# cc-ai/MUNIT

Measured on AMD Instinct MI355X. Metric: images/sec (gen_update+dis_update) @256x256 bs=8, higher is better.
Workload: dtype f32; 1 GPU; config_256.yaml AdaINGen_double+MsImageDis dis_update+gen_update, 256x256, per-GPU batch 8, fp32; global_batch=8, parallelism=dp1, gen_state=1

## Files before the change

### munit_amd/csrc/common.h

```cpp
#pragma once
#include <hip/hip_runtime.h>
#include <cstdarg>
#include <cstdio>
#include <cstdlib>
#include "../../include/munit_hip.h"

typedef float f32x4 __attribute__((ext_vector_type(4)));
typedef float f32x16 __attribute__((ext_vector_type(16)));

typedef __bf16 bf16_t;
typedef __bf16 bf16v4 __attribute__((ext_vector_type(4)));
typedef __bf16 bf16v8 __attribute__((ext_vector_type(8)));

__device__ inline f32x4 ld4(const float* p) { return *reinterpret_cast<const f32x4*>(p); }
__device__ inline f32x4 ld4(const bf16_t* p) {
  const bf16v4 h = *reinterpret_cast<const bf16v4*>(p);
  return f32x4{(float)h[0], (float)h[1], (float)h[2], (float)h[3]};
}
__device__ inline void st4(float* p, f32x4 v) { *reinterpret_cast<f32x4*>(p) = v; }
__device__ inline void st4(bf16_t* p, f32x4 v) {
  *reinterpret_cast<bf16v4*>(p) = bf16v4{(bf16_t)v[0], (bf16_t)v[1], (bf16_t)v[2], (bf16_t)v[3]};
}
__device__ inline float ld1(const float* p) { return *p; }
__device__ inline float ld1(const bf16_t* p) { return (float)*p; }
__device__ inline void st1(float* p, float v) { *p = v; }
__device__ inline void st1(bf16_t* p, float v) { *p = (bf16_t)v; }

void munit_set_error(const char* fmt, ...);

#define MUNIT_CHECK_ARG(cond, ...)         \
  do {                                     \
    if (!(cond)) {                         \
      munit_set_error(__VA_ARGS__);        \
      return MUNIT_ERR_ARG;                \
    }                                      \
  } while (0)

#define MUNIT_CHECK_LAUNCH(what)                                                   \
  do {                                                                             \
    hipError_t e_ = hipGetLastError();                                             \
    if (e_ != hipSuccess) {                                                        \
      munit_set_error("%s: launch failed: %s", what, hipGetErrorString(e_));       \
      return MUNIT_ERR_LAUNCH;                                                     \
    }                                                                              \
  } while (0)

#define MUNIT_ENV_FLAG(name) ([]() -> bool { static const bool v_ = getenv(name) != nullptr; return v_; }())

static inline size_t align_up(size_t v, size_t a) { return (v + a - 1) / a * a; }
static inline int cdiv(long long a, long long b) { return (int)((a + b - 1) / b); }

__device__ inline float wave_sum(float v) {
#pragma unroll
  for (int off = 32; off > 0; off >>= 1) v += __shfl_xor(v, off, 64);
  return v;
}

__device__ inline float apply_act(float v, int act, float slope) {
  if (act == MUNIT_ACT_RELU) return v > 0.f ? v : 0.f;
  if (act == MUNIT_ACT_LRELU) return v > 0.f ? v : v * slope;
  if (act == MUNIT_ACT_TANH) return tanhf(v);
  return v;
}

__device__ inline int src_coord(int v, int Hu, int ups, int reflect) {
  const bool inside = v >= 0 && v < Hu;
  int r = v < 0 ? -v : v;
  r = r >= Hu ? 2 * Hu - 2 - r : r;
  r = reflect ? r : (inside ? v : -1);
  return r < 0 ? -1 : (r >> ups);
}

double munit_igemm_executed_flops(const munit_conv_desc* d, int pass);
const char* munit_igemm_kernel_name(const munit_conv_desc* d, int pass);

bool munit_small_fwd_supported(const munit_conv_desc* d);
bool munit_small_fwd_ok(const munit_conv_desc* d);
bool munit_small_wgrad_ok(const munit_conv_desc* d);
enum SmallFwdKernel { SMALL_FWD_PK, SMALL_FWD_MFMA, SMALL_FWD_PATCH };
SmallFwdKernel munit_small_fwd_kernel(int Cin);
bool munit_small_wgrad_pk();
size_t munit_small_fwd_workspace(const munit_conv_desc* d);
int munit_small_fwd(const munit_conv_desc* d, int Ho, int Wo, const void* x, const float* w, const float* bias,
                    float* y, void* ws, hipStream_t st);
size_t munit_small_wgrad_workspace(const munit_conv_desc* d, int Ho);
int munit_small_wgrad(const munit_conv_desc* d, int Ho, int Wo, const void* x, const float* dy, float* dw,
                      float* db, float beta, void* ws, hipStream_t st);
```

### munit_amd/csrc/conv_igemm.hip

```cpp
#include "common.h"
#include "wino.h"
#include <cstdlib>

namespace {

struct IgemmParams {
  const float* x;
  const float* w;
  const float* bias;
  void* y;
  int B, H, W, Cin;
  int Hu, Wu, ups;
  int Ho, Wo, Cout;
  int KH, KW, stride, pad, reflect;
  int Ktot;
  long long w_row;
  long long y_sb;
  long long y_sh;
  int y_sw;
  int M;
  int act;
  float slope;
  int ps;
  long long w_phase;
  long long y_phase_row;
  int y_phase_col;
  int n_tiles;
  int f_pad, f_ups, f_reflect, f_Hu, f_Wu;
  int frame;
  int ksplit, kt_per_split;
  float* slab;
  int ct;
  int patch;
  int out_bf16;
  int bf16s;
  int cin4;
};

__device__ inline f32x4 bf16x8_add4(f32x4 l, f32x4 a, f32x4 b, f32x4 c) {
  const bf16v8 L = __builtin_bit_cast(bf16v8, l), A = __builtin_bit_cast(bf16v8, a), B = __builtin_bit_cast(bf16v8, b),
               C = __builtin_bit_cast(bf16v8, c);
  bf16v8 r;
#pragma unroll
  for (int e = 0; e < 8; ++e) r[e] = (bf16_t)((float)L[e] + (((float)A[e] + (float)B[e]) + (float)C[e]));
  return __builtin_bit_cast(f32x4, r);
}

__device__ inline void decode_pixel(int m, int Ho, int Wo, int frame, int& b, int& oh, int& ow) {
  if (!frame) {
    const int HoWo = Ho * Wo;
    b = m / HoWo;
    const int rem = m - b * HoWo;
    oh = rem / Wo;
    ow = rem - oh * Wo;
  } else {
    const int F = frame, F2 = 2 * frame;
    const int nb = F2 * Wo + F2 * (Ho - F2);
    b = m / nb;
    int r = m - b * nb;
    if (r < F2 * Wo) {
      const int q = r / Wo;
      ow = r - q * Wo;
      oh = q < F ? q : Ho - F2 + q;
    } else {
      r -= F2 * Wo;
      const int rr = r / F2, q = r - rr * F2;
      oh = F + rr;
      ow = q < F ? q : Wo - F2 + q;
    }
  }
}

constexpr int BM = 128;
constexpr int BK = 32;
#ifndef IGEMM_WAVES
#define IGEMM_WAVES 8
#endif
constexpr int NWAVES = IGEMM_WAVES;
constexpr int NTHR = 64 * NWAVES;
constexpr int LDS_LD = BK + 4;

__device__ inline uint2 fold_cands(int i, int Hu, int ups, int P, int reflect) {
  unsigned long long pk = ~0ull;
  int n = 0;
  auto push = [&](int v) {
    if (n < 4) {
      const int sh = 16 * n;
      pk = (pk & ~(0xFFFFull << sh)) | ((unsigned long long)(unsigned)v << sh);
      ++n;
    }
  };
  const int nu = 1 << ups;
  for (int du = 0; du < nu; ++du) {
    const int hu = (i << ups) + du;
    push(hu + P);
    if (reflect) {
      if (hu >= 1 && hu <= P) push(P - hu);
      if (hu >= Hu - 1 - P && hu <= Hu - 2) push(2 * Hu - 2 - hu + P);
    }
  }
  return make_uint2((unsigned)(pk & 0xFFFFFFFFull), (unsigned)(pk >> 32));
}
__device__ inline int cand_at(uint2 v, int a) {
  const unsigned w = (a & 2) ? v.y : v.x;
  return (int)((w >> ((a & 1) * 16)) & 0xFFFFu);
}

typedef __bf16 bf16x4 __attribute__((ext_vector_type(4)));
typedef __bf16 bf16x8 __attribute__((ext_vector_type(8)));

__device__ const float munit_zero_page[32] = {0.f};

template <int BN, bool ALIGNED, int ROLE, int CT = 0>
__global__ __launch_bounds__(NTHR, NWAVES == 8 ? ((CT == 3 && BN == 64) ? 6 : 4) : 2) void conv_igemm_kernel(IgemmParams p) {
  constexpr bool BF16 = CT == 1 || CT == 2;
  constexpr bool DMA = CT == 3 || CT == 4 || CT == 5;
  constexpr bool BF16S = CT == 4;
  constexpr bool CIN4 = CT == 5;
  static_assert(!CIN4 || ROLE != 2, "4-channel taps: single-gather roles only");
  static_assert(!DMA || (ALIGNED && NWAVES == 8), "direct-to-LDS loads: aligned variants only");
  constexpr bool PATCH = DMA && ROLE == 2;
  constexpr int NPL = CT == 2 ? 3 : 1;
  static_assert(!BF16 || ALIGNED, "bf16 operands need Cin % 32 == 0");
  constexpr int WN = NWAVES == 8 ? 32 : 64;
  constexpr int WAVES_N = BN / WN;
  constexpr int WAVES_M = NWAVES / WAVES_N;
  constexpr int WM = BM / WAVES_M;
  constexpr int MT = WM / 16;
  constexpr int NT = WN / 16;
#ifndef IGEMM_LOADER_WAVES
#define IGEMM_LOADER_WAVES 8
#endif
  constexpr int LW = (CT == 3 && ROLE != 2 && NWAVES == 8) ? IGEMM_LOADER_WAVES : NWAVES;
  constexpr int RSTEP = 64 * LW / 8;
  constexpr int AROWS = BM / RSTEP;
  constexpr int BROWS = BN / RSTEP;
  constexpr int CLD = BN + 4;
  static_assert(BM * CLD <= 2 * (BM + BN) * LDS_LD, "C staging tile must fit in the operand buffers");
  constexpr int SMEM_FLOATS = DMA ? (2 * (BM + BN) * 32 > BM * CLD ? 2 * (BM + BN) * 32 : BM * CLD) : 2 * (BM + BN) * LDS_LD;
  __shared__ __attribute__((aligned(16))) float smem[SMEM_FLOATS];
  float* const As = smem;
  float* const Bs = smem + 2 * BM * LDS_LD;

  const int tid = threadIdx.x;
  const int lane = tid & 63;
  const int wave = tid >> 6;
  const int wm = wave / WAVES_N, wn = wave % WAVES_N;

  int tile = blockIdx.x;
  {
    const int nb = gridDim.x, q = nb >> 3, r = nb & 7, xcd = tile & 7, idx = tile >> 3;
    tile = (xcd < r ? xcd * (q + 1) : r * (q + 1) + (xcd - r) * q) + idx;
  }
  const int n_tile = tile % p.n_tiles;
  const int m_tile = tile / p.n_tiles;
  const int m0 = m_tile * BM;
  const int n0 = n_tile * BN;

  const float* __restrict__ xg = p.x;
  const float* __restrict__ wg = p.w;
  long long y_base = 0;
  if (p.ps > 1) {
    const int pa = blockIdx.y / p.ps, pb = blockIdx.y % p.ps;
    wg += (long long)blockIdx.y * p.w_phase;
    y_base = (long long)pa * p.y_phase_row + (long long)pb * p.y_phase_col;
  }

  const int c4 = tid & 7;
  const int r0 = tid >> 3;
  int a_base[AROWS];
  int a_ih0[AROWS], a_iw0[AROWS];
  bool a_ok[AROWS];
  uint2 a_ch[AROWS], a_cw[AROWS];
  int a_nc[AROWS];
  int f_h1[PATCH ? AROWS : 1], f_w1[PATCH ? AROWS : 1];
#pragma unroll
  for (int i = 0; i < AROWS; ++i) {
    int m = m0 + r0 + RSTEP * i;
    a_ok[i] = m < p.M;
    int mm = a_ok[i] ? m : 0;
    int b, oh, ow;
    decode_pixel(mm, p.Ho, p.Wo, p.frame, b, oh, ow);
    a_base[i] = b * p.H * p.W;
    a_ih0[i] = oh * p.stride - p.pad;
    a_iw0[i] = ow * p.stride - p.pad;
    if constexpr (PATCH) {
      constexpr int NONE = -(1 << 20);
      const int P = p.f_pad, K1 = p.KH - 1;
      int h1 = NONE, w1 = NONE;
      if (p.f_reflect) {
        if (oh >= 1 && oh <= P) h1 = P - oh - K1;
        else if (oh >= p.f_Hu - 1 - P && oh <= p.f_Hu - 2) h1 = 2 * p.f_Hu - 2 - oh + P - K1;
        if (ow >= 1 && ow <= P) w1 = P - ow - K1;
        else if (ow >= p.f_Wu - 1 - P && ow <= p.f_Wu - 2) w1 = 2 * p.f_Wu - 2 - ow + P - K1;
      }
      a_ih0[i] = oh + P - K1;
      a_iw0[i] = ow + P - K1;
      f_h1[i] = h1;
      f_w1[i] = w1;
    } else if constexpr (ROLE == 2) {
      a_ch[i] = fold_cands(oh, p.f_Hu, p.f_ups, p.f_pad, p.f_reflect);
      a_cw[i] = fold_cands(ow, p.f_Wu, p.f_ups, p.f_pad, p.f_reflect);
      int nh = 0, nw = 0;
      for (int a = 0; a < 4; ++a) {
        nh += cand_at(a_ch[i], a) != 0xFFFF;
        nw += cand_at(a_cw[i], a) != 0xFFFF;
      }
      a_nc[i] = nh | (nw << 4);
    }
  }

  f32x4 ra[AROWS], rb[BROWS];
  f32x4 rx[ROLE == 2 ? AROWS : 1];
  int kh = 0, kw = 0, c0 = 0;
  const int nk_total = (p.Ktot + BK - 1) / BK;
  const int kt_begin = p.ksplit > 1 ? blockIdx.z * p.kt_per_split : 0;
  const int kt_end = p.ksplit > 1 ? min(nk_total, kt_begin + p.kt_per_split) : nk_total;
  if constexpr (ALIGNED) {
    if (kt_begin > 0) {
      const int k0 = kt_begin * BK, tap = k0 / p.Cin;
      c0 = k0 - tap * p.Cin;
      kh = tap / p.KW;
      kw = tap - kh * p.KW;
    }
  }
  int aoff[AROWS];
  int aoff1[ROLE == 2 ? AROWS : 1];
  int aoffp[PATCH ? 3 : 1][AROWS];
  f32x4 xp[PATCH ? 3 : 1][AROWS];
  bool wave_patch = false;

  auto tap_setup = [&]() {
#pragma unroll
    for (int i = 0; i < AROWS; ++i) {
      if constexpr (PATCH) {
        const int vh0 = a_ih0[i] + kh, vh1 = f_h1[i] + kh, vw0 = a_iw0[i] + kw, vw1 = f_w1[i] + kw;
        const bool h0 = a_ok[i] && (unsigned)vh0 < (unsigned)p.H, h1 = a_ok[i] && (unsigned)vh1 < (unsigned)p.H;
        const bool w0 = (unsigned)vw0 < (unsigned)p.W, w1 = (unsigned)vw1 < (unsigned)p.W;
        aoff[i] = (h0 && w0) ? (a_base[i] + vh0 * p.W + vw0) * p.Cin : -1;
        aoffp[0][i] = (h0 && w1) ? (a_base[i] + vh0 * p.W + vw1) * p.Cin : -1;
        aoffp[1][i] = (h1 && w0) ? (a_base[i] + vh1 * p.W + vw0) * p.Cin : -1;
        aoffp[2][i] = (h1 && w1) ? (a_base[i] + vh1 * p.W + vw1) * p.Cin : -1;
        if (i == 0) wave_patch = false;
        wave_patch = wave_patch || __builtin_amdgcn_ballot_w64((aoffp[0][i] & aoffp[1][i] & aoffp[2][i]) >= 0) != 0;
      } else if constexpr (ROLE == 2) {
        const int nw = a_nc[i] >> 4;
        const int ncomb = (a_nc[i] & 15) * nw;
        int o0 = -1, o1 = -1;
        {
          const int vh = cand_at(a_ch[i], 0) + kh - (p.KH - 1);
          const int vw = cand_at(a_cw[i], 0) + kw - (p.KW - 1);
          const bool ok = a_ok[i] && vh >= 0 && vh < p.H && vw >= 0 && vw < p.W;
          o0 = ok ? (a_base[i] + vh * p.W + vw) * p.Cin : -1;
        }
        {
          const int vh = cand_at(a_ch[i], nw >= 2 ? 0 : 1) + kh - (p.KH - 1);
          const int vw = cand_at(a_cw[i], nw >= 2 ? 1 : 0) + kw - (p.KW - 1);
          const bool ok = a_ok[i] && ncomb >= 2 && vh >= 0 && vh < p.H && vw >= 0 && vw < p.W;
          o1 = ok ? (a_base[i] + vh * p.W + vw) * p.Cin : -1;
        }
        aoff[i] = o0;
        aoff1[i] = o1;
      } else {
        const int ih = src_coord(a_ih0[i] + kh, p.Hu, p.ups, p.reflect);
        const int iw = src_coord(a_iw0[i] + kw, p.Wu, p.ups, p.reflect);
        const bool ok = a_ok[i] && ih >= 0 && iw >= 0;
        aoff[i] = ok ? (a_base[i] + ih * p.W + iw) * p.Cin : -1;
      }
    }
  };

  auto load_tile = [&](int kt) {
    if constexpr (ALIGNED) {
      if (c0 == 0 || kt == kt_begin) tap_setup();
#pragma unroll
      for (int i = 0; i < AROWS; ++i) {
        f32x4 v = {0.f, 0.f, 0.f, 0.f};
        if (aoff[i] >= 0) v = *reinterpret_cast<const f32x4*>(xg + (long long)aoff[i] + c0 + c4 * 4);
        if constexpr (ROLE == 2) {
          f32x4 x1 = {0.f, 0.f, 0.f, 0.f};
          if (aoff1[i] >= 0) x1 = *reinterpret_cast<const f32x4*>(xg + (long long)aoff1[i] + c0 + c4 * 4);
          const int nw = a_nc[i] >> 4;
          const int ncomb = (a_nc[i] & 15) * nw;
          if (a_ok[i] && ncomb > 2) {
            for (int cidx = 2; cidx < ncomb; cidx += 2) {
              f32x4 t0 = {0.f, 0.f, 0.f, 0.f}, t1 = {0.f, 0.f, 0.f, 0.f};
              {
                const int a = cidx / nw, b2 = cidx - a * nw;
                const int vh = cand_at(a_ch[i], a) + kh - (p.KH - 1);
                const int vw = cand_at(a_cw[i], b2) + kw - (p.KW - 1);
                if (vh >= 0 && vh < p.H && vw >= 0 && vw < p.W)
                  t0 = *reinterpret_cast<const f32x4*>(xg + (long long)(a_base[i] + vh * p.W + vw) * p.Cin + c0 + c4 * 4);
              }
              if (cidx + 1 < ncomb) {
                const int a = (cidx + 1) / nw, b2 = cidx + 1 - a * nw;
                const int vh = cand_at(a_ch[i], a) + kh - (p.KH - 1);
                const int vw = cand_at(a_cw[i], b2) + kw - (p.KW - 1);
                if (vh >= 0 && vh < p.H && vw >= 0 && vw < p.W)
                  t1 = *reinterpret_cast<const f32x4*>(xg + (long long)(a_base[i] + vh * p.W + vw) * p.Cin + c0 + c4 * 4);
              }
              x1 += t0 + t1;
            }
          }
          rx[i] = x1;
        }
        ra[i] = v;
      }
#pragma unroll
      for (int i = 0; i < BROWS; ++i) {
        const int n = n0 + r0 + RSTEP * i;
        f32x4 v = {0.f, 0.f, 0.f, 0.f};
        if (n < p.Cout) v = *reinterpret_cast<const f32x4*>(wg + (long long)n * p.w_row + kt * BK + c4 * 4);
        rb[i] = v;
      }
      c0 += BK;
      if (c0 >= p.Cin) {
        c0 = 0;
        if (++kw == p.KW) { kw = 0; ++kh; }
      }
    } else {
      int ekh[4], ekw[4], eci[4];
      bool eok[4];
#pragma unroll
      for (int e = 0; e < 4; ++e) {
        int k = kt * BK + c4 * 4 + e;
        eok[e] = k < p.Ktot;
        int kk = eok[e] ? k : 0;
        int tap = kk / p.Cin;
        eci[e] = kk - tap * p.Cin;
        ekh[e] = tap / p.KW;
        ekw[e] = tap - ekh[e] * p.KW;
      }
#pragma unroll
      for (int i = 0; i < AROWS; ++i) {
        f32x4 v;
#pragma unroll
        for (int e = 0; e < 4; ++e) {
          int ih = src_coord(a_ih0[i] + ekh[e], p.Hu, p.ups, p.reflect);
          int iw = src_coord(a_iw0[i] + ekw[e], p.Wu, p.ups, p.reflect);
          bool ok = a_ok[i] && eok[e] && ih >= 0 && iw >= 0;
          float s = 0.f;
          if (ok) s = xg[(a_base[i] + (long long)ih * p.W + iw) * p.Cin + eci[e]];
          v[e] = s;
        }
        ra[i] = v;
      }
#pragma unroll
      for (int i = 0; i < BROWS; ++i) {
        int n = n0 + r0 + RSTEP * i;
        f32x4 v;
#pragma unroll
        for (int e = 0; e < 4; ++e) {
          int k = kt * BK + c4 * 4 + e;
          float s = 0.f;
          if (n < p.Cout && k < p.Ktot) s = wg[(long long)n * p.w_row + k];
          v[e] = s;
        }
        rb[i] = v;
      }
    }
  };

  const int dma_col = ((c4 ^ ((r0 >> 1) & 7)) * 4);
  auto dma_tile = [&](int kt, int buf) {
    if constexpr (DMA) {
      if (LW < NWAVES && __builtin_amdgcn_readfirstlane(wave) >= LW) return;
      if constexpr (!CIN4) {
        if (c0 == 0 || kt == kt_begin) tap_setup();
      }
      const int wrow = __builtin_amdgcn_readfirstlane(wave) * 8;
      const int tap4 = kt * 8 + (dma_col >> 2);
      const int kh4 = tap4 / p.KW, kw4 = tap4 - kh4 * p.KW;
#pragma unroll
      for (int i = 0; i < AROWS; ++i) {
        const float* g;
        if constexpr (CIN4) {
          const int ih = src_coord(a_ih0[i] + kh4, p.Hu, p.ups, p.reflect);
          const int iw = src_coord(a_iw0[i] + kw4, p.Wu, p.ups, p.reflect);
          const bool ok = a_ok[i] && tap4 < p.KH * p.KW && ih >= 0 && iw >= 0;
          g = ok ? xg + (long long)(a_base[i] + ih * p.W + iw) * 4 : munit_zero_page;
        } else {
          g = aoff[i] >= 0 ? xg + (long long)aoff[i] + c0 + dma_col : munit_zero_page + dma_col;
        }
        float* l = smem + buf * (BM * 32) + (wrow + RSTEP * i) * 32;
        __builtin_amdgcn_global_load_lds((const __attribute__((address_space(1))) void*)g,
                                         (__attribute__((address_space(3))) void*)l, 16, 0, 0);
        if constexpr (PATCH) {
          if (wave_patch) {
#pragma unroll
            for (int c = 0; c < 3; ++c) {
              f32x4 v = {0.f, 0.f, 0.f, 0.f};
              if (aoffp[c][i] >= 0) v = *reinterpret_cast<const f32x4*>(xg + (long long)aoffp[c][i] + c0 + dma_col);
              xp[c][i] = v;
            }
          }
        }
      }
#pragma unroll
      for (int i = 0; i < BROWS; ++i) {
        const int n = min(n0 + r0 + RSTEP * i, p.Cout - 1);
        const float* g = wg + (long long)n * p.w_row + kt * BK + dma_col;
        float* l = smem + 2 * BM * 32 + buf * (BN * 32) + (wrow + RSTEP * i) * 32;
        __builtin_amdgcn_global_load_lds((const __attribute__((address_space(1))) void*)g,
                                         (__attribute__((address_space(3))) void*)l, 16, 0, 0);
      }
      if constexpr (!CIN4) {
        c0 += BK;
        if (c0 >= p.Cin) {
          c0 = 0;
          if (++kw == p.KW) { kw = 0; ++kh; }
        }
      }
    }
  };

  __bf16* const Ah = reinterpret_cast<__bf16*>(smem);
  __bf16* const Bh = Ah + (CT == 2 ? 3 : 2) * BM * 32;
  const int st_swz = (0x78 >> (2 * ((r0 >> 2) & 3))) & 3;
  const int st_col = (((c4 >> 1) ^ st_swz) * 8) + (c4 & 1) * 4;
  auto store_tile = [&](int buf) {
    if constexpr (BF16) {
      auto put = [&](__bf16* base, int plane_elems, int row, f32x4 v) {
#pragma unroll
        for (int pl = 0; pl < NPL; ++pl) {
          bf16x4 h;
#pragma unroll
          for (int e = 0; e < 4; ++e) h[e] = (__bf16)v[e];
          *reinterpret_cast<bf16x4*>(&base[pl * plane_elems + row * 32 + st_col]) = h;
          if (pl + 1 < NPL) {
#pragma unroll
            for (int e = 0; e < 4; ++e) v[e] -= (float)h[e];
          }
        }
      };
#pragma unroll
      for (int i = 0; i < AROWS; ++i) {
        if constexpr (ROLE == 2) ra[i] += rx[i];
        put(Ah + buf * NPL * (BM * 32), BM * 32, r0 + RSTEP * i, ra[i]);
      }
#pragma unroll
      for (int i = 0; i < BROWS; ++i) put(Bh + buf * NPL * (BN * 32), BN * 32, r0 + RSTEP * i, rb[i]);
      return;
    }
    float* Ad = As + buf * (BM * LDS_LD);
    float* Bd = Bs + buf * (BN * LDS_LD);
#pragma unroll
    for (int i = 0; i < AROWS; ++i) {
      if constexpr (ROLE == 2) ra[i] += rx[i];
      *reinterpret_cast<f32x4*>(&Ad[(r0 + RSTEP * i) * LDS_LD + c4 * 4]) = ra[i];
    }
#pragma unroll
    for (int i = 0; i < BROWS; ++i)
      *reinterpret_cast<f32x4*>(&Bd[(r0 + RSTEP * i) * LDS_LD + c4 * 4]) = rb[i];
  };

  f32x4 acc[MT][NT];
#pragma unroll
  for (int mt = 0; mt < MT; ++mt)
#pragma unroll
    for (int nt = 0; nt < NT; ++nt)
#pragma unroll
      for (int r = 0; r < 4; ++r) acc[mt][nt][r] = 0.f;

  const int frag_row = lane & 15;
  const int frag_k = (lane >> 4) * 4;
  const int fr_col = (((lane >> 4) ^ ((0x78 >> (2 * ((frag_row >> 2) & 3))) & 3)) * 8);
  auto compute_half = [&](int buf, int kg) {
    if constexpr (BF16) {
      const __bf16* Ac = Ah + buf * NPL * (BM * 32);
      const __bf16* Bc = Bh + buf * NPL * (BN * 32);
      bf16x8 hb[NPL][NT];
#pragma unroll
      for (int pl = 0; pl < NPL; ++pl)
#pragma unroll
        for (int nt = 0; nt < NT; ++nt)
          hb[pl][nt] = *reinterpret_cast<const bf16x8*>(&Bc[pl * (BN * 32) + (wn * WN + nt * 16 + frag_row) * 32 + fr_col]);
#pragma unroll
      for (int mt = kg * (MT / 2); mt < (kg + 1) * (MT / 2); ++mt) {
        bf16x8 ha[NPL];
#pragma unroll
        for (int pl = 0; pl < NPL; ++pl)
          ha[pl] = *reinterpret_cast<const bf16x8*>(&Ac[pl * (BM * 32) + (wm * WM + mt * 16 + frag_row) * 32 + fr_col]);
#pragma unroll
        for (int sum = NPL - 1; sum >= 0; --sum)
#pragma unroll
          for (int i = 0; i <= sum; ++i)
#pragma unroll
            for (int nt = 0; nt < NT; ++nt)
              acc[mt][nt] = __builtin_amdgcn_mfma_f32_16x16x32_bf16(ha[i], hb[sum - i][nt], acc[mt][nt], 0, 0, 0);
      }
      return;
    }
    if constexpr (DMA) {
      const float* Ac = smem + buf * (BM * 32);
      const float* Bc = smem + 2 * BM * 32 + buf * (BN * 32);
      const int pos = ((kg * 4 + (lane >> 4)) ^ ((frag_row >> 1) & 7)) * 4;
      f32x4 a[MT], b[NT];
#pragma unroll
      for (int nt = 0; nt < NT; ++nt)
        b[nt] = *reinterpret_cast<const f32x4*>(&Bc[(wn * WN + nt * 16 + frag_row) * 32 + pos]);
#pragma unroll
      for (int mt = 0; mt < MT; ++mt)
        a[mt] = *reinterpret_cast<const f32x4*>(&Ac[(wm * WM + mt * 16 + frag_row) * 32 + pos]);
      if constexpr (BF16S) {
#pragma unroll
        for (int mt = 0; mt < MT; ++mt)
#pragma unroll
          for (int nt = 0; nt < NT; ++nt)
            acc[mt][nt] = __builtin_amdgcn_mfma_f32_16x16x32_bf16(__builtin_bit_cast(bf16x8, a[mt]),
                                                                  __builtin_bit_cast(bf16x8, b[nt]), acc[mt][nt], 0, 0, 0);
        return;
      }
#pragma unroll
      for (int t = 0; t < 4; ++t)
#pragma unroll
        for (int mt = 0; mt < MT; ++mt)
#pragma unroll
          for (int nt = 0; nt < NT; ++nt)
            acc[mt][nt] = __builtin_amdgcn_mfma_f32_16x16x4f32(a[mt][t], b[nt][t], acc[mt][nt], 0, 0, 0);
      return;
    }
    const float* Ac = As + buf * (BM * LDS_LD);
    const float* Bc = Bs + buf * (BN * LDS_LD);
    f32x4 a[MT], b[NT];
#pragma unroll
    for (int nt = 0; nt < NT; ++nt)
      b[nt] = *reinterpret_cast<const f32x4*>(&Bc[(wn * WN + nt * 16 + frag_row) * LDS_LD + kg * 16 + frag_k]);
    constexpr int MB = (ROLE == 2 && MT >= 4) ? MT / 2 : MT;
#pragma unroll
    for (int m0t = 0; m0t < MT; m0t += MB) {
#pragma unroll
      for (int mt = m0t; mt < m0t + MB; ++mt)
        a[mt] = *reinterpret_cast<const f32x4*>(&Ac[(wm * WM + mt * 16 + frag_row) * LDS_LD + kg * 16 + frag_k]);
#pragma unroll
      for (int t = 0; t < 4; ++t)
#pragma unroll
        for (int mt = m0t; mt < m0t + MB; ++mt)
#pragma unroll
          for (int nt = 0; nt < NT; ++nt)
            acc[mt][nt] = __builtin_amdgcn_mfma_f32_16x16x4f32(a[mt][t], b[nt][t], acc[mt][nt], 0, 0, 0);
      if constexpr (MB != MT) __builtin_amdgcn_sched_barrier(0);
    }
  };

  const int nk = kt_end - kt_begin;
  auto patch_tile = [&](int buf) {
    if constexpr (PATCH) {
      if (!wave_patch) return;
#pragma unroll
      for (int i = 0; i < AROWS; ++i) {
        if ((aoffp[0][i] & aoffp[1][i] & aoffp[2][i]) >= 0) {
          f32x4* l = reinterpret_cast<f32x4*>(smem + buf * (BM * 32) + (r0 + RSTEP * i) * 32 + c4 * 4);
          if constexpr (BF16S) *l = bf16x8_add4(*l, xp[0][i], xp[1][i], xp[2][i]);
          else *l = *l + ((xp[0][i] + xp[1][i]) + xp[2][i]);
        }
      }
    }
  };
  if constexpr (DMA) {
    if (nk > 0) dma_tile(kt_begin, 0);
    asm volatile("s_waitcnt vmcnt(0)" ::: "memory");
    if (nk > 0) patch_tile(0);
    __syncthreads();
    for (int kt = 0; kt < nk; ++kt) {
      const int cur = kt & 1;
      if (kt + 1 < nk) dma_tile(kt_begin + kt + 1, cur ^ 1);
      compute_half(cur, 0);
      compute_half(cur, 1);
      asm volatile("s_waitcnt vmcnt(0)" ::: "memory");
      if (kt + 1 < nk) patch_tile(cur ^ 1);
      __syncthreads();
    }
  } else if constexpr (CT == 2) {
    if (nk > 0) load_tile(kt_begin);
    for (int kt = 0; kt < nk; ++kt) {
      __syncthreads();
      store_tile(0);
      if (kt + 1 < nk) load_tile(kt_begin + kt + 1);
      __syncthreads();
      compute_half(0, 0);
      compute_half(0, 1);
    }
    __syncthreads();
  } else {
    if (nk > 0) {
      load_tile(kt_begin);
      store_tile(0);
    }
    __syncthreads();
    if (nk > 1) load_tile(kt_begin + 1);
    for (int kt = 0; kt < nk; ++kt) {
      const int cur = kt & 1;
      compute_half(cur, 0);
      if (kt + 1 < nk) {
#ifndef ABL_NOLDSW
        store_tile(cur ^ 1);
#endif
#ifndef ABL_NOGLOBAL
        if (kt + 2 < nk) load_tile(kt_begin + kt + 2);
#endif
      }
      if constexpr (ROLE == 2) __builtin_amdgcn_sched_barrier(0);
      compute_half(cur, 1);
#ifndef ABL_NOBAR
      __syncthreads();
#endif
    }
  }

  float* const Cs = smem;
#pragma unroll
  for (int nt = 0; nt < NT; ++nt)
#pragma unroll
    for (int mt = 0; mt < MT; ++mt)
#pragma unroll
      for (int r = 0; r < 4; ++r)
        Cs[(wm * WM + mt * 16 + 4 * (lane >> 4) + r) * CLD + wn * WN + nt * 16 + (lane & 15)] = acc[mt][nt][r];
  __syncthreads();
  constexpr int CQ = BN / 4;
  constexpr int CRPT = NTHR / CQ;
  const int cq = tid % CQ, cr0 = tid / CQ;
  const int n = n0 + cq * 4;
  const bool split = p.ksplit > 1;
  float* const sl = split ? p.slab + ((long long)blockIdx.y * p.ksplit + blockIdx.z) * (long long)p.M * p.Cout : nullptr;
  const bool vec = (p.Cout & 3) == 0 && (split || ((p.y_sw & 3) == 0 && (p.y_sh & 3) == 0 && (p.y_sb & 3) == 0));
  f32x4 bv = {0.f, 0.f, 0.f, 0.f};
  if (!split && p.bias != nullptr) {
#pragma unroll
    for (int e = 0; e < 4; ++e)
      if (n + e < p.Cout) bv[e] = p.bias[n + e];
  }
#pragma unroll 2
  for (int row = cr0; row < BM; row += CRPT) {
    const int m = m0 + row;
    if (m >= p.M || n >= p.Cout) continue;
    f32x4 v = *reinterpret_cast<const f32x4*>(&Cs[row * CLD + cq * 4]);
    if (split) {
      float* dst = sl + (long long)m * p.Cout + n;
      if (vec) {
        *reinterpret_cast<f32x4*>(dst) = v;
      } else {
#pragma unroll
        for (int e = 0; e < 4; ++e)
          if (n + e < p.Cout) dst[e] = v[e];
      }
      continue;
    }
    int b, oh, ow;
    decode_pixel(m, p.Ho, p.Wo, p.frame, b, oh, ow);
    const long long off = y_base + (long long)b * p.y_sb + (long long)oh * p.y_sh + (long long)ow * p.y_sw + n;
#pragma unroll
    for (int e = 0; e < 4; ++e) v[e] = apply_act(v[e] + bv[e], p.act, p.slope);
    if (p.out_bf16) {
      bf16_t* dst = reinterpret_cast<bf16_t*>(p.y) + off;
      if (vec) {
        st4(dst, v);
      } else {
#pragma unroll
        for (int e = 0; e < 4; ++e)
          if (n + e < p.Cout) dst[e] = (bf16_t)v[e];
      }
    } else {
      float* dst = reinterpret_cast<float*>(p.y) + off;
      if (vec) {
        *reinterpret_cast<f32x4*>(dst) = v;
      } else {
#pragma unroll
        for (int e = 0; e < 4; ++e)
          if (n + e < p.Cout) dst[e] = v[e];
      }
    }
  }
}

__global__ void splitk_epilogue_kernel(IgemmParams p, int phases) {
  const long long per = (long long)p.M * p.Cout;
  const long long total = per * phases;
  for (long long i = (long long)blockIdx.x * blockDim.x + threadIdx.x; i < total;
       i += (long long)gridDim.x * blockDim.x) {
    const int ph = (int)(i / per);
    const long long r = i - (long long)ph * per;
    const int m = (int)(r / p.Cout), n = (int)(r - (long long)m * p.Cout);
    float s = 0.f;
    for (int k = 0; k < p.ksplit; ++k) s += p.slab[((long long)ph * p.ksplit + k) * per + r];
    int b, oh, ow;
    decode_pixel(m, p.Ho, p.Wo, p.frame, b, oh, ow);
    long long off = (long long)b * p.y_sb + (long long)oh * p.y_sh + (long long)ow * p.y_sw + n;
    if (p.ps > 1) off += (long long)(ph / p.ps) * p.y_phase_row + (long long)(ph % p.ps) * p.y_phase_col;
    const float bv = p.bias != nullptr ? p.bias[n] : 0.f;
    const float res = apply_act(s + bv, p.act, p.slope);
    if (p.out_bf16) reinterpret_cast<bf16_t*>(p.y)[off] = (bf16_t)res;
    else reinterpret_cast<float*>(p.y)[off] = res;
  }
}

typedef munit_prep_item PrepItem;

__device__ inline void prep_dgrad_elem(const PrepItem& it, long long i) {
  const int ps = it.ps, TH = it.KH / ps, TW = it.KW / ps;
  long long r_ = i;
  int co = (int)(r_ % it.Cout); r_ /= it.Cout;
  int r = (int)(r_ % TW); r_ /= TW;
  int t = (int)(r_ % TH); r_ /= TH;
  int ci = (int)(r_ % it.Cin); r_ /= it.Cin;
  int ph = (int)r_;
  int pa = ph / ps, pb = ph % ps;
  int kh = pa + ps * (TH - 1 - t);
  int kw = pb + ps * (TW - 1 - r);
  const float v = it.w[(((long long)co * it.KH + kh) * it.KW + kw) * it.Cin + ci];
  if (it.bf16) reinterpret_cast<bf16_t*>(it.wp)[i] = (bf16_t)v;
  else it.wp[i] = v;
}

__device__ inline void prep_cast_elem(const PrepItem& it, long long i) { reinterpret_cast<bf16_t*>(it.wp)[i] = (bf16_t)it.w[i]; }

__device__ inline void prep_subpixel_elem(const PrepItem& it, long long i) {
  const long long merged = (long long)4 * 9 * it.Cout * it.Cin;
  if (i >= merged) {
    reinterpret_cast<bf16_t*>(it.wp)[i] = (bf16_t)it.w[i - merged];
    return;
  }
  long long r = i;
  const int ci = (int)(r % it.Cin); r /= it.Cin;
  const int dw = (int)(r % 3); r /= 3;
  const int dh = (int)(r % 3); r /= 3;
  const int co = (int)(r % it.Cout); r /= it.Cout;
  const int ph = (int)r;
  const int a = ph >> 1, b = ph & 1;
  const int h0 = a == 0 ? (dh == 0 ? 0 : dh == 1 ? 2 : 4) : (dh == 0 ? 0 : dh == 1 ? 1 : 3);
  const int hn = a == 0 ? (dh == 2 ? 1 : 2) : (dh == 0 ? 1 : 2);
  const int w0 = b == 0 ? (dw == 0 ? 0 : dw == 1 ? 2 : 4) : (dw == 0 ? 0 : dw == 1 ? 1 : 3);
  const int wn = b == 0 ? (dw == 2 ? 1 : 2) : (dw == 0 ? 1 : 2);
  float s = 0.f;
  for (int kh = h0; kh < h0 + hn; ++kh)
    for (int kw = w0; kw < w0 + wn; ++kw) s += it.w[(((long long)co * 5 + kh) * 5 + kw) * it.Cin + ci];
  if (it.bf16) reinterpret_cast<bf16_t*>(it.wp)[i] = (bf16_t)s;
  else it.wp[i] = s;
}

__host__ __device__ inline long long prep_elems(const PrepItem& it) {
  const long long cc = (long long)it.Cout * it.Cin;
  if (it.kind == MUNIT_PREP_SUBPIXEL) return it.bf16 ? (4 * 9 + 25) * cc : 4 * 9 * cc;
  if (it.kind == MUNIT_PREP_WINOGRAD || it.kind == MUNIT_PREP_WINOGRAD_DGRAD) return wino_image_elems(it.Cin, it.Cout);
  if (it.kind == MUNIT_PREP_SUBPIXEL_WINOGRAD_DGRAD) return cc * it.KH * it.KW + 4 * wino_image_elems(it.Cin, it.Cout);
  if (it.kind == MUNIT_PREP_SUBPIXEL_WINOGRAD || it.kind == MUNIT_PREP_WINOGRAD_S2 || it.kind == MUNIT_PREP_WINOGRAD_S2_DGRAD)
    return 4 * wino_image_elems(it.Cin, it.Cout);
  return cc * it.KH * it.KW;
}

__host__ __device__ inline long long prep_trips(const PrepItem& it) {
  const bool wino = it.kind == MUNIT_PREP_WINOGRAD || it.kind == MUNIT_PREP_WINOGRAD_DGRAD || it.kind == MUNIT_PREP_SUBPIXEL_WINOGRAD ||
                    it.kind == MUNIT_PREP_WINOGRAD_S2 || it.kind == MUNIT_PREP_WINOGRAD_S2_DGRAD;
  if (it.kind == MUNIT_PREP_SUBPIXEL_WINOGRAD_DGRAD) return (long long)it.Cout * it.Cin * (it.KH * it.KW + 4);
  return wino ? prep_elems(it) / 16 : prep_elems(it);
}
template <bool DEV>
__global__ void prep_weights_kernel(const PrepItem* __restrict__ items, PrepItem one) {
  const PrepItem it = DEV ? items[blockIdx.y] : one;
  const long long total = prep_trips(it);
  for (long long i = (long long)blockIdx.x * blockDim.x + threadIdx.x; i < total; i += (long long)gridDim.x * blockDim.x) {
    if (it.kind == MUNIT_PREP_SUBPIXEL) prep_subpixel_elem(it, i);
    else if (it.kind == MUNIT_PREP_WINOGRAD || it.kind == MUNIT_PREP_WINOGRAD_DGRAD)
      wino_weight_item(it.w, it.wp, it.Cout, it.Cin, it.kind == MUNIT_PREP_WINOGRAD_DGRAD, i);
    else if (it.kind == MUNIT_PREP_SUBPIXEL_WINOGRAD) wino_subpixel_weight_item(it.w, it.wp, it.Cout, it.Cin, i);
    else if (it.kind == MUNIT_PREP_WINOGRAD_S2) wino_s2_weight_item(it.w, it.wp, it.Cout, it.Cin, i);
    else if (it.kind == MUNIT_PREP_WINOGRAD_S2_DGRAD) wino_s2_dgrad_weight_item(it.w, it.wp, it.Cout, it.Cin, i);
    else if (it.kind == MUNIT_PREP_SUBPIXEL_WINOGRAD_DGRAD) {
      const long long nd = (long long)it.Cout * it.Cin * it.KH * it.KW;
      if (i < nd) prep_dgrad_elem(it, i);
      else wino_subpixel_dgrad_weight_item(it.w, it.wp + nd, it.Cout, it.Cin, i - nd);
    }
    else if (it.kind == MUNIT_PREP_CAST) prep_cast_elem(it, i);
    else prep_dgrad_elem(it, i);
  }
}

int launch_prep_one(const PrepItem& it, hipStream_t st) {
  const long long total = prep_trips(it);
  const int blocks = (int)std::min<long long>((total + 255) / 256, 4096);
  hipLaunchKernelGGL(prep_weights_kernel<false>, dim3(blocks), dim3(256), 0, st, nullptr, it);
  MUNIT_CHECK_LAUNCH("prep_weights");
  return MUNIT_OK;
}

template <typename T>
__global__ void fold_kernel(const T* __restrict__ g, const T* __restrict__ add,
                            T* __restrict__ dx, int B, int H, int W, int C, int ups, int pad,
                            int reflect, int Hq, int Wq) {
  const int C4 = C >> 2;
  const long long total = (long long)B * H * W * C4;
  const int Hu = H << ups, Wu = W << ups;
  for (long long i = (long long)blockIdx.x * blockDim.x + threadIdx.x; i < total;
       i += (long long)gridDim.x * blockDim.x) {
    long long r_ = i;
    int c4 = (int)(r_ % C4); r_ /= C4;
    int iw = (int)(r_ % W); r_ /= W;
    int ih = (int)(r_ % H); r_ /= H;
    int b = (int)r_;
    f32x4 s = {0.f, 0.f, 0.f, 0.f};
    const int nu = 1 << ups;
    for (int du = 0; du < nu; ++du) {
      int hu = (ih << ups) + du;
      int qr[3], nr = 0;
      qr[nr++] = hu + pad;
      if (reflect) {
        if (hu >= 1 && hu <= pad) qr[nr++] = pad - hu;
        if (hu >= Hu - 1 - pad && hu <= Hu - 2) qr[nr++] = 2 * Hu - 2 - hu + pad;
      }
      for (int dv = 0; dv < nu; ++dv) {
        int wu = (iw << ups) + dv;
        int qc[3], nc = 0;
        qc[nc++] = wu + pad;
        if (reflect) {
          if (wu >= 1 && wu <= pad) qc[nc++] = pad - wu;
          if (wu >= Wu - 1 - pad && wu <= Wu - 2) qc[nc++] = 2 * Wu - 2 - wu + pad;
        }
        for (int a = 0; a < nr; ++a) {
          if (qr[a] >= Hq) continue;
          for (int c = 0; c < nc; ++c) {
            if (qc[c] >= Wq) continue;
            s += ld4(g + (((long long)b * Hq + qr[a]) * Wq + qc[c]) * C + c4 * 4);
          }
        }
      }
    }
    if (add != nullptr) s += ld4(add + i * 4);
    st4(dx + i * 4, s);
  }
}

__global__ void fold_scalar_kernel(const float* __restrict__ g, const float* __restrict__ add,
                                   float* __restrict__ dx, int B, int H, int W, int C, int ups, int pad,
                                   int reflect, int Hq, int Wq) {
  const long long total = (long long)B * H * W * C;
  const int Hu = H << ups, Wu = W << ups;
  for (long long i = (long long)blockIdx.x * blockDim.x + threadIdx.x; i < total;
       i += (long long)gridDim.x * blockDim.x) {
    long long r_ = i;
    int c = (int)(r_ % C); r_ /= C;
    int iw = (int)(r_ % W); r_ /= W;
    int ih = (int)(r_ % H); r_ /= H;
    int b = (int)r_;
    float s = 0.f;
    const int nu = 1 << ups;
    for (int du = 0; du < nu; ++du) {
      int hu = (ih << ups) + du;
      int qr[3], nr = 0;
      qr[nr++] = hu + pad;
      if (reflect) {
        if (hu >= 1 && hu <= pad) qr[nr++] = pad - hu;
        if (hu >= Hu - 1 - pad && hu <= Hu - 2) qr[nr++] = 2 * Hu - 2 - hu + pad;
      }
      for (int dv = 0; dv < nu; ++dv) {
        int wu = (iw << ups) + dv;
        int qc[3], nc = 0;
        qc[nc++] = wu + pad;
        if (reflect) {
          if (wu >= 1 && wu <= pad) qc[nc++] = pad - wu;
          if (wu >= Wu - 1 - pad && wu <= Wu - 2) qc[nc++] = 2 * Wu - 2 - wu + pad;
        }
        for (int a = 0; a < nr; ++a) {
          if (qr[a] >= Hq) continue;
          for (int cc = 0; cc < nc; ++cc) {
            if (qc[cc] >= Wq) continue;
            s += g[(((long long)b * Hq + qr[a]) * Wq + qc[cc]) * C + c];
          }
        }
      }
    }
    if (add != nullptr) s += add[i];
    dx[i] = s;
  }
}

__global__ void add_inplace_kernel(float* __restrict__ y, const float* __restrict__ a, long long n) {
  for (long long i = (long long)blockIdx.x * blockDim.x + threadIdx.x; i < n; i += (long long)gridDim.x * blockDim.x)
    y[i] += a[i];
}

int pick_ksplit(int M, int Cout, int Ktot, int phases) {
  const int bn = Cout <= 64 ? 64 : 128;
  const int tiles = cdiv(M, BM) * cdiv(Cout, bn) * phases;
  const int nk = cdiv(Ktot, BK);
  if (tiles >= 192 || nk < 16 || MUNIT_ENV_FLAG("MUNIT_DEBUG_NO_SPLITK")) return 1;
  int ks = std::min(cdiv(512, tiles), nk / 4);
  return std::max(1, std::min(ks, 32));
}
size_t splitk_bytes(int M, int Cout, int Ktot, int phases) {
  const int ks = pick_ksplit(M, Cout, Ktot, phases);
  return ks > 1 ? align_up((size_t)ks * phases * M * Cout * sizeof(float), 256) : 0;
}

enum IgemmForm {
  IG_REFUSED_BF16_CIN, IG_REFUSED_CIN4_FOLD, IG_REFUSED_BF16_FOLD, IG_REFUSED_FOLD_UNALIGNED,
  IG_CIN4,
  IG_BF16S,
  IG_PATCH,
  IG_DMA,
  IG_CT2,
  IG_CT1,
  IG_F32,
  IG_UNALIGNED
};
IgemmForm igemm_form(const IgemmParams& p, int role) {
  if (p.bf16s && (p.Cin % (2 * BK) != 0 || NWAVES != 8)) return IG_REFUSED_BF16_CIN;
  const int cin = p.bf16s ? p.Cin / 2 : p.Cin, w_row = p.bf16s ? p.w_row / 2 : p.w_row;
  const bool aligned = (cin % BK == 0) && (w_row % 4 == 0);
  if (p.cin4) return role == 2 ? IG_REFUSED_CIN4_FOLD : IG_CIN4;
  if (p.bf16s) return role == 2 && (!p.patch || p.frame) ? IG_REFUSED_BF16_FOLD : IG_BF16S;
  if (role == 2) {
    if (!aligned) return IG_REFUSED_FOLD_UNALIGNED;
    if (p.ct == 0 && p.patch && !p.frame && NWAVES == 8 && !MUNIT_ENV_FLAG("MUNIT_DEBUG_NO_PATCH")) return IG_PATCH;
    return p.ct == 2 ? IG_CT2 : p.ct == 1 ? IG_CT1 : IG_F32;
  }
  if (aligned && p.ct == 0 && NWAVES == 8 && !MUNIT_ENV_FLAG("MUNIT_DEBUG_NO_DMA")) return IG_DMA;
  if (!aligned) return IG_UNALIGNED;
  return p.ct == 2 ? IG_CT2 : p.ct == 1 ? IG_CT1 : IG_F32;
}
int igemm_bn(const IgemmParams& p) { return p.Cout <= 64 ? 64 : 128; }

#define IGEMM_LAUNCH(...)                                                                                  \
  do {                                                                                                     \
    if (bn == 64) hipLaunchKernelGGL((conv_igemm_kernel<64, __VA_ARGS__>), grid, block, 0, st, q);         \
    else hipLaunchKernelGGL((conv_igemm_kernel<128, __VA_ARGS__>), grid, block, 0, st, q);                 \
  } while (0)

template <int ROLE>
int launch_igemm(const IgemmParams& p, int phases, hipStream_t st, void* slab = nullptr, size_t slab_bytes = 0) {
  const int bn = igemm_bn(p);
  IgemmParams q = p;
  const IgemmForm form = igemm_form(p, ROLE);
  switch (form) {
    case IG_REFUSED_BF16_CIN:
      munit_set_error("conv_igemm: bf16 storage needs a multiple of 64 input channels (got %d)", p.Cin);
      return MUNIT_ERR_ARG;
    case IG_REFUSED_CIN4_FOLD:
      munit_set_error("conv_igemm: 4-channel taps are not a folded-backward-data form");
      return MUNIT_ERR_ARG;
    case IG_REFUSED_BF16_FOLD:
      munit_set_error("conv_igemm: bf16-storage folded backward-data exists for the LDS-patch form only");
      return MUNIT_ERR_ARG;
    case IG_REFUSED_FOLD_UNALIGNED:
      munit_set_error("conv_igemm: folded backward-data needs Cout %% 32 == 0");
      return MUNIT_ERR_ARG;
    default: break;
  }
  if (p.bf16s) {
    q.Cin = p.Cin / 2; q.Ktot = p.Ktot / 2; q.w_row = p.w_row / 2; q.w_phase = p.w_phase / 2;
    slab = nullptr;
  }
  q.n_tiles = cdiv(p.Cout, bn);
  const int m_tiles = cdiv(p.M, BM);
  q.ksplit = 1;
  if (slab != nullptr) {
    const int ks = pick_ksplit(p.M, p.Cout, p.Ktot, phases);
    if (ks > 1 && slab_bytes >= splitk_bytes(p.M, p.Cout, p.Ktot, phases)) {
      const int nk = cdiv(p.Ktot, BK);
      q.kt_per_split = cdiv(nk, ks);
      q.ksplit = cdiv(nk, q.kt_per_split);
      q.slab = reinterpret_cast<float*>(slab);
    }
  }
  dim3 grid((unsigned)(m_tiles * q.n_tiles), (unsigned)phases, (unsigned)q.ksplit);
  dim3 block(NTHR);
  switch (form) {
    case IG_CIN4:
      if constexpr (ROLE != 2) IGEMM_LAUNCH(true, ROLE, 5);
      break;
    case IG_BF16S: IGEMM_LAUNCH(true, ROLE, 4); break;
    case IG_PATCH: IGEMM_LAUNCH(true, 2, 3); break;
    case IG_DMA: IGEMM_LAUNCH(true, ROLE, 3); break;
    case IG_CT2: IGEMM_LAUNCH(true, ROLE, 2); break;
    case IG_CT1: IGEMM_LAUNCH(true, ROLE, 1); break;
    case IG_F32: IGEMM_LAUNCH(true, ROLE); break;
    default:
      if constexpr (ROLE != 2) IGEMM_LAUNCH(false, ROLE);
      break;
  }
  MUNIT_CHECK_LAUNCH("conv_igemm");
  if (q.ksplit > 1) {
    const long long total = (long long)p.M * p.Cout * phases;
    const int blocks = (int)std::min<long long>((total + 255) / 256, 4096);
    hipLaunchKernelGGL(splitk_epilogue_kernel, dim3(blocks), dim3(256), 0, st, q, phases);
    MUNIT_CHECK_LAUNCH("splitk_epilogue");
  }
  return MUNIT_OK;
}

int check_desc(const munit_conv_desc* d) {
  MUNIT_CHECK_ARG(d != nullptr, "conv: null descriptor");
  MUNIT_CHECK_ARG(d->B > 0 && d->H > 0 && d->W > 0 && d->Cin > 0 && d->Cout > 0, "conv: bad dims");
  MUNIT_CHECK_ARG(d->KH > 0 && d->KW > 0 && d->stride > 0 && d->pad >= 0, "conv: bad kernel geometry");
  MUNIT_CHECK_ARG(d->upsample == 0 || d->upsample == 1, "conv: upsample must be 0 or 1");
  MUNIT_CHECK_ARG(d->compute >= MUNIT_COMPUTE_F32 && d->compute <= MUNIT_COMPUTE_F32X3, "conv: bad compute mode %d", d->compute);
  MUNIT_CHECK_ARG(d->pad_mode == MUNIT_PAD_ZERO || d->pad_mode == MUNIT_PAD_REFLECT, "conv: bad pad mode");
  MUNIT_CHECK_ARG((d->in_dtype == MUNIT_DTYPE_F32 || d->in_dtype == MUNIT_DTYPE_BF16) &&
                  (d->out_dtype == MUNIT_DTYPE_F32 || d->out_dtype == MUNIT_DTYPE_BF16), "conv: bad tensor dtype");
  MUNIT_CHECK_ARG(d->in_dtype == MUNIT_DTYPE_F32 || d->Cin % 64 == 0, "conv: a bf16 input needs Cin %% 64 == 0 (got %d)", d->Cin);
  MUNIT_CHECK_ARG(d->out_dtype == MUNIT_DTYPE_F32 || d->Cout % 64 == 0, "conv: a bf16 output needs Cout %% 64 == 0 (got %d)", d->Cout);
  const int Hu = d->H << d->upsample, Wu = d->W << d->upsample;
  if (d->pad_mode == MUNIT_PAD_REFLECT)
    MUNIT_CHECK_ARG(d->pad < Hu && d->pad < Wu, "conv: reflect pad %d needs input > pad (got %dx%d)", d->pad, Hu, Wu);
  MUNIT_CHECK_ARG(Hu + 2 * d->pad >= d->KH && Wu + 2 * d->pad >= d->KW, "conv: kernel larger than padded input");
  MUNIT_CHECK_ARG((long long)d->B * Hu * Wu < (1ll << 31) / 4, "conv: too many pixels for 32-bit tile indices");
  MUNIT_CHECK_ARG((long long)d->B * (Hu + 2 * d->pad) * (Wu + 2 * d->pad) * std::max(d->Cin, d->Cout) < (1ll << 31),
                  "conv: tensor too large for the 32-bit element offsets of the tile loader");
  return MUNIT_OK;
}

}

extern "C" int munit_conv2d_out_hw(const munit_conv_desc* d, int* Ho, int* Wo) {
  int rc = check_desc(d);
  if (rc) return rc;
  *Ho = ((d->H << d->upsample) + 2 * d->pad - d->KH) / d->stride + 1;
  *Wo = ((d->W << d->upsample) + 2 * d->pad - d->KW) / d->stride + 1;
  return MUNIT_OK;
}

namespace {
bool subpixel_ok(const munit_conv_desc* d) {
  return d->upsample == 1 && d->KH == 5 && d->KW == 5 && d->pad == 2 && d->stride == 1 &&
         d->pad_mode == MUNIT_PAD_REFLECT && d->Cin % 32 == 0 && d->H >= 3 && d->W >= 3 &&
         !MUNIT_ENV_FLAG("MUNIT_DEBUG_NO_SUBPIXEL");
}
}

namespace {
__global__ void pad3to4_image_kernel(const float* __restrict__ x, f32x4* __restrict__ x4, long long npix) {
  for (long long i = (long long)blockIdx.x * blockDim.x + threadIdx.x; i < npix; i += (long long)gridDim.x * blockDim.x)
    x4[i] = f32x4{x[3 * i], x[3 * i + 1], x[3 * i + 2], 0.f};
}
__global__ void pad3to4_weight_kernel(const float* __restrict__ w, float* __restrict__ w4, int N, int taps, int kpad) {
  const long long total = (long long)N * kpad;
  for (long long i = (long long)blockIdx.x * blockDim.x + threadIdx.x; i < total; i += (long long)gridDim.x * blockDim.x) {
    const int n = (int)(i / kpad), k = (int)(i - (long long)n * kpad);
    const int tap = k >> 2, c = k & 3;
    w4[i] = (tap < taps && c < 3) ? w[((long long)n * taps + tap) * 3 + c] : 0.f;
  }
}
struct Cin4Plan {
  int kpad;
  size_t x4_bytes, w4_bytes;
};
Cin4Plan plan_cin4(long long npix, int N, int taps) {
  Cin4Plan c;
  c.kpad = (taps * 4 + BK - 1) / BK * BK;
  c.x4_bytes = align_up((size_t)npix * 4 * sizeof(float), 256);
  c.w4_bytes = align_up((size_t)N * c.kpad * sizeof(float), 256);
  return c;
}
int build_cin4(const Cin4Plan& c, const float* x3, long long npix, const float* w3, int N, int taps, void* ws, hipStream_t st) {
  f32x4* x4 = reinterpret_cast<f32x4*>(ws);
  float* w4 = reinterpret_cast<float*>(reinterpret_cast<char*>(ws) + c.x4_bytes);
  hipLaunchKernelGGL(pad3to4_image_kernel, dim3((unsigned)std::min<long long>((npix + 255) / 256, 8192)), dim3(256), 0, st, x3, x4, npix);
  MUNIT_CHECK_LAUNCH("pad3to4_image");
  hipLaunchKernelGGL(pad3to4_weight_kernel, dim3((unsigned)cdiv((long long)N * c.kpad, 256)), dim3(256), 0, st, w3, w4, N, taps, c.kpad);
  MUNIT_CHECK_LAUNCH("pad3to4_weight");
  return MUNIT_OK;
}
bool cin4_fwd_ok(const munit_conv_desc* d) {
  return d->Cin == 3 && d->in_dtype == MUNIT_DTYPE_F32 && d->upsample == 0 && d->KH * d->KW <= 64 && d->Cout % 4 == 0 &&
         NWAVES == 8 && !MUNIT_ENV_FLAG("MUNIT_DEBUG_NO_CIN4");
}

void set_cin4(IgemmParams* p, const Cin4Plan& c) { p->Ktot = c.kpad; p->w_row = c.kpad; p->cin4 = 1; }

IgemmParams fwd_params(const munit_conv_desc* d, int Ho, int Wo) {
  IgemmParams p{};
  p.B = d->B; p.H = d->H; p.W = d->W; p.Cin = d->Cin;
  p.ups = d->upsample; p.Hu = d->H << p.ups; p.Wu = d->W << p.ups;
  p.Ho = Ho; p.Wo = Wo; p.Cout = d->Cout;
  p.KH = d->KH; p.KW = d->KW; p.stride = d->stride; p.pad = d->pad;
  p.reflect = d->pad_mode == MUNIT_PAD_REFLECT;
  p.Ktot = d->KH * d->KW * d->Cin;
  p.w_row = p.Ktot;
  p.y_sw = d->Cout;
  p.y_sh = (long long)Wo * d->Cout;
  p.y_sb = (long long)Ho * Wo * d->Cout;
  p.M = d->B * Ho * Wo;
  p.act = d->act; p.slope = d->slope;
  p.ct = d->compute;
  p.ps = 1;
  p.bf16s = d->in_dtype == MUNIT_DTYPE_BF16;
  p.out_bf16 = d->out_dtype == MUNIT_DTYPE_BF16;
  return p;
}
IgemmParams subpixel_phase_params(const IgemmParams& p, const munit_conv_desc* d, int Wo) {
  IgemmParams q = p;
  q.ups = 0; q.Hu = d->H; q.Wu = d->W;
  q.Ho = d->H; q.Wo = d->W;
  q.KH = 3; q.KW = 3; q.pad = 1; q.reflect = 0;
  q.Ktot = 9 * d->Cin; q.w_row = q.Ktot;
  q.y_sw = 2 * d->Cout;
  q.y_sh = (long long)2 * Wo * d->Cout;
  q.M = d->B * d->H * d->W;
  q.ps = 2;
  q.w_phase = (long long)d->Cout * q.Ktot;
  q.y_phase_row = (long long)Wo * d->Cout;
  q.y_phase_col = d->Cout;
  return q;
}
void set_subpixel_frame(IgemmParams* p, const munit_conv_desc* d, int Ho, int Wo, int ring) {
  p->frame = ring;
  p->M = d->B * (2 * ring * Wo + 2 * ring * (Ho - 2 * ring));
}

bool wino_geometry_ok(const munit_conv_desc* d) {
  return d->compute == MUNIT_COMPUTE_F32 && d->in_dtype == MUNIT_DTYPE_F32 && d->out_dtype == MUNIT_DTYPE_F32 &&
         d->KH == 3 && d->KW == 3 && d->stride == 1 && d->pad == 1 && d->upsample == 0 && d->act != MUNIT_ACT_TANH;
}
bool wino_fwd_ok(const munit_conv_desc* d) { return wino_geometry_ok(d) && munit_wino_ok(d->B, d->H, d->W, d->Cin, d->Cout); }
long long wino_s2_min_blocks(bool dgrad) {
  static const char* const e = getenv("MUNIT_WINO_S2_MIN_BLOCKS");
  static const long long v = e ? atoll(e) : 0;
  return e ? v : dgrad ? 100 : 192;
}
bool wino_s2_fwd_ok(const munit_conv_desc* d) {
  return d->compute == MUNIT_COMPUTE_F32 && d->in_dtype == MUNIT_DTYPE_F32 && d->out_dtype == MUNIT_DTYPE_F32 && d->KH == 4 &&
         d->KW == 4 && d->stride == 2 && d->pad == 1 && d->upsample == 0 && d->act != MUNIT_ACT_TANH && d->H >= 4 && d->W >= 4 &&
         munit_wino_ok(d->B, d->H, d->W, d->Cin, d->Cout) && !MUNIT_ENV_FLAG("MUNIT_DEBUG_NO_WINOGRAD_S2") &&
         (long long)cdiv((long long)d->B * cdiv(d->H / 2, 3) * cdiv(d->W / 2, 3), 64) * (d->Cout / 64) >= wino_s2_min_blocks(false);
}
bool wino_s2_dgrad_ok(const munit_conv_desc* d) {
  if (!(d->compute == MUNIT_COMPUTE_F32 && d->in_dtype == MUNIT_DTYPE_F32 && d->out_dtype == MUNIT_DTYPE_F32 && d->KH == 4 &&
        d->KW == 4 && d->stride == 2 && d->pad == 1 && d->upsample == 0 && d->H >= 4 && d->W >= 4 && d->H % 2 == 0 && d->W % 2 == 0 &&
        d->Cout % 8 == 0 && d->Cin % 64 == 0 && !MUNIT_ENV_FLAG("MUNIT_DEBUG_NO_WINOGRAD_S2") && !MUNIT_ENV_FLAG("MUNIT_DEBUG_NO_WINOGRAD")))
    return false;
  const int Hd = d->H / 2, Wd = d->W / 2;
  if (d->pad_mode == MUNIT_PAD_REFLECT && (Hd % 3 == 0 || Wd % 3 == 0)) return false;
  if ((long long)d->B * d->H * d->W * std::max(d->Cin, d->Cout) >= (1ll << 29)) return false;
  return (long long)cdiv((long long)d->B * cdiv(Hd + 1, 3) * cdiv(Wd + 1, 3), 64) * (d->Cin / 64) * 4 >= wino_s2_min_blocks(true);
}
bool subpixel_wino_ok(const munit_conv_desc* d) {
  return d->compute == MUNIT_COMPUTE_F32 && d->in_dtype == MUNIT_DTYPE_F32 && d->out_dtype == MUNIT_DTYPE_F32 &&
         d->act != MUNIT_ACT_TANH && munit_wino_ok(d->B, d->H, d->W, d->Cin, d->Cout);
}

enum FwdRoute { FWD_SMALL, FWD_SUBPIXEL_WINO, FWD_SUBPIXEL, FWD_WINO, FWD_WINO_S2, FWD_CIN4, FWD_IGEMM };
struct FwdPlan {
  int rc;
  FwdRoute route;
  int Ho, Wo;
  munit_prep_item prep;
  Cin4Plan cin4;
  int ring;
  size_t img_bytes, ws_bytes;
};
FwdPlan plan_fwd(const munit_conv_desc* d) {
  FwdPlan pl{};
  if ((pl.rc = munit_conv2d_out_hw(d, &pl.Ho, &pl.Wo)) != MUNIT_OK) return pl;
  const int Ho = pl.Ho, Wo = pl.Wo, Ktot = d->KH * d->KW * d->Cin;
  const bool bf16 = d->in_dtype == MUNIT_DTYPE_BF16;
  int kind = bf16 ? MUNIT_PREP_CAST : MUNIT_PREP_NONE;
  if (munit_small_fwd_ok(d)) {
    pl.route = FWD_SMALL; kind = MUNIT_PREP_NONE;
  } else if (subpixel_ok(d)) {
    const bool wino = subpixel_wino_ok(d);
    pl.route = wino ? FWD_SUBPIXEL_WINO : FWD_SUBPIXEL; kind = wino ? MUNIT_PREP_SUBPIXEL_WINOGRAD : MUNIT_PREP_SUBPIXEL;
    pl.ring = wino ? 1 : 2;
  } else if (wino_fwd_ok(d)) {
    pl.route = FWD_WINO; kind = MUNIT_PREP_WINOGRAD;
  } else if (wino_s2_fwd_ok(d)) {
    pl.route = FWD_WINO_S2; kind = MUNIT_PREP_WINOGRAD_S2;
  } else {
    pl.route = cin4_fwd_ok(d) ? FWD_CIN4 : FWD_IGEMM;
  }
  pl.prep = munit_prep_item{nullptr, nullptr, d->Cout, d->KH, d->KW, d->Cin, kind, 1, pl.route != FWD_SMALL && bf16};
  pl.ws_bytes = pl.img_bytes = kind == MUNIT_PREP_NONE ? 0 : align_up((size_t)prep_elems(pl.prep) * (bf16 ? 2 : 4), 256);
  if (pl.route == FWD_SMALL) pl.ws_bytes = munit_small_fwd_workspace(d);
  if (pl.route == FWD_CIN4) pl.cin4 = plan_cin4((long long)d->B * d->H * d->W, d->Cout, d->KH * d->KW), pl.ws_bytes = pl.cin4.x4_bytes + pl.cin4.w4_bytes;
  if (bf16 || munit_small_fwd_supported(d)) return pl;
  if (pl.ring)
    pl.ws_bytes += std::max(splitk_bytes(d->B * (4 * Wo + 4 * (Ho - 4)), d->Cout, Ktot, 1), splitk_bytes(d->B * (2 * Wo + 2 * (Ho - 2)), d->Cout, Ktot, 1));
  if (pl.route == FWD_IGEMM) pl.ws_bytes += splitk_bytes(d->B * Ho * Wo, d->Cout, Ktot, 1);
  return pl;
}

enum WinoForm { WINO_FWD, WINO_FWD_S2, WINO_FWD_SUBPIXEL, WINO_DGRAD, WINO_DGRAD_S2, WINO_DGRAD_UP };
WinoParams wino_params(const munit_conv_desc* d, int Ho, int Wo, WinoForm f, const float* x, const float* u, const float* bias, float* y) {
  const bool fwd = f <= WINO_FWD_SUBPIXEL, refl = d->pad_mode == MUNIT_PAD_REFLECT;
  WinoParams q{};
  q.x = x; q.u = u; q.bias = bias; q.y = y;
  q.B = d->B; q.H = d->H; q.W = d->W;
  q.xc = fwd ? d->Cin : d->Cout; q.N = fwd ? d->Cout : d->Cin; q.K = q.xc;
  const int oh = fwd ? Ho : d->H, ow = fwd ? Wo : d->W;
  q.y_sw = q.N; q.y_sh = (long long)ow * q.N; q.y_sb = (long long)oh * ow * q.N;
  q.mode = refl ? 0 : 1;
  q.th = d->H / 2; q.tw = d->W / 2;
  q.act = fwd ? d->act : MUNIT_ACT_NONE; q.slope = fwd ? d->slope : 0.f;
  switch (f) {
    case WINO_FWD: break;
    case WINO_FWD_S2:
      q.K = 4 * q.xc; q.s2 = 1; q.Ho = Ho; q.Wo = Wo;
      q.th = cdiv(Ho, 3); q.tw = cdiv(Wo, 3);
      break;
    case WINO_FWD_SUBPIXEL:
      q.y_sw *= 2; q.y_sh *= 2; q.y_prow = (long long)Wo * d->Cout; q.y_pcol = d->Cout;
      q.u_phase = wino_image_elems(d->Cin, d->Cout); q.phases = 4;
      q.mode = 1; q.edge = 1;
      break;
    case WINO_DGRAD: q.mode = refl ? 2 : 1; break;
    case WINO_DGRAD_S2:
      q.H = d->H / 2; q.W = d->W / 2; q.s2 = 2; q.Ho = d->H; q.Wo = d->W;
      q.th = cdiv(q.H + 1, 3); q.tw = cdiv(q.W + 1, 3);
      q.u_phase = wino_image_elems(d->Cout, d->Cin); q.phases = 4;
      break;
    case WINO_DGRAD_UP:
      q.H = Ho; q.W = Wo; q.K = 4 * q.xc; q.s2 = 3; q.mode = 1;
      q.th = (d->H - 4) / 2; q.tw = (d->W - 4) / 2;
      break;
  }
  q.cpp = q.xc / 8; q.NB = q.N / 64;
  q.x_bytes = (unsigned)((size_t)d->B * q.H * q.W * q.xc * 4);
  q.bth = cdiv(q.th, 8); q.btw = cdiv(q.tw, 8);
  return q;
}
}

extern "C" size_t munit_conv2d_fwd_workspace_bytes(const munit_conv_desc* d) {
  const FwdPlan pl = plan_fwd(d);
  return pl.rc ? 0 : pl.ws_bytes;
}

extern "C" int munit_conv2d_fwd(const munit_conv_desc* d, const void* x, const float* w,
                                const float* bias, void* y, void* ws, size_t ws_bytes,
                                munit_stream_t stream) {
  return munit_conv2d_fwd_prepared(d, x, w, nullptr, bias, y, ws, ws_bytes, stream);
}

extern "C" int munit_conv2d_fwd_prepared(const munit_conv_desc* d, const void* x, const float* w, const void* wp,
                                         const float* bias, void* y, void* ws, size_t ws_bytes,
                                         munit_stream_t stream) {
  const FwdPlan pl = plan_fwd(d);
  int rc = pl.rc;
  if (rc) return rc;
  const int Ho = pl.Ho, Wo = pl.Wo;
  MUNIT_CHECK_ARG(x && w && y, "conv2d_fwd: null pointer");
  MUNIT_CHECK_ARG(pl.route != FWD_SMALL || d->out_dtype == MUNIT_DTYPE_F32, "conv2d_fwd: the 3-channel image head writes fp32");
  hipStream_t st = (hipStream_t)stream;
  if (pl.ws_bytes != 0 && (ws == nullptr || ws_bytes < pl.ws_bytes)) {
    munit_set_error("conv2d_fwd: workspace %zu < %zu", ws_bytes, pl.ws_bytes);
    return MUNIT_ERR_WORKSPACE;
  }
  if (pl.route == FWD_SMALL) return munit_small_fwd(d, Ho, Wo, x, w, bias, reinterpret_cast<float*>(y), ws, st);
  const float* wimg = w;
  if (pl.prep.kind != MUNIT_PREP_NONE) {
    wimg = reinterpret_cast<const float*>(wp);
    if (wimg == nullptr) {
      munit_prep_item it = pl.prep;
      it.w = w; it.wp = reinterpret_cast<float*>(ws);
      rc = launch_prep_one(it, st);
      if (rc) return rc;
      wimg = it.wp;
    }
  }
  if (pl.route == FWD_WINO || pl.route == FWD_WINO_S2 || pl.route == FWD_SUBPIXEL_WINO) {
    const WinoForm f = pl.route == FWD_WINO ? WINO_FWD : pl.route == FWD_WINO_S2 ? WINO_FWD_S2 : WINO_FWD_SUBPIXEL;
    rc = munit_wino_launch(wino_params(d, Ho, Wo, f, reinterpret_cast<const float*>(x), wimg, bias, reinterpret_cast<float*>(y)), st);
    if (rc || pl.route != FWD_SUBPIXEL_WINO) return rc;
  }
  IgemmParams p = fwd_params(d, Ho, Wo);
  p.x = reinterpret_cast<const float*>(x); p.w = wimg; p.bias = bias; p.y = y;
  if (pl.route == FWD_CIN4) {
    const long long npix = (long long)d->B * d->H * d->W;
    rc = build_cin4(pl.cin4, reinterpret_cast<const float*>(x), npix, w, d->Cout, d->KH * d->KW, ws, st);
    if (rc) return rc;
    p.x = reinterpret_cast<const float*>(ws);
    p.w = reinterpret_cast<const float*>(reinterpret_cast<const char*>(ws) + pl.cin4.x4_bytes);
    set_cin4(&p, pl.cin4);
    return launch_igemm<0>(p, 1, st);
  }
  if (pl.ring) {
    if (pl.route == FWD_SUBPIXEL) rc = launch_igemm<0>(subpixel_phase_params(p, d, Wo), 4, st);
    if (rc) return rc;
    set_subpixel_frame(&p, d, Ho, Wo, pl.ring);
    p.w = pl.prep.bf16 ? reinterpret_cast<const float*>(reinterpret_cast<const bf16_t*>(wimg) + (size_t)4 * 9 * d->Cout * d->Cin) : w;
  }
  return launch_igemm<0>(p, 1, st, ws ? reinterpret_cast<char*>(ws) + pl.img_bytes : nullptr, ws ? ws_bytes - pl.img_bytes : 0);
}

namespace {
__global__ void box2x2_kernel(const f32x4* __restrict__ dy, f32x4* __restrict__ s, int B, int H, int W, int C4) {
  const long long total = (long long)B * H * W * C4;
  for (long long i = (long long)blockIdx.x * blockDim.x + threadIdx.x; i < total; i += (long long)gridDim.x * blockDim.x) {
    const int c = (int)(i % C4);
    long long r = i / C4;
    const int v = (int)(r % W); r /= W;
    const int u = (int)(r % H);
    f32x4 a = dy[i];
    if (v + 1 < W) a += dy[i + C4];
    if (u + 1 < H) {
      a += dy[i + (long long)W * C4];
      if (v + 1 < W) a += dy[i + (long long)W * C4 + C4];
    }
    s[i] = a;
    (void)c;
  }
}

enum DgradRoute {
  DG_WINO_S2,
  DG_WINO,
  DG_SMALL,
  DG_FOLD_UPWINO,
  DG_FOLD_BOXSUM,
  DG_FOLD,
  DG_CIN4,
  DG_DIRECT,
  DG_CORR
};
struct DgradPlan {
  int rc;
  DgradRoute route;
  int Ho, Wo, ps, TH, TW, Hq, Wq;
  bool bf16s;
  bool patch;
  munit_prep_item prep;
  munit_conv_desc t;
  Cin4Plan cin4;
  size_t off_g, off_tail, slab_bytes, ws_bytes;
};
int max_fold_cands(int H, int ups, int P, int reflect) {
  const int Hu = H << ups;
  int worst = 0;
  for (int i = 0; i < H; ++i) {
    int n = 0;
    for (int du = 0; du < (1 << ups); ++du) {
      const int hu = (i << ups) + du;
      ++n;
      if (reflect) {
        if (hu >= 1 && hu <= P) ++n;
        if (hu >= Hu - 1 - P && hu <= Hu - 2) ++n;
      }
    }
    worst = std::max(worst, n);
    if (i == 2 * P + 2 && H > 4 * P + 8) i = H - 2 * P - 4;
  }
  return worst;
}
DgradPlan plan_dgrad(const munit_conv_desc* d) {
  DgradPlan pl{};
  if ((pl.rc = munit_conv2d_out_hw(d, &pl.Ho, &pl.Wo)) != MUNIT_OK) return pl;
  if (d->KH % d->stride != 0 || d->KW % d->stride != 0) {
    munit_set_error("conv2d_dgrad: kernel %dx%d not a multiple of stride %d", d->KH, d->KW, d->stride);
    pl.rc = MUNIT_ERR_ARG;
    return pl;
  }
  pl.ps = d->stride;
  pl.TH = d->KH / d->stride;
  pl.TW = d->KW / d->stride;
  pl.Hq = d->stride * (pl.Ho + pl.TH - 1);
  pl.Wq = d->stride * (pl.Wo + pl.TW - 1);
  const bool direct = d->pad == 0 && d->upsample == 0 && pl.Hq == d->H && pl.Wq == d->W;
  const int reflect = d->pad_mode == MUNIT_PAD_REFLECT;
  munit_conv_desc& t = pl.t;
  t.B = d->B; t.H = pl.Ho; t.W = pl.Wo; t.Cin = d->Cout; t.Cout = d->Cin; t.KH = pl.TH; t.KW = pl.TW;
  t.stride = 1; t.pad = pl.TH - 1; t.pad_mode = MUNIT_PAD_ZERO; t.upsample = 0; t.act = MUNIT_ACT_NONE;
  t.in_dtype = d->out_dtype; t.out_dtype = MUNIT_DTYPE_F32;
  int kind = MUNIT_PREP_DGRAD;
  if (wino_s2_dgrad_ok(d)) {
    pl.route = DG_WINO_S2; kind = MUNIT_PREP_WINOGRAD_S2_DGRAD;
  } else if (wino_geometry_ok(d) && munit_wino_ok(d->B, d->H, d->W, d->Cout, d->Cin)) {
    pl.route = DG_WINO; kind = MUNIT_PREP_WINOGRAD_DGRAD;
  } else if (!direct && pl.ps == 1 && munit_small_fwd_supported(&t) && !MUNIT_ENV_FLAG("MUNIT_DEBUG_NO_SMALL_DGRAD")) {
    pl.route = DG_SMALL;
  } else {
    pl.bf16s = d->out_dtype == MUNIT_DTYPE_BF16;
    const bool foldable = !direct && d->stride == 1 && d->Cout % 32 == 0 && d->KH == d->KW &&
                          (d->H << d->upsample) + 2 * d->pad < 0xFFFF && (d->W << d->upsample) + 2 * d->pad < 0xFFFF &&
                          max_fold_cands(d->H, d->upsample, d->pad, reflect) <= 4 &&
                          max_fold_cands(d->W, d->upsample, d->pad, reflect) <= 4 && !MUNIT_ENV_FLAG("MUNIT_DEBUG_NO_FOLD");
    pl.patch = foldable && d->upsample == 0 && max_fold_cands(d->H, 0, d->pad, reflect) <= 2 &&
               max_fold_cands(d->W, 0, d->pad, reflect) <= 2;
    if (foldable && (!pl.bf16s || pl.patch)) {
      const bool boxsum = !pl.bf16s && d->in_dtype == MUNIT_DTYPE_F32 && d->upsample == 1 && d->KH == 5 && d->pad == 2 && reflect &&
                          d->Cin % 4 == 0 && d->H >= 8 && d->W >= 8 && !MUNIT_ENV_FLAG("MUNIT_DEBUG_NO_BOXSUM");
      const bool upwino = boxsum && d->compute == MUNIT_COMPUTE_F32 && d->H % 2 == 0 && d->W % 2 == 0 && d->Cout % 8 == 0 &&
                          d->Cin % 64 == 0 && (long long)d->B * 4 * d->H * d->W * d->Cout < (1ll << 29) &&
                          !MUNIT_ENV_FLAG("MUNIT_DEBUG_NO_WINOGRAD");
      pl.route = upwino ? DG_FOLD_UPWINO : boxsum ? DG_FOLD_BOXSUM : DG_FOLD;
      if (upwino) kind = MUNIT_PREP_SUBPIXEL_WINOGRAD_DGRAD;
    } else if (!direct && pl.ps == 1 && d->Cout == 3 && d->out_dtype == MUNIT_DTYPE_F32 && pl.TH * pl.TW <= 64 && d->Cin % 4 == 0 &&
               NWAVES == 8 && !MUNIT_ENV_FLAG("MUNIT_DEBUG_NO_CIN4")) {
      pl.route = DG_CIN4;
    } else {
      pl.route = direct ? DG_DIRECT : DG_CORR;
    }
  }
  pl.prep = munit_prep_item{nullptr, nullptr, d->Cout, d->KH, d->KW, d->Cin, kind, pl.ps, pl.bf16s};
  pl.off_g = align_up((size_t)prep_elems(pl.prep) * (pl.bf16s ? 2 : 4), 256);
  size_t g_bytes = align_up((size_t)d->B * pl.Hq * pl.Wq * d->Cin * (d->in_dtype == MUNIT_DTYPE_BF16 ? 2 : 4), 256), tail = 0;
  switch (pl.route) {
    case DG_WINO_S2: case DG_WINO: case DG_FOLD: g_bytes = 256; break;
    case DG_SMALL: tail = munit_small_fwd_workspace(&t); break;
    case DG_FOLD_UPWINO: case DG_FOLD_BOXSUM:
      g_bytes = align_up((size_t)d->B * pl.Ho * pl.Wo * d->Cout * sizeof(float), 256);
      tail = pl.slab_bytes = splitk_bytes(d->B * (4 * d->W + 4 * (d->H - 4)), d->Cin, d->KH * d->KW * d->Cout, 1);
      break;
    case DG_CIN4:
      pl.cin4 = plan_cin4((long long)d->B * pl.Ho * pl.Wo, d->Cin, pl.TH * pl.TW);
      tail = pl.cin4.x4_bytes + pl.cin4.w4_bytes;
      break;
    case DG_DIRECT: case DG_CORR:
      if (!pl.bf16s)
        tail = pl.slab_bytes = splitk_bytes(d->B * (pl.Ho + pl.TH - 1) * (pl.Wo + pl.TW - 1), d->Cin, pl.TH * pl.TW * d->Cout, pl.ps * pl.ps);
      break;
  }
  pl.off_tail = pl.off_g + g_bytes;
  pl.ws_bytes = pl.off_tail + tail;
  return pl;
}

IgemmParams dgrad_fold_params(const munit_conv_desc* d, const DgradPlan& pl) {
  IgemmParams p{};
  p.B = d->B; p.H = pl.Ho; p.W = pl.Wo; p.Cin = d->Cout;
  p.ups = 0; p.Hu = pl.Ho; p.Wu = pl.Wo;
  p.Ho = d->H; p.Wo = d->W; p.Cout = d->Cin;
  p.KH = d->KH; p.KW = d->KW; p.stride = 1; p.pad = d->KH - 1; p.reflect = 0;
  p.Ktot = d->KH * d->KW * d->Cout;
  p.w_row = p.Ktot;
  p.y_sw = d->Cin;
  p.y_sh = (long long)d->W * d->Cin;
  p.y_sb = (long long)d->H * d->W * d->Cin;
  p.M = d->B * d->H * d->W;
  p.act = MUNIT_ACT_NONE; p.slope = 0.f;
  p.ct = d->compute;
  p.ps = 1;
  p.f_pad = d->pad; p.f_ups = d->upsample; p.f_reflect = d->pad_mode == MUNIT_PAD_REFLECT;
  p.f_Hu = d->H << d->upsample; p.f_Wu = d->W << d->upsample;
  p.patch = pl.patch;
  p.bf16s = pl.bf16s; p.out_bf16 = d->in_dtype == MUNIT_DTYPE_BF16;
  return p;
}
bool dgrad_fold_dtypes_ok(const munit_conv_desc* d, const DgradPlan& pl) {
  return d->in_dtype != MUNIT_DTYPE_BF16 || pl.bf16s || pl.patch;
}
IgemmParams boxsum_interior_params(const IgemmParams& p, const munit_conv_desc* d) {
  IgemmParams q = p;
  q.Ho = d->H - 4; q.Wo = d->W - 4;
  q.stride = 2; q.pad = -2;
  q.M = d->B * q.Ho * q.Wo;
  return q;
}
void set_boxsum_frame(IgemmParams* p, const munit_conv_desc* d) {
  p->frame = 2;
  p->M = d->B * (4 * d->W + 4 * (d->H - 4));
}
IgemmParams dgrad_corr_params(const munit_conv_desc* d, const DgradPlan& pl) {
  IgemmParams p{};
  p.B = d->B; p.H = pl.Ho; p.W = pl.Wo; p.Cin = d->Cout;
  p.ups = 0; p.Hu = pl.Ho; p.Wu = pl.Wo;
  p.Ho = pl.Ho + pl.TH - 1; p.Wo = pl.Wo + pl.TW - 1; p.Cout = d->Cin;
  p.KH = pl.TH; p.KW = pl.TW; p.stride = 1; p.pad = pl.TH - 1;
  p.reflect = 0;
  p.Ktot = pl.TH * pl.TW * d->Cout;
  p.w_row = p.Ktot;
  p.y_sw = pl.ps * d->Cin;
  p.y_sh = (long long)pl.ps * pl.Wq * d->Cin;
  p.y_sb = (long long)pl.Hq * pl.Wq * d->Cin;
  p.M = d->B * p.Ho * p.Wo;
  p.act = MUNIT_ACT_NONE; p.slope = 0.f;
  p.ct = d->compute;
  p.ps = pl.ps;
  p.w_phase = (long long)d->Cin * p.Ktot;
  p.y_phase_row = (long long)pl.Wq * d->Cin;
  p.y_phase_col = d->Cin;
  p.bf16s = pl.bf16s; p.out_bf16 = d->in_dtype == MUNIT_DTYPE_BF16;
  return p;
}
bool fold_vectorised(const munit_conv_desc* d) { return d->Cin % 4 == 0; }
}

extern "C" size_t munit_conv2d_dgrad_workspace_bytes(const munit_conv_desc* d) {
  const DgradPlan pl = plan_dgrad(d);
  return pl.rc ? 0 : pl.ws_bytes;
}

extern "C" int munit_conv2d_dgrad(const munit_conv_desc* d, const void* dy, const float* w,
                                  const void* add, void* dx, void* ws, size_t ws_bytes,
                                  munit_stream_t stream) {
  return munit_conv2d_dgrad_prepared(d, dy, w, nullptr, add, dx, ws, ws_bytes, stream);
}

namespace {
template <typename T>
int launch_fold(const munit_conv_desc* d, const DgradPlan& pl, const void* g, const void* add, void* dx, hipStream_t st) {
  const int reflect = d->pad_mode == MUNIT_PAD_REFLECT;
  long long total = (long long)d->B * d->H * d->W * (d->Cin / 4);
  int blocks = (int)std::min<long long>((total + 255) / 256, 8192);
  hipLaunchKernelGGL(fold_kernel<T>, dim3(blocks), dim3(256), 0, st, reinterpret_cast<const T*>(g),
                     reinterpret_cast<const T*>(add), reinterpret_cast<T*>(dx), d->B, d->H, d->W, d->Cin, d->upsample,
                     d->pad, reflect, pl.Hq, pl.Wq);
  MUNIT_CHECK_LAUNCH("fold");
  return MUNIT_OK;
}
int launch_fold_scalar(const munit_conv_desc* d, const DgradPlan& pl, const float* g, const float* add, float* dx, hipStream_t st) {
  const int reflect = d->pad_mode == MUNIT_PAD_REFLECT;
  long long total = (long long)d->B * d->H * d->W * d->Cin;
  int blocks = (int)std::min<long long>((total + 255) / 256, 8192);
  hipLaunchKernelGGL(fold_scalar_kernel, dim3(blocks), dim3(256), 0, st, g, add, dx, d->B, d->H, d->W,
                     d->Cin, d->upsample, d->pad, reflect, pl.Hq, pl.Wq);
  MUNIT_CHECK_LAUNCH("fold");
  return MUNIT_OK;
}
int launch_add_inplace(const munit_conv_desc* d, float* dx, const float* add, hipStream_t st) {
  long long n = (long long)d->B * d->H * d->W * d->Cin;
  int blocks = (int)std::min<long long>((n + 255) / 256, 8192);
  hipLaunchKernelGGL(add_inplace_kernel, dim3(blocks), dim3(256), 0, st, dx, add, n);
  MUNIT_CHECK_LAUNCH("add_inplace");
  return MUNIT_OK;
}
}

extern "C" int munit_conv2d_dgrad_prepared(const munit_conv_desc* d, const void* dy_, const float* w, const void* wp,
                                           const void* add_, void* dx_, void* ws, size_t ws_bytes,
                                           munit_stream_t stream) {
  const DgradPlan pl = plan_dgrad(d);
  int rc = pl.rc;
  if (rc) return rc;
  MUNIT_CHECK_ARG(dy_ && (w || wp) && dx_ && ws, "conv2d_dgrad: null pointer");
  if (ws_bytes < pl.ws_bytes) {
    munit_set_error("conv2d_dgrad: workspace %zu < %zu", ws_bytes, pl.ws_bytes);
    return MUNIT_ERR_WORKSPACE;
  }
  const float* dy = reinterpret_cast<const float*>(dy_);
  const float* add = reinterpret_cast<const float*>(add_);
  float* dx = reinterpret_cast<float*>(dx_);
  const bool dx_bf16 = d->in_dtype == MUNIT_DTYPE_BF16;
  MUNIT_CHECK_ARG(!dx_bf16 || d->Cin % 4 == 0, "conv2d_dgrad: bf16 dx needs Cin %% 4 == 0");
  hipStream_t st = (hipStream_t)stream;
  const float* wt = reinterpret_cast<const float*>(wp);
  float* g = reinterpret_cast<float*>(reinterpret_cast<char*>(ws) + pl.off_g);
  char* tail = reinterpret_cast<char*>(ws) + pl.off_tail;
  if (wt == nullptr) {
    munit_prep_item it = pl.prep;
    it.w = w; it.wp = reinterpret_cast<float*>(ws);
    rc = launch_prep_one(it, st);
    if (rc) return rc;
    wt = it.wp;
  }
  switch (pl.route) {
    case DG_WINO_S2:
      rc = munit_wino_launch(wino_params(d, pl.Ho, pl.Wo, WINO_DGRAD_S2, dy, wt, nullptr, dx), st);
      if (rc || add == nullptr) return rc;
      return launch_add_inplace(d, dx, add, st);
    case DG_WINO: {
      WinoParams q = wino_params(d, pl.Ho, pl.Wo, WINO_DGRAD, dy, wt, nullptr, dx);
      q.add = add;
      return munit_wino_launch(q, st);
    }
    case DG_SMALL:
      MUNIT_CHECK_ARG(!dx_bf16, "conv2d_dgrad: the 3-channel data gradient is fp32");
      rc = munit_small_fwd(&pl.t, pl.Hq, pl.Wq, dy_, wt, nullptr, g, tail, st);
      if (rc) return rc;
      return launch_fold_scalar(d, pl, g, add, dx, st);
    case DG_FOLD_UPWINO: case DG_FOLD_BOXSUM: case DG_FOLD: {
      IgemmParams p = dgrad_fold_params(d, pl);
      p.x = dy; p.w = wt; p.bias = nullptr; p.y = dx;
      MUNIT_CHECK_ARG(dgrad_fold_dtypes_ok(d, pl), "conv2d_dgrad: unsupported dtype combination");
      if (pl.route == DG_FOLD) {
        rc = launch_igemm<2>(p, 1, st);
      } else {
        if (pl.route == DG_FOLD_UPWINO) {
          rc = munit_wino_launch(wino_params(d, pl.Ho, pl.Wo, WINO_DGRAD_UP, dy, wt + (size_t)d->Cout * 25 * d->Cin, nullptr,
                                             dx + ((long long)2 * d->W + 2) * d->Cin), st);
        } else {
          const long long total = (long long)d->B * pl.Ho * pl.Wo * (d->Cout / 4);
          hipLaunchKernelGGL(box2x2_kernel, dim3((unsigned)std::min<long long>((total + 255) / 256, 16384)), dim3(256), 0, st,
                             reinterpret_cast<const f32x4*>(dy), reinterpret_cast<f32x4*>(g), d->B, pl.Ho, pl.Wo, d->Cout / 4);
          MUNIT_CHECK_LAUNCH("box2x2");
          IgemmParams q = boxsum_interior_params(p, d);
          q.x = g;
          q.y = dx + ((long long)2 * d->W + 2) * d->Cin;
          rc = launch_igemm<0>(q, 1, st);
        }
        if (rc) return rc;
        set_boxsum_frame(&p, d);
        rc = launch_igemm<2>(p, 1, st, tail, pl.slab_bytes);
      }
      if (rc || add == nullptr) return rc;
      MUNIT_CHECK_ARG(!dx_bf16, "conv2d_dgrad: `add` with a bf16 dx is not supported on the folded path");
      return launch_add_inplace(d, dx, add, st);
    }
    case DG_CIN4: case DG_DIRECT: case DG_CORR: break;
  }
  MUNIT_CHECK_ARG(pl.TH == pl.TW, "conv2d_dgrad: non-square kernels are not supported");
  const bool direct = pl.route == DG_DIRECT && add == nullptr;
  IgemmParams p = dgrad_corr_params(d, pl);
  p.x = dy; p.w = wt; p.bias = nullptr; p.y = direct ? (void*)dx : (void*)g;
  if (pl.route == DG_CIN4) {
    rc = build_cin4(pl.cin4, dy, (long long)d->B * pl.Ho * pl.Wo, wt, d->Cin, pl.TH * pl.TW, tail, st);
    if (rc) return rc;
    p.x = reinterpret_cast<const float*>(tail);
    p.w = reinterpret_cast<const float*>(tail + pl.cin4.x4_bytes);
    set_cin4(&p, pl.cin4);
    rc = launch_igemm<1>(p, 1, st);
  } else {
    rc = launch_igemm<1>(p, pl.ps * pl.ps, st, tail, pl.slab_bytes);
  }
  if (rc || direct) return rc;
  if (!fold_vectorised(d)) return launch_fold_scalar(d, pl, g, add, dx, st);
  return dx_bf16 ? launch_fold<bf16_t>(d, pl, g, add_, dx_, st) : launch_fold<float>(d, pl, g, add_, dx_, st);
}

extern "C" int munit_conv2d_prep_item(const munit_conv_desc* d, int pass, const float* w, float* wp, munit_prep_item* out) {
  int Ho, Wo;
  int rc = munit_conv2d_out_hw(d, &Ho, &Wo);
  if (rc) return rc;
  MUNIT_CHECK_ARG(out != nullptr, "conv2d_prep_item: null item");
  MUNIT_CHECK_ARG(pass == MUNIT_PASS_FWD || pass == MUNIT_PASS_DGRAD, "conv2d_prep_item: pass must be MUNIT_PASS_FWD or _DGRAD");
  munit_prep_item it;
  if (pass == MUNIT_PASS_FWD) {
    it = plan_fwd(d).prep;
  } else {
    const DgradPlan pl = plan_dgrad(d);
    if (pl.rc) return pl.rc;
    it = pl.prep;
  }
  it.w = w; it.wp = wp;
  *out = it;
  return MUNIT_OK;
}

extern "C" size_t munit_conv2d_prepared_weight_bytes(const munit_conv_desc* d, int pass) {
  munit_prep_item it;
  if (munit_conv2d_prep_item(d, pass, nullptr, nullptr, &it) || it.kind == MUNIT_PREP_NONE) return 0;
  return (size_t)prep_elems(it) * (it.bf16 ? 2 : 4);
}

extern "C" int munit_conv2d_prepare_weights(const munit_prep_item* item, munit_stream_t stream) {
  MUNIT_CHECK_ARG(item && item->w && item->wp, "conv2d_prepare_weights: null pointer");
  const bool wino = item->kind == MUNIT_PREP_WINOGRAD || item->kind == MUNIT_PREP_WINOGRAD_DGRAD;
  const bool spw = item->kind == MUNIT_PREP_SUBPIXEL_WINOGRAD || item->kind == MUNIT_PREP_SUBPIXEL_WINOGRAD_DGRAD;
  const bool ws2 = item->kind == MUNIT_PREP_WINOGRAD_S2 || item->kind == MUNIT_PREP_WINOGRAD_S2_DGRAD;
  MUNIT_CHECK_ARG(!ws2 || (item->KH == 4 && item->KW == 4 && !item->bf16 &&
                           (item->kind == MUNIT_PREP_WINOGRAD_S2 ? item->Cin % 8 == 0 && item->Cout % 64 == 0
                                                                 : item->Cout % 8 == 0 && item->Cin % 64 == 0)),
                  "conv2d_prepare_weights: stride-2 Winograd image needs a 4x4 fp32 filter, K %% 8 == 0, N %% 64 == 0");
  MUNIT_CHECK_ARG(!spw || (item->KH == 5 && item->KW == 5 && !item->bf16 &&
                           (item->kind != MUNIT_PREP_SUBPIXEL_WINOGRAD_DGRAD ? item->Cin % 8 == 0 && item->Cout % 64 == 0
                                                                       : item->Cout % 8 == 0 && item->Cin % 64 == 0)),
                  "conv2d_prepare_weights: sub-pixel Winograd image needs a 5x5 fp32 filter, Cin %% 8 == 0, Cout %% 64 == 0");
  MUNIT_CHECK_ARG(item->kind == MUNIT_PREP_DGRAD || item->kind == MUNIT_PREP_SUBPIXEL || wino || spw || ws2 || (item->kind == MUNIT_PREP_CAST && item->bf16),
                  "conv2d_prepare_weights: bad kind %d", item->kind);
  MUNIT_CHECK_ARG(!wino || (item->KH == 3 && item->KW == 3 && !item->bf16 &&
                            (item->kind != MUNIT_PREP_WINOGRAD_DGRAD ? item->Cin % 8 == 0 && item->Cout % 64 == 0
                                                               : item->Cout % 8 == 0 && item->Cin % 64 == 0)),
                  "conv2d_prepare_weights: Winograd image needs a 3x3 fp32 filter, K %% 8 == 0, N %% 64 == 0");
  MUNIT_CHECK_ARG(item->ps >= 1 && item->KH % item->ps == 0 && item->KW % item->ps == 0, "conv2d_prepare_weights: bad phase count");
  MUNIT_CHECK_ARG(item->kind != MUNIT_PREP_SUBPIXEL || (item->KH == 5 && item->KW == 5), "conv2d_prepare_weights: sub-pixel needs 5x5");
  return launch_prep_one(*item, (hipStream_t)stream);
}

extern "C" int munit_conv2d_prepare_weights_batch(const munit_prep_item* items_dev, int n, munit_stream_t stream) {
  MUNIT_CHECK_ARG(items_dev != nullptr && n > 0 && n <= 65535, "conv2d_prepare_weights_batch: bad table (n=%d)", n);
  hipLaunchKernelGGL(prep_weights_kernel<true>, dim3(64, (unsigned)n), dim3(256), 0, (hipStream_t)stream, items_dev, PrepItem{});
  MUNIT_CHECK_LAUNCH("prep_weights_batch");
  return MUNIT_OK;
}

namespace {
const char* igemm_refusal(IgemmForm f) {
  switch (f) {
    case IG_REFUSED_BF16_CIN: return "refused: bf16 storage needs a multiple of 64 input channels";
    case IG_REFUSED_CIN4_FOLD: return "refused: 4-channel taps are not a folded backward-data form";
    case IG_REFUSED_BF16_FOLD: return "refused: bf16-storage folded backward-data exists for the LDS-patch form only";
    case IG_REFUSED_FOLD_UNALIGNED: return "refused: folded backward-data needs Cout % 32 == 0";
    default: return nullptr;
  }
}
}

const char* munit_igemm_kernel_name(const munit_conv_desc* d, int pass) {
  const bool refl = d->pad_mode == MUNIT_PAD_REFLECT;
  const bool x_bf16 = d->in_dtype == MUNIT_DTYPE_BF16, y_bf16 = d->out_dtype == MUNIT_DTYPE_BF16;
  static const char* const head[2][3][2] = {
      {{"conv_head_pk_kernel", "conv_head_pk_kernel<bf16_t>"}, {"conv_head_mfma_kernel", "conv_head_mfma_kernel<bf16_t>"},
       {"conv_patch_fwd_kernel", "conv_patch_fwd_kernel<bf16_t>"}},
      {{"conv_head_pk_kernel (padded-domain correlation)", "conv_head_pk_kernel<bf16_t> (padded-domain correlation)"},
       {"conv_head_mfma_kernel (padded-domain correlation)", "conv_head_mfma_kernel<bf16_t> (padded-domain correlation)"},
       {"conv_patch_fwd_kernel (padded-domain correlation)", "conv_patch_fwd_kernel<bf16_t> (padded-domain correlation)"}}};
  if (pass == MUNIT_PASS_FWD) {
    const FwdPlan fp = plan_fwd(d);
    if (fp.rc) return "invalid";
    const int Ho = fp.Ho, Wo = fp.Wo;
    IgemmParams p = fwd_params(d, Ho, Wo);
    const int bn = igemm_bn(p);
    switch (fp.route) {
      case FWD_SMALL: return y_bf16 ? "refused: the 3-channel image head writes fp32" : head[0][munit_small_fwd_kernel(d->Cin)][x_bf16];
      case FWD_SUBPIXEL_WINO: return "conv_wino_kernel<1, 0> x4 sub-pixel phases + conv_igemm_kernel frame";
      case FWD_SUBPIXEL: {
        const IgemmForm ph = igemm_form(subpixel_phase_params(p, d, Wo), 0);
        set_subpixel_frame(&p, d, Ho, Wo, fp.ring);
        const IgemmForm fr = igemm_form(p, 0);
        if (igemm_refusal(ph)) return igemm_refusal(ph);
        if (igemm_refusal(fr)) return igemm_refusal(fr);
        if (ph != fr) return "invalid";
        if (ph == IG_BF16S) return bn == 64 ? "conv_igemm_kernel<64, true, 0, 4> x4 sub-pixel phases + frame"
                                            : "conv_igemm_kernel<128, true, 0, 4> x4 sub-pixel phases + frame";
        if (ph == IG_CT1) return "conv_igemm_kernel<.., 0, 1> x4 sub-pixel phases + frame";
        if (ph == IG_CT2) return "conv_igemm_kernel<.., 0, 2> x4 sub-pixel phases + frame";
        return "conv_igemm_kernel x4 sub-pixel phases + frame";
      }
      case FWD_WINO: return refl ? "conv_wino_kernel<0, 0>" : "conv_wino_kernel<1, 0>";
      case FWD_WINO_S2: return refl ? "conv_wino_kernel<0, 1>" : "conv_wino_kernel<1, 1>";
      case FWD_CIN4: set_cin4(&p, fp.cin4); break;
      case FWD_IGEMM: break;
    }
    const IgemmForm f = igemm_form(p, 0);
    if (igemm_refusal(f)) return igemm_refusal(f);
    if (fp.route == FWD_CIN4) return y_bf16 ? "conv_igemm_kernel<.., 5> (3 input channels as 4-channel taps, bf16 y)"
                                            : "conv_igemm_kernel<.., 5> (3 input channels as 4-channel taps)";
    if (f == IG_BF16S) return bn == 64 ? "conv_igemm_kernel<64, true, 0, 4>" : "conv_igemm_kernel<128, true, 0, 4>";
    if (f == IG_CT1) return "conv_igemm_kernel<.., 0, 1>";
    if (f == IG_CT2) return "conv_igemm_kernel<.., 0, 2>";
    return "conv_igemm_kernel<fwd>";
  }
  const DgradPlan pl = plan_dgrad(d);
  if (pl.rc) return "invalid";
  if (x_bf16 && d->Cin % 4 != 0) return "refused: bf16 dx needs Cin % 4 == 0";
  switch (pl.route) {
    case DG_WINO_S2: return refl ? "conv_wino_kernel<0, 2>" : "conv_wino_kernel<1, 2>";
    case DG_WINO: return refl ? "conv_wino_kernel<2, 0>" : "conv_wino_kernel<1, 0>";
    case DG_SMALL: return x_bf16 ? "refused: the 3-channel data gradient is fp32" : head[1][munit_small_fwd_kernel(d->Cout)][y_bf16];
    case DG_FOLD_UPWINO: case DG_FOLD_BOXSUM: case DG_FOLD: {
      if (!dgrad_fold_dtypes_ok(d, pl)) return "refused: unsupported dtype combination";
      IgemmParams p = dgrad_fold_params(d, pl);
      const int bn = igemm_bn(p);
      if (pl.route == DG_FOLD_UPWINO) return "conv_wino_kernel<1, 3> + conv_igemm_kernel frame";
      if (pl.route == DG_FOLD_BOXSUM) {
        const IgemmForm in = igemm_form(boxsum_interior_params(p, d), 0);
        set_boxsum_frame(&p, d);
        const IgemmForm fr = igemm_form(p, 2);
        if (igemm_refusal(in)) return igemm_refusal(in);
        if (igemm_refusal(fr)) return igemm_refusal(fr);
        if (in == IG_CT1 && fr == IG_CT1) return "box2x2_kernel + conv_igemm_kernel<.., 1> (box-sum backward-data)";
        if (in == IG_CT2 && fr == IG_CT2) return "box2x2_kernel + conv_igemm_kernel<.., 2> (box-sum backward-data)";
        return "box2x2_kernel + conv_igemm_kernel (box-sum backward-data)";
      }
      const IgemmForm f = igemm_form(p, 2);
      if (igemm_refusal(f)) return igemm_refusal(f);
      if (f == IG_BF16S) return bn == 64 ? "conv_igemm_kernel<64, true, 2, 4> (LDS-patch fold)" : "conv_igemm_kernel<128, true, 2, 4> (LDS-patch fold)";
      if (f == IG_PATCH) return "conv_igemm_kernel<.., 2, 3> (LDS-patch fold)";
      if (f == IG_CT1) return "conv_igemm_kernel<.., 2, 1> (folded gather)";
      if (f == IG_CT2) return "conv_igemm_kernel<.., 2, 2> (folded gather)";
      return "conv_igemm_kernel<.., 2, 0> (folded gather)";
    }
    case DG_CIN4: case DG_DIRECT: case DG_CORR: break;
  }
  if (pl.TH != pl.TW) return "refused: non-square kernels are not supported";
  IgemmParams p = dgrad_corr_params(d, pl);
  const int bn = igemm_bn(p);
  if (pl.route == DG_CIN4) set_cin4(&p, pl.cin4);
  const IgemmForm f = igemm_form(p, 1);
  if (igemm_refusal(f)) return igemm_refusal(f);
  if (pl.route == DG_CIN4) return x_bf16 ? "conv_igemm_kernel<.., 1, 5> (3 output channels as 4-channel taps) + fold_kernel<bf16_t>"
                                         : "conv_igemm_kernel<.., 1, 5> (3 output channels as 4-channel taps)";
  if (pl.route == DG_DIRECT) {
    if (f == IG_BF16S) return bn == 64 ? "conv_igemm_kernel<64, true, 1, 4> direct" : "conv_igemm_kernel<128, true, 1, 4> direct";
    if (f == IG_CT1) return "conv_igemm_kernel<.., 1, 1> direct";
    if (f == IG_CT2) return "conv_igemm_kernel<.., 1, 2> direct";
    return "conv_igemm_kernel<dgrad direct>";
  }
  const bool fold16 = x_bf16 && fold_vectorised(d);
  if (f == IG_BF16S) {
    if (fold16) return bn == 64 ? "conv_igemm_kernel<64, true, 1, 4> phases + fold_kernel<bf16_t>" : "conv_igemm_kernel<128, true, 1, 4> phases + fold_kernel<bf16_t>";
    return bn == 64 ? "conv_igemm_kernel<64, true, 1, 4> phases + fold_kernel" : "conv_igemm_kernel<128, true, 1, 4> phases + fold_kernel";
  }
  if (f == IG_CT1) return fold16 ? "conv_igemm_kernel<.., 1, 1> phases + fold_kernel<bf16_t>" : "conv_igemm_kernel<.., 1, 1> phases + fold_kernel";
  if (f == IG_CT2) return fold16 ? "conv_igemm_kernel<.., 1, 2> phases + fold_kernel<bf16_t>" : "conv_igemm_kernel<.., 1, 2> phases + fold_kernel";
  return fold16 ? "conv_igemm_kernel<.., 1, .> phases + fold_kernel<bf16_t>" : "conv_igemm_kernel<.., 1, .> phases + fold_kernel";
}

double munit_igemm_executed_flops(const munit_conv_desc* d, int pass) {
  int Ho, Wo;
  if (munit_conv2d_out_hw(d, &Ho, &Wo)) return 0.0;
  const double cc = 2.0 * d->Cin * d->Cout;
  if (pass == MUNIT_PASS_FWD) {
    const FwdPlan fp = plan_fwd(d);
    switch (fp.route) {
      case FWD_SUBPIXEL_WINO: return cc * d->B * ((double)(d->H / 2) * (d->W / 2) * 4 * 16 + (2.0 * Wo + 2.0 * (Ho - 2)) * 25);
      case FWD_SUBPIXEL: return cc * d->B * ((double)d->H * d->W * 4 * 9 + (4.0 * Wo + 4.0 * (Ho - 4)) * 25);
      case FWD_WINO: return cc * d->B * (d->H / 2) * (d->W / 2) * 16;
      case FWD_WINO_S2: return 4 * cc * d->B * cdiv(Ho, 3) * cdiv(Wo, 3) * 16;
      case FWD_CIN4: return 2.0 * d->Cout * d->B * Ho * Wo * fp.cin4.kpad;
      default: return cc * d->B * Ho * Wo * d->KH * d->KW;
    }
  }
  const DgradPlan pl = plan_dgrad(d);
  if (pl.rc) return 0.0;
  switch (pl.route) {
    case DG_WINO_S2: return 4 * cc * d->B * cdiv(d->H / 2 + 1, 3) * cdiv(d->W / 2 + 1, 3) * 16;
    case DG_WINO: return cc * d->B * (d->H / 2) * (d->W / 2) * 16;
    case DG_FOLD_UPWINO: return cc * d->B * ((double)((d->H - 4) / 2) * ((d->W - 4) / 2) * 4 * 16 + (4.0 * d->W + 4.0 * (d->H - 4)) * 25);
    case DG_FOLD_BOXSUM: return cc * d->B * ((double)(d->H - 4) * (d->W - 4) + 4.0 * d->W + 4.0 * (d->H - 4)) * d->KH * d->KW;
    case DG_FOLD: return cc * d->B * d->H * d->W * d->KH * d->KW;
    case DG_DIRECT: return cc * d->B * Ho * Wo * d->KH * d->KW;
    case DG_CIN4: return 2.0 * d->Cin * d->B * (double)(pl.Ho + pl.TH - 1) * (pl.Wo + pl.TW - 1) * pl.cin4.kpad;
    case DG_SMALL: case DG_CORR: return cc * d->B * (double)(pl.Ho + pl.TH - 1) * (pl.Wo + pl.TW - 1) * pl.TH * pl.TW * pl.ps * pl.ps;
  }
  return 0.0;
}

namespace {
munit_conv_desc linear_desc(int B, int K, int N, int act, float slope, int compute) {
  munit_conv_desc d{};
  d.B = B; d.H = 1; d.W = 1; d.Cin = K; d.Cout = N; d.KH = 1; d.KW = 1; d.stride = 1; d.pad = 0;
  d.pad_mode = MUNIT_PAD_ZERO; d.upsample = 0; d.act = act; d.slope = slope; d.compute = compute;
  return d;
}
}

extern "C" size_t munit_linear_workspace_bytes(int B, int K, int N) {
  const munit_conv_desc d = linear_desc(B, K, N, MUNIT_ACT_NONE, 0.f, MUNIT_COMPUTE_F32);
  return std::max(std::max(munit_conv2d_fwd_workspace_bytes(&d), munit_conv2d_dgrad_workspace_bytes(&d)),
                  munit_conv2d_wgrad_workspace_bytes(&d));
}

extern "C" int munit_linear_fwd(const float* x, const float* w, const float* bias, float* y, int B, int K, int N, int act,
                                float slope, void* ws, size_t ws_bytes, munit_stream_t stream) {
  const munit_conv_desc d = linear_desc(B, K, N, act, slope, MUNIT_COMPUTE_F32);
  return munit_conv2d_fwd(&d, x, w, bias, y, ws, ws_bytes, stream);
}

extern "C" int munit_linear_bwd(const float* x, const float* w, const float* dy, float* dx, float* dw, float* db, int B,
                                int K, int N, float beta, void* ws, size_t ws_bytes, munit_stream_t stream) {
  const munit_conv_desc d = linear_desc(B, K, N, MUNIT_ACT_NONE, 0.f, MUNIT_COMPUTE_F32);
  const size_t need = std::max(dx != nullptr ? munit_conv2d_dgrad_workspace_bytes(&d) : 0,
                               dw != nullptr ? munit_conv2d_wgrad_workspace_bytes(&d) : 0);
  if (ws_bytes < need) {
    munit_set_error("linear_bwd: workspace %zu < %zu", ws_bytes, need);
    return MUNIT_ERR_WORKSPACE;
  }
  if (dx != nullptr) {
    const int rc = munit_conv2d_dgrad(&d, dy, w, nullptr, dx, ws, ws_bytes, stream);
    if (rc) return rc;
  }
  if (dw != nullptr) return munit_conv2d_wgrad(&d, x, dy, dw, db, beta, ws, ws_bytes, stream);
  return MUNIT_OK;
}
```

### munit_amd/csrc/conv_wgrad.hip

```cpp
#include "common.h"
#include "wino.h"
#include <cstdlib>
#include <type_traits>

namespace {

struct WgradParams {
  const void* x;
  const void* dy;
  float* slab;
  float* bias_slab;
  int B, H, W, Cin, Hu, Wu, ups;
  int Ho, Wo, Cout;
  int KH, KW, stride, pad, reflect;
  int Ktot, M;
  int pix_per_split;
  long long dy_sb, dy_sh;
  int dy_sw;
  long long dy_off;
  int frame;
  unsigned x_bytes, dy_bytes;
  int ct;
  int x_bf16, dy_bf16;
};

__device__ const float munit_wgrad_zero16[4] = {0.f, 0.f, 0.f, 0.f};
constexpr int DMA_MAX_HW = 1024;

__device__ inline void decode_pixel(int m, int Ho, int Wo, int frame, int& b, int& oh, int& ow) {
  if (!frame) {
    const int HoWo = Ho * Wo;
    b = m / HoWo;
    const int rem = m - b * HoWo;
    oh = rem / Wo;
    ow = rem - oh * Wo;
  } else {
    const int F = frame, F2 = 2 * frame;
    const int nb = F2 * Wo + F2 * (Ho - F2);
    b = m / nb;
    int r = m - b * nb;
    if (r < F2 * Wo) {
      const int q = r / Wo;
      ow = r - q * Wo;
      oh = q < F ? q : Ho - F2 + q;
    } else {
      r -= F2 * Wo;
      const int rr = r / F2, q = r - rr * F2;
      oh = F + rr;
      ow = q < F ? q : Wo - F2 + q;
    }
  }
}

constexpr int WP = 32;

constexpr int WTHR = 512;

typedef float f32x2 __attribute__((ext_vector_type(2)));
typedef unsigned u32x4 __attribute__((ext_vector_type(4)));
constexpr unsigned OOB = 0x80000000u;

template <int NTILE>
struct Frag;
template <>
struct Frag<4> {
  f32x4 v;
  __device__ inline void load(const float* row, int col, int ) { v = *reinterpret_cast<const f32x4*>(row + col); }
  __device__ inline float at(int t) const { return v[t]; }
};
template <>
struct Frag<2> {
  f32x2 v;
  __device__ inline void load(const float* row, int col, int swz) { v = *reinterpret_cast<const f32x2*>(row + (col ^ swz)); }
  __device__ inline float at(int t) const { return v[t]; }
};

typedef __bf16 bf16x4 __attribute__((ext_vector_type(4)));
typedef __bf16 bf16x8 __attribute__((ext_vector_type(8)));
typedef short s16x4 __attribute__((ext_vector_type(4)));
typedef short s16x8 __attribute__((ext_vector_type(8)));

__device__ inline int img_off(int row, int ch) { return 256 * row + 16 * (ch ^ (((row & 3) << 2) | ((row >> 2) & 3))); }

template <int BC, bool ALIGNED, bool FAST, int CT = 0, bool XB = false, bool DYB = false>
__global__ __launch_bounds__(WTHR, 4) void conv_wgrad_kernel(WgradParams p) {
  constexpr bool DMA = CT == 3;
  static_assert(!(XB || DYB) || (FAST && !DMA), "bf16 tensors: FAST register loader only");
  constexpr bool BF16 = CT == 1 || CT == 2;
  static_assert(!DMA || (FAST && ALIGNED), "direct-to-LDS loads: FAST variants only");
  constexpr int NPL = CT == 2 ? 3 : 1;
  static_assert(!BF16 || FAST, "the bf16 variants use the FAST loader");
  constexpr int WKT = BC == 128 ? 128 : 256;
  constexpr int WC = BC / 2;
  constexpr int WK = WKT / 4;
  constexpr int MT = WC / 16;
  constexpr int NT = WK / 16;
  constexpr int XQ = WKT / 4;
  constexpr int XRPT = WTHR / XQ;
  constexpr int XROWS = WP / XRPT;
  constexpr int DQ = BC / 4;
  constexpr int DRPT = WTHR / DQ;
  constexpr int DROWS = WP / DRPT;
  constexpr int SWZ_D = MT == 2 ? 32 : 0;
  constexpr int SWZ_X = NT == 2 ? 32 : 0;
  static_assert(XRPT % 2 == 0 && DRPT % 2 == 0, "row parity of a loader thread must not change between passes");
  __shared__ __attribute__((aligned(16))) float smem[2 * WP * BC + 2 * WP * WKT + (DMA ? DMA_MAX_HW : 0)];
  float* const Ds = smem;
  float* const Xs = smem + 2 * WP * BC;
  int* const offtab = reinterpret_cast<int*>(smem + 2 * WP * BC + 2 * WP * WKT);

  const int tid = threadIdx.x;
  const int lane = tid & 63;
  const int wave = tid >> 6;
  const int wm = wave >> 2, wn = wave & 3;
  const int kc0 = blockIdx.x * WKT;
  const int co0 = blockIdx.y * BC;
  const int split = blockIdx.z;
  const int m_begin = split * p.pix_per_split;
  const int m_end = min(p.M, m_begin + p.pix_per_split);

  const int xq = tid % XQ;
  const int xr0 = tid / XQ;
  int ekh[4], ekw[4], eci[4];
  bool eok[4];
  if constexpr (ALIGNED) {
    int k = kc0 + (DMA ? (xq ^ (((xr0 & 1) ? SWZ_X : 0) >> 2)) : xq) * 4;
    eok[0] = k < p.Ktot;
    int kk = eok[0] ? k : 0;
    int tap = kk / p.Cin;
    eci[0] = kk - tap * p.Cin;
    ekh[0] = tap / p.KW;
    ekw[0] = tap - ekh[0] * p.KW;
  } else {
#pragma unroll
    for (int e = 0; e < 4; ++e) {
      int k = kc0 + xq * 4 + e;
      eok[e] = k < p.Ktot;
      int kk = eok[e] ? k : 0;
      int tap = kk / p.Cin;
      eci[e] = kk - tap * p.Cin;
      ekh[e] = tap / p.KW;
      ekw[e] = tap - ekh[e] * p.KW;
    }
  }
  const int dq = tid % DQ;
  const int dr0 = tid / DQ;
  const int dq_g = DMA ? (dq ^ (((dr0 & 1) ? SWZ_D : 0) >> 2)) : dq;
  const int xs_col = (xq * 4) ^ ((xr0 & 1) ? SWZ_X : 0);
  const int ds_col = (dq * 4) ^ ((dr0 & 1) ? SWZ_D : 0);

  f32x4 rx[XROWS], rd[DROWS];

  int px_oh[FAST ? XROWS : 1], px_ow[FAST ? XROWS : 1], px_b[FAST ? XROWS : 1];
  int dp_oh[FAST ? DROWS : 1], dp_ow[FAST ? DROWS : 1], dp_b[FAST ? DROWS : 1];
  if constexpr (FAST) {
#pragma unroll
    for (int i = 0; i < XROWS; ++i) {
      int m = m_begin + xr0 + XRPT * i;
      decode_pixel(m < p.M ? m : 0, p.Ho, p.Wo, 0, px_b[i], px_oh[i], px_ow[i]);
    }
#pragma unroll
    for (int i = 0; i < DROWS; ++i) {
      int m = m_begin + dr0 + DRPT * i;
      decode_pixel(m < p.M ? m : 0, p.Ho, p.Wo, 0, dp_b[i], dp_oh[i], dp_ow[i]);
    }
  }
  const int hw = p.Ho * p.Wo;
  const int step_b = WP / hw;
  const int step_h = (WP - step_b * hw) / p.Wo;
  const int step_w = WP - step_b * hw - step_h * p.Wo;
  int dp_off[DROWS];
  const int d_step = step_b * (int)p.dy_sb + step_h * (int)p.dy_sh + step_w * p.dy_sw;
  const int d_carry_w = (int)p.dy_sh - p.Wo * p.dy_sw;
  const int d_carry_h = (int)p.dy_sb - p.Ho * (int)p.dy_sh;
  if constexpr (FAST) {
#pragma unroll
    for (int i = 0; i < DROWS; ++i)
      dp_off[i] = dp_b[i] * (int)p.dy_sb + dp_oh[i] * (int)p.dy_sh + dp_ow[i] * p.dy_sw + (int)p.dy_off + co0 + dq_g * 4;
  }
  const bool d_col_ok = co0 + dq_g * 4 < p.Cout;

  auto load_tiles = [&](int mbase) {
    if constexpr (FAST) {
      const __amdgpu_buffer_rsrc_t xres = __builtin_amdgcn_make_buffer_rsrc(const_cast<void*>(p.x), 0, p.x_bytes, 0x00020000);
      const __amdgpu_buffer_rsrc_t dres = __builtin_amdgcn_make_buffer_rsrc(const_cast<void*>(p.dy), 0, p.dy_bytes, 0x00020000);
      auto fetch4 = [&](const __amdgpu_buffer_rsrc_t& res, bool ok, unsigned off, auto is_bf16) -> f32x4 {
        if constexpr (decltype(is_bf16)::value) {
          typedef unsigned u32x2 __attribute__((ext_vector_type(2)));
          const u32x2 raw = __builtin_amdgcn_raw_buffer_load_b64(res, ok ? off * 2u : OOB, 0, 0);
          const bf16v4 h = __builtin_bit_cast(bf16v4, raw);
          return f32x4{(float)h[0], (float)h[1], (float)h[2], (float)h[3]};
        } else {
          return __builtin_bit_cast(f32x4, __builtin_amdgcn_raw_buffer_load_b128(res, ok ? off * 4u : OOB, 0, 0));
        }
      };
#pragma unroll
      for (int i = 0; i < XROWS; ++i) {
        const int m = mbase + xr0 + XRPT * i;
        const int ih = src_coord(__mul24(px_oh[i], p.stride) - p.pad + ekh[0], p.Hu, p.ups, p.reflect);
        const int iw = src_coord(__mul24(px_ow[i], p.stride) - p.pad + ekw[0], p.Wu, p.ups, p.reflect);
        const bool ok = m < m_end && eok[0] && ih >= 0 && iw >= 0;
        const int pix = __mul24(__mul24(px_b[i], p.H) + ih, p.W) + iw;
        const unsigned off = (unsigned)(__mul24(pix, p.Cin) + eci[0]);
        rx[i] = fetch4(xres, ok, off, std::integral_constant<bool, XB>{});
        int ow = px_ow[i] + step_w;
        const bool cw = ow >= p.Wo;
        ow -= cw ? p.Wo : 0;
        int oh = px_oh[i] + step_h + (cw ? 1 : 0);
        const bool ch = oh >= p.Ho;
        oh -= ch ? p.Ho : 0;
        px_ow[i] = ow;
        px_oh[i] = oh;
        px_b[i] += step_b + (ch ? 1 : 0);
      }
#pragma unroll
      for (int i = 0; i < DROWS; ++i) {
        const int m = mbase + dr0 + DRPT * i;
        const bool ok = m < m_end && d_col_ok;
        rd[i] = fetch4(dres, ok, (unsigned)dp_off[i], std::integral_constant<bool, DYB>{});
        int ow = dp_ow[i] + step_w;
        const bool cw = ow >= p.Wo;
        ow -= cw ? p.Wo : 0;
        int oh = dp_oh[i] + step_h + (cw ? 1 : 0);
        const bool ch = oh >= p.Ho;
        oh -= ch ? p.Ho : 0;
        dp_ow[i] = ow;
        dp_oh[i] = oh;
        dp_off[i] += d_step + (cw ? d_carry_w : 0) + (ch ? d_carry_h : 0);
      }
      return;
    }
#pragma unroll
    for (int i = 0; i < XROWS; ++i) {
      const int m = mbase + xr0 + XRPT * i;
      const bool mok = m < m_end;
      int b, oh, ow;
      decode_pixel(mok ? m : 0, p.Ho, p.Wo, p.frame, b, oh, ow);
      const long long base = (long long)b * p.H * p.W;
      int ih0 = oh * p.stride - p.pad, iw0 = ow * p.stride - p.pad;
      f32x4 v = {0.f, 0.f, 0.f, 0.f};
      if constexpr (ALIGNED) {
        int ih = src_coord(ih0 + ekh[0], p.Hu, p.ups, p.reflect);
        int iw = src_coord(iw0 + ekw[0], p.Wu, p.ups, p.reflect);
        if (mok && eok[0] && ih >= 0 && iw >= 0)
          v = *reinterpret_cast<const f32x4*>(reinterpret_cast<const float*>(p.x) + (base + (long long)ih * p.W + iw) * p.Cin + eci[0]);
      } else {
#pragma unroll
        for (int e = 0; e < 4; ++e) {
          int ih = src_coord(ih0 + ekh[e], p.Hu, p.ups, p.reflect);
          int iw = src_coord(iw0 + ekw[e], p.Wu, p.ups, p.reflect);
          float s = 0.f;
          if (mok && eok[e] && ih >= 0 && iw >= 0) s = reinterpret_cast<const float*>(p.x)[(base + (long long)ih * p.W + iw) * p.Cin + eci[e]];
          v[e] = s;
        }
      }
      rx[i] = v;
    }
#pragma unroll
    for (int i = 0; i < DROWS; ++i) {
      const int m = mbase + dr0 + DRPT * i;
      const bool mok = m < m_end;
      int b, oh, ow;
      decode_pixel(mok ? m : 0, p.Ho, p.Wo, p.frame, b, oh, ow);
      const float* ptr = reinterpret_cast<const float*>(p.dy) + (long long)b * p.dy_sb + (long long)oh * p.dy_sh +
                         (long long)ow * p.dy_sw + p.dy_off + co0 + dq * 4;
      const int co = co0 + dq * 4;
      f32x4 v = {0.f, 0.f, 0.f, 0.f};
      if (mok) {
        if ((p.Cout & 3) == 0) {
          if (co < p.Cout) v = *reinterpret_cast<const f32x4*>(ptr);
        } else {
#pragma unroll
          for (int e = 0; e < 4; ++e)
            if (co + e < p.Cout) v[e] = ptr[e];
        }
      }
      rd[i] = v;
    }
  };
  constexpr int OFF_NONE = -(1 << 30);
  if constexpr (DMA) {
    for (int t = tid; t < p.Ho + p.Wo; t += WTHR) {
      if (t < p.Ho) {
        const int ih = src_coord(t * p.stride - p.pad + ekh[0], p.Hu, p.ups, p.reflect);
        offtab[t] = ih >= 0 ? ih * p.W * p.Cin : OFF_NONE;
      } else {
        const int iw = src_coord((t - p.Ho) * p.stride - p.pad + ekw[0], p.Wu, p.ups, p.reflect);
        offtab[t] = iw >= 0 ? iw * p.Cin : OFF_NONE;
      }
    }
    __syncthreads();
  }
  const int hwc = p.H * p.W * p.Cin;
  auto dma_tiles = [&](int mbase, int buf) {
    if constexpr (DMA) {
      const int w = __builtin_amdgcn_readfirstlane(wave);
#pragma unroll
      for (int i = 0; i < XROWS; ++i) {
        const int m = mbase + xr0 + XRPT * i;
        const int off = px_b[i] * hwc + offtab[px_oh[i]] + offtab[p.Ho + px_ow[i]] + eci[0];
        const bool ok = m < m_end && eok[0] && off >= 0;
        const float* g = ok ? reinterpret_cast<const float*>(p.x) + off : munit_wgrad_zero16;
        float* l = Xs + buf * (WP * WKT) + (XRPT * i) * WKT + w * 256;
        __builtin_amdgcn_global_load_lds((const __attribute__((address_space(1))) void*)g,
                                         (__attribute__((address_space(3))) void*)l, 16, 0, 0);
        int ow = px_ow[i] + step_w;
        const bool cw = ow >= p.Wo;
        ow -= cw ? p.Wo : 0;
        int oh = px_oh[i] + step_h + (cw ? 1 : 0);
        const bool ch = oh >= p.Ho;
        oh -= ch ? p.Ho : 0;
        px_ow[i] = ow;
        px_oh[i] = oh;
        px_b[i] += step_b + (ch ? 1 : 0);
      }
#pragma unroll
      for (int i = 0; i < DROWS; ++i) {
        const int m = mbase + dr0 + DRPT * i;
        const bool ok = m < m_end && d_col_ok;
        const float* g = ok ? reinterpret_cast<const float*>(p.dy) + dp_off[i] : munit_wgrad_zero16;
        float* l = Ds + buf * (WP * BC) + (DRPT * i) * BC + w * 256;
        __builtin_amdgcn_global_load_lds((const __attribute__((address_space(1))) void*)g,
                                         (__attribute__((address_space(3))) void*)l, 16, 0, 0);
        int ow = dp_ow[i] + step_w;
        const bool cw = ow >= p.Wo;
        ow -= cw ? p.Wo : 0;
        int oh = dp_oh[i] + step_h + (cw ? 1 : 0);
        const bool ch = oh >= p.Ho;
        oh -= ch ? p.Ho : 0;
        dp_ow[i] = ow;
        dp_oh[i] = oh;
        dp_off[i] += d_step + (cw ? d_carry_w : 0) + (ch ? d_carry_h : 0);
      }
    }
  };
  constexpr int NXI = WKT / 128;
  static_assert((CT == 2 ? 3 : 2) * (1 + NXI) * 8192 <= (int)sizeof(float) * (2 * WP * BC + 2 * WP * WKT), "bf16 images must fit the LDS allocation");
  char* const img_base = reinterpret_cast<char*>(smem);
  auto store_tiles = [&](int buf) {
    if constexpr (BF16) {
      char* ib = img_base + buf * (NPL * (1 + NXI) * 8192);
      auto put = [&](char* dst, f32x4 v) {
#pragma unroll
        for (int pl = 0; pl < NPL; ++pl) {
          bf16x4 h;
#pragma unroll
          for (int e = 0; e < 4; ++e) h[e] = (__bf16)v[e];
          *reinterpret_cast<bf16x4*>(dst + pl * ((1 + NXI) * 8192)) = h;
          if (pl + 1 < NPL) {
#pragma unroll
            for (int e = 0; e < 4; ++e) v[e] -= (float)h[e];
          }
        }
      };
#pragma unroll
      for (int i = 0; i < XROWS; ++i) {
        const int quad = xq & 31;
        put(ib + (1 + (xq >> 5)) * 8192 + img_off(xr0 + XRPT * i, quad >> 1) + 8 * (quad & 1), rx[i]);
      }
#pragma unroll
      for (int i = 0; i < DROWS; ++i) put(ib + img_off(dr0 + DRPT * i, dq >> 1) + 8 * (dq & 1), rd[i]);
      return;
    }
    float* Xd = Xs + buf * (WP * WKT);
    float* Dd = Ds + buf * (WP * BC);
#pragma unroll
    for (int i = 0; i < XROWS; ++i) *reinterpret_cast<f32x4*>(&Xd[(xr0 + XRPT * i) * WKT + xs_col]) = rx[i];
#pragma unroll
    for (int i = 0; i < DROWS; ++i) *reinterpret_cast<f32x4*>(&Dd[(dr0 + DRPT * i) * BC + ds_col]) = rd[i];
  };

  f32x4 acc[MT][NT];
#pragma unroll
  for (int a = 0; a < MT; ++a)
#pragma unroll
    for (int t = 0; t < NT; ++t)
#pragma unroll
      for (int r = 0; r < 4; ++r) acc[a][t][r] = 0.f;
  float bsum = 0.f;
  const bool do_bias = p.bias_slab != nullptr && blockIdx.x == 0;

  const int fj = lane & 15;
  const int fg = lane >> 4;
  const int a_col = wm * WC + MT * fj;
  const int b_col = wn * WK + NT * fj;
  const int a_swz = (fg & 1) ? SWZ_D : 0;
  const int b_swz = (fg & 1) ? SWZ_X : 0;
  constexpr int GB = (FAST || BC == 128) ? 4 : 2;
  auto tr_frag = [&](const char* im, int c0) -> bf16x8 {
    const int q = fj >> 2, pp = lane & 3;
    const int ch = (c0 >> 3) + (pp >> 1);
    const s16x4 lo = __builtin_amdgcn_ds_read_tr16_b64_v4i16(
        (s16x4 __attribute__((address_space(3)))*)(im + img_off(8 * fg + q, ch) + 8 * (pp & 1)));
    const s16x4 hi = __builtin_amdgcn_ds_read_tr16_b64_v4i16(
        (s16x4 __attribute__((address_space(3)))*)(im + img_off(8 * fg + 4 + q, ch) + 8 * (pp & 1)));
    const s16x8 v = __builtin_shufflevector(lo, hi, 0, 1, 2, 3, 4, 5, 6, 7);
    return __builtin_bit_cast(bf16x8, v);
  };
  auto compute_half = [&](int buf, int p0) {
    if constexpr (BF16) {
      const char* ib = img_base + buf * (NPL * (1 + NXI) * 8192);
      constexpr int PLB = (1 + NXI) * 8192;
      const int h = p0 ? 1 : 0;
      if constexpr (NT <= MT) {
        bf16x8 hb[NPL][NT];
#pragma unroll
        for (int pl = 0; pl < NPL; ++pl)
#pragma unroll
          for (int u = 0; u < NT; ++u) {
            const int col = wn * WK + 16 * u;
            hb[pl][u] = tr_frag(ib + pl * PLB + (1 + (col >> 7)) * 8192, col & 127);
          }
#pragma unroll
        for (int t = h * (MT / 2); t < (h + 1) * (MT / 2); ++t) {
          bf16x8 ha[NPL];
#pragma unroll
          for (int pl = 0; pl < NPL; ++pl) ha[pl] = tr_frag(ib + pl * PLB, wm * WC + 16 * t);
#pragma unroll
          for (int sum = NPL - 1; sum >= 0; --sum)
#pragma unroll
            for (int i = 0; i <= sum; ++i)
#pragma unroll
              for (int u = 0; u < NT; ++u)
                acc[t][u] = __builtin_amdgcn_mfma_f32_16x16x32_bf16(ha[i], hb[sum - i][u], acc[t][u], 0, 0, 0);
        }
      } else {
        bf16x8 ha[NPL][MT];
#pragma unroll
        for (int pl = 0; pl < NPL; ++pl)
#pragma unroll
          for (int t = 0; t < MT; ++t) ha[pl][t] = tr_frag(ib + pl * PLB, wm * WC + 16 * t);
#pragma unroll
        for (int u = h * (NT / 2); u < (h + 1) * (NT / 2); ++u) {
          const int col = wn * WK + 16 * u;
          bf16x8 hb[NPL];
#pragma unroll
          for (int pl = 0; pl < NPL; ++pl) hb[pl] = tr_frag(ib + pl * PLB + (1 + (col >> 7)) * 8192, col & 127);
#pragma unroll
          for (int sum = NPL - 1; sum >= 0; --sum)
#pragma unroll
            for (int i = 0; i <= sum; ++i)
#pragma unroll
              for (int t = 0; t < MT; ++t)
                acc[t][u] = __builtin_amdgcn_mfma_f32_16x16x32_bf16(ha[i][t], hb[sum - i], acc[t][u], 0, 0, 0);
        }
      }
      return;
    }
    const float* Dc = Ds + buf * (WP * BC);
    const float* Xc = Xs + buf * (WP * WKT);
#pragma unroll
    for (int s0 = 0; s0 < 4; s0 += GB) {
      Frag<MT> a[GB];
      Frag<NT> b[GB];
#pragma unroll
      for (int s = 0; s < GB; ++s) {
        a[s].load(Dc + (p0 + 4 * (s0 + s) + fg) * BC, a_col, a_swz);
        b[s].load(Xc + (p0 + 4 * (s0 + s) + fg) * WKT, b_col, b_swz);
      }
#pragma unroll
      for (int s = 0; s < GB; ++s)
#pragma unroll
        for (int t = 0; t < MT; ++t)
#pragma unroll
          for (int u = 0; u < NT; ++u)
            acc[t][u] = __builtin_amdgcn_mfma_f32_16x16x4f32(a[s].at(t), b[s].at(u), acc[t][u], 0, 0, 0);
      if constexpr (GB != 4) __builtin_amdgcn_sched_barrier(0);
    }
  };

  if constexpr (DMA) {
    if (m_begin < m_end) dma_tiles(m_begin, 0);
    asm volatile("s_waitcnt vmcnt(0)" ::: "memory");
    __syncthreads();
    int cur = 0;
    for (int mb = m_begin; mb < m_end; mb += WP) {
      if (mb + WP < m_end) dma_tiles(mb + WP, cur ^ 1);
      compute_half(cur, 0);
      compute_half(cur, WP / 2);
      if (do_bias && tid < BC) {
        const float* Dc = Ds + cur * (WP * BC);
#pragma unroll 8
        for (int r = 0; r < WP; ++r) bsum += Dc[r * BC + (tid ^ ((r & 1) ? SWZ_D : 0))];
      }
      asm volatile("s_waitcnt vmcnt(0)" ::: "memory");
      __syncthreads();
      cur ^= 1;
    }
  } else if constexpr (CT == 2) {
    if (m_begin < m_end) load_tiles(m_begin);
    for (int mb = m_begin; mb < m_end; mb += WP) {
      __syncthreads();
      store_tiles(0);
      if (mb + WP < m_end) load_tiles(mb + WP);
      __syncthreads();
      compute_half(0, 0);
      compute_half(0, WP / 2);
      if (do_bias && tid < BC) {
        const char* ib = img_base;
#pragma unroll 8
        for (int r = 0; r < WP; ++r) {
          float v = 0.f;
#pragma unroll
          for (int pl = NPL - 1; pl >= 0; --pl)
            v += (float)*reinterpret_cast<const __bf16*>(ib + pl * ((1 + NXI) * 8192) + img_off(r, tid >> 3) + 2 * (tid & 7));
          bsum += v;
        }
      }
    }
  } else {
    if (m_begin < m_end) {
      load_tiles(m_begin);
      store_tiles(0);
    }
    __syncthreads();
    if (m_begin + WP < m_end) load_tiles(m_begin + WP);
    int cur = 0;
    for (int mb = m_begin; mb < m_end; mb += WP) {
      compute_half(cur, 0);
      if (mb + WP < m_end) {
        store_tiles(cur ^ 1);
        if (mb + 2 * WP < m_end) load_tiles(mb + 2 * WP);
      }
      compute_half(cur, WP / 2);
      if (do_bias && tid < BC) {
        if constexpr (BF16) {
          const char* ib = img_base + cur * (NPL * (1 + NXI) * 8192);
  #pragma unroll 8
          for (int r = 0; r < WP; ++r) {
            float v = 0.f;
  #pragma unroll
            for (int pl = NPL - 1; pl >= 0; --pl)
              v += (float)*reinterpret_cast<const __bf16*>(ib + pl * ((1 + NXI) * 8192) + img_off(r, tid >> 3) + 2 * (tid & 7));
            bsum += v;
          }
        } else {
          const float* Dc = Ds + cur * (WP * BC);
  #pragma unroll 8
          for (int r = 0; r < WP; ++r) bsum += Dc[r * BC + (tid ^ ((r & 1) ? SWZ_D : 0))];
        }
      }
      __syncthreads();
      cur ^= 1;
    }
  }

  float* out = p.slab + (long long)split * p.Cout * p.Ktot;
  if constexpr (BF16) {
#pragma unroll
    for (int t = 0; t < MT; ++t)
#pragma unroll
      for (int r = 0; r < 4; ++r) {
        const int co = co0 + wm * WC + 16 * t + 4 * fg + r;
#pragma unroll
        for (int u = 0; u < NT; ++u) {
          const int k = kc0 + wn * WK + 16 * u + fj;
          if (co < p.Cout && k < p.Ktot) out[(long long)co * p.Ktot + k] = acc[t][u][r];
        }
      }
    if (do_bias && tid < BC && co0 + tid < p.Cout) p.bias_slab[(long long)split * p.Cout + co0 + tid] = bsum;
    return;
  }
  const int k_base = kc0 + wn * WK + NT * fj;
#pragma unroll
  for (int t = 0; t < MT; ++t) {
#pragma unroll
    for (int r = 0; r < 4; ++r) {
      const int co = co0 + wm * WC + MT * (4 * fg + r) + t;
      if (co >= p.Cout) continue;
      float* dst = out + (long long)co * p.Ktot + k_base;
      if (ALIGNED && k_base + NT <= p.Ktot) {
        if constexpr (NT == 2) {
          f32x2 v = {acc[t][0][r], acc[t][1][r]};
          *reinterpret_cast<f32x2*>(dst) = v;
        } else {
          f32x4 v = {acc[t][0][r], acc[t][1][r], acc[t][2][r], acc[t][3][r]};
          *reinterpret_cast<f32x4*>(dst) = v;
        }
      } else {
#pragma unroll
        for (int u = 0; u < NT; ++u)
          if (k_base + u < p.Ktot) dst[u] = acc[t][u][r];
      }
    }
  }
  if (do_bias && tid < BC && co0 + tid < p.Cout) p.bias_slab[(long long)split * p.Cout + co0 + tid] = bsum;
}

constexpr int BS_WP = 64;
__device__ const float munit_wgrad_zero16b[4] = {0.f, 0.f, 0.f, 0.f};
#ifdef WGB_STAMP
__device__ long long g_wgb_stamps[8 * 8 * 4];
#define WGB(i) do { const long long t_ = __builtin_amdgcn_s_memtime(); wgb_acc[i] += t_ - wgb_last; wgb_last = t_; } while (0)
#else
#define WGB(i) do { } while (0)
#endif

template <int TC>
__global__ __launch_bounds__(WTHR, TC == 1 ? 4 : 2) void conv_wgrad_bf16s_kernel(WgradParams p) {
  constexpr int BC = 128 * TC, WKT = 128 * TC, WC = 64 * TC, WK = 32 * TC, MT = 4 * TC, NT = 2 * TC;
  constexpr int IMG = 8192;
  constexpr int STAGE = 4 * TC * IMG;
  __shared__ __attribute__((aligned(16))) char smem[2 * STAGE + 4 * DMA_MAX_HW];
  int* const offtab = reinterpret_cast<int*>(smem + 2 * STAGE);

  const int tid = threadIdx.x, lane = tid & 63, wave = tid >> 6;
  const int wm = wave >> 2, wn = wave & 3;
  int blk = blockIdx.x + gridDim.x * (blockIdx.y + gridDim.y * blockIdx.z);
  {
    const int nb = gridDim.x * gridDim.y * gridDim.z, q = nb >> 3, rr = nb & 7, xcd = blk & 7, idx = blk >> 3;
    blk = (xcd < rr ? xcd * (q + 1) : rr * (q + 1) + (xcd - rr) * q) + idx;
  }
  const int bx = blk % gridDim.x, by = (blk / gridDim.x) % gridDim.y, split = blk / (gridDim.x * gridDim.y);
  const int kc0 = bx * WKT, co0 = by * BC;
  const int m_begin = split * p.pix_per_split;
  const int m_end = min(p.M, m_begin + p.pix_per_split);
  const bf16_t* __restrict__ xg = reinterpret_cast<const bf16_t*>(p.x);
  const bf16_t* __restrict__ dyg = reinterpret_cast<const bf16_t*>(p.dy);

  const int tap = kc0 / p.Cin, ci0 = kc0 - tap * p.Cin;
  const int kh = tap / p.KW, kw = tap - kh * p.KW;
  constexpr int OFF_NONE = -(1 << 30);
  for (int t = tid; t < p.Ho + p.Wo; t += WTHR) {
    if (t < p.Ho) {
      const int ih = src_coord(t * p.stride - p.pad + kh, p.Hu, p.ups, p.reflect);
      offtab[t] = ih >= 0 ? ih * p.W * p.Cin : OFF_NONE;
    } else {
      const int iw = src_coord((t - p.Ho) * p.stride - p.pad + kw, p.Wu, p.ups, p.reflect);
      offtab[t] = iw >= 0 ? iw * p.Cin : OFF_NONE;
    }
  }

  const int r = tid >> 4, pos = tid & 15;
  const int chunk = pos ^ (((r & 3) << 2) | ((r >> 2) & 3));
  const int x_col = ci0 + 8 * chunk;
  const int d_col = co0 + 8 * chunk;
  int px_b[2], px_oh[2], px_ow[2], dp_off[2];
#pragma unroll
  for (int i = 0; i < 2; ++i) {
    const int m = m_begin + 32 * i + r;
    decode_pixel(m < p.M ? m : 0, p.Ho, p.Wo, p.frame, px_b[i], px_oh[i], px_ow[i]);
    dp_off[i] = px_b[i] * (int)p.dy_sb + px_oh[i] * (int)p.dy_sh + px_ow[i] * p.dy_sw + (int)p.dy_off + d_col;
  }
  const int hw = p.Ho * p.Wo;
  const int step_b = BS_WP / hw;
  const int step_h = (BS_WP - step_b * hw) / p.Wo;
  const int step_w = BS_WP - step_b * hw - step_h * p.Wo;
  const int d_step = step_b * (int)p.dy_sb + step_h * (int)p.dy_sh + step_w * p.dy_sw;
  const int d_carry_w = (int)p.dy_sh - p.Wo * p.dy_sw;
  const int d_carry_h = (int)p.dy_sb - p.Ho * (int)p.dy_sh;
  const int hwc = p.H * p.W * p.Cin;
  __syncthreads();

  auto dma = [&](int mbase, int stage) {
    const int w = __builtin_amdgcn_readfirstlane(wave);
    char* sb = smem + stage * STAGE;
#pragma unroll
    for (int i = 0; i < 2; ++i) {
      const int m = mbase + 32 * i + r;
      const bool mok = m < m_end;
      const int xo = px_b[i] * hwc + offtab[px_oh[i]] + offtab[p.Ho + px_ow[i]] + x_col;
#pragma unroll
      for (int c = 0; c < TC; ++c) {
        const void* gx = (mok && xo >= 0) ? (const void*)(xg + xo + 128 * c) : (const void*)munit_wgrad_zero16b;
        const void* gd = (mok && d_col + 128 * c < p.Cout) ? (const void*)(dyg + dp_off[i] + 128 * c) : (const void*)munit_wgrad_zero16b;
        __builtin_amdgcn_global_load_lds((const __attribute__((address_space(1))) void*)gd,
                                         (__attribute__((address_space(3))) void*)(sb + (i * TC + c) * IMG + 1024 * w), 16, 0, 0);
        __builtin_amdgcn_global_load_lds((const __attribute__((address_space(1))) void*)gx,
                                         (__attribute__((address_space(3))) void*)(sb + ((2 + i) * TC + c) * IMG + 1024 * w), 16, 0, 0);
      }
      if (p.frame) {
        const int mn = m + BS_WP;
        decode_pixel(mn < p.M ? mn : 0, p.Ho, p.Wo, p.frame, px_b[i], px_oh[i], px_ow[i]);
        dp_off[i] = px_b[i] * (int)p.dy_sb + px_oh[i] * (int)p.dy_sh + px_ow[i] * p.dy_sw + (int)p.dy_off + d_col;
        continue;
      }
      int ow = px_ow[i] + step_w;
      const bool cw = ow >= p.Wo;
      ow -= cw ? p.Wo : 0;
      int oh = px_oh[i] + step_h + (cw ? 1 : 0);
      const bool ch = oh >= p.Ho;
      oh -= ch ? p.Ho : 0;
      px_ow[i] = ow;
      px_oh[i] = oh;
      px_b[i] += step_b + (ch ? 1 : 0);
      dp_off[i] += d_step + (cw ? d_carry_w : 0) + (ch ? d_carry_h : 0);
    }
  };

  f32x4 acc[MT][NT];
#pragma unroll
  for (int a = 0; a < MT; ++a)
#pragma unroll
    for (int t = 0; t < NT; ++t)
#pragma unroll
      for (int e = 0; e < 4; ++e) acc[a][t][e] = 0.f;
  float bsum = 0.f;
  const bool do_bias = p.bias_slab != nullptr && bx == 0;
  const int fj = lane & 15, fg = lane >> 4;
  auto tr_frag = [&](const char* im0, int c0) -> bf16x8 {
    const int q = fj >> 2, pp = lane & 3;
    const char* im = im0 + (c0 >> 7) * IMG;
    const int ch = ((c0 & 127) >> 3) + (pp >> 1);
    const s16x4 lo = __builtin_amdgcn_ds_read_tr16_b64_v4i16(
        (s16x4 __attribute__((address_space(3)))*)(im + img_off(8 * fg + q, ch) + 8 * (pp & 1)));
    const s16x4 hi = __builtin_amdgcn_ds_read_tr16_b64_v4i16(
        (s16x4 __attribute__((address_space(3)))*)(im + img_off(8 * fg + 4 + q, ch) + 8 * (pp & 1)));
    const s16x8 v = __builtin_shufflevector(lo, hi, 0, 1, 2, 3, 4, 5, 6, 7);
    return __builtin_bit_cast(bf16x8, v);
  };

  if (m_begin < m_end) dma(m_begin, 0);
  asm volatile("s_waitcnt vmcnt(0)" ::: "memory");
  __syncthreads();
#ifdef WGB_STAMP
  long long wgb_acc[4] = {0, 0, 0, 0};
  long long wgb_last = __builtin_amdgcn_s_memtime();
#endif
  int cur = 0;
  for (int mb = m_begin; mb < m_end; mb += BS_WP) {
    if (mb + BS_WP < m_end) dma(mb + BS_WP, cur ^ 1);
    WGB(0);
    const char* sb = smem + cur * STAGE;
#pragma unroll
    for (int h = 0; h < 2; ++h) {
      bf16x8 hb[NT];
#pragma unroll
      for (int u = 0; u < NT; ++u) hb[u] = tr_frag(sb + (2 + h) * TC * IMG, wn * WK + 16 * u);
#pragma unroll
      for (int t = 0; t < MT; ++t) {
        const bf16x8 ha = tr_frag(sb + h * TC * IMG, wm * WC + 16 * t);
#pragma unroll
        for (int u = 0; u < NT; ++u)
          acc[t][u] = __builtin_amdgcn_mfma_f32_16x16x32_bf16(ha, hb[u], acc[t][u], 0, 0, 0);
      }
    }
    if (do_bias && tid < BC) {
#pragma unroll 8
      for (int rr = 0; rr < BS_WP; ++rr)
        bsum += (float)*reinterpret_cast<const bf16_t*>(sb + ((rr >> 5) * TC + (tid >> 7)) * IMG + img_off(rr & 31, (tid & 127) >> 3) +
                                                       2 * (tid & 7));
    }
    WGB(1);
    asm volatile("s_waitcnt vmcnt(0)" ::: "memory");
    WGB(2);
    __syncthreads();
    WGB(3);
    cur ^= 1;
  }
#ifdef WGB_STAMP
  if (blk < 8 && lane == 0)
    for (int i = 0; i < 4; ++i) g_wgb_stamps[(blk * 8 + wave) * 4 + i] = wgb_acc[i];
#endif

  float* out = p.slab + (long long)split * p.Cout * p.Ktot;
#pragma unroll
  for (int t = 0; t < MT; ++t)
#pragma unroll
    for (int e = 0; e < 4; ++e) {
      const int co = co0 + wm * WC + 16 * t + 4 * fg + e;
#pragma unroll
      for (int u = 0; u < NT; ++u) {
        const int k = kc0 + wn * WK + 16 * u + fj;
        if (co < p.Cout && k < p.Ktot) out[(long long)co * p.Ktot + k] = acc[t][u][e];
      }
    }
  if (do_bias && tid < BC && co0 + tid < p.Cout) p.bias_slab[(long long)split * p.Cout + co0 + tid] = bsum;
}

__global__ void slab_reduce_kernel(const float* __restrict__ slab, float* __restrict__ dw, long long n,
                                   const float* __restrict__ bias_slab, float* __restrict__ db, int nb,
                                   int nsplit, float beta, float beta_b) {
  const long long total = n + (db != nullptr ? nb : 0);
  for (long long i = (long long)blockIdx.x * blockDim.x + threadIdx.x; i < total;
       i += (long long)gridDim.x * blockDim.x) {
    float s = 0.f;
    if (i < n) {
      for (int k = 0; k < nsplit; ++k) s += slab[(long long)k * n + i];
      dw[i] = (beta != 0.f ? beta * dw[i] : 0.f) + s;
    } else {
      const long long j = i - n;
      for (int k = 0; k < nsplit; ++k) s += bias_slab[(long long)k * nb + j];
      db[j] = (beta_b != 0.f ? beta_b * db[j] : 0.f) + s;
    }
  }
}

__global__ __launch_bounds__(1024) void slab_reduce_wide_kernel(const float* __restrict__ slab, float* __restrict__ dw,
                                                                long long n, const float* __restrict__ bias_slab,
                                                                float* __restrict__ db, int nb, int nsplit, float beta,
                                                                float beta_b) {
  __shared__ float red[16][64];
  const int il = threadIdx.x & 63, kg = threadIdx.x >> 6;
  const long long total = n + (db != nullptr ? nb : 0);
  const long long i = (long long)blockIdx.x * 64 + il;
  float s = 0.f;
  if (i < total) {
    if (i < n) {
      for (int k = kg; k < nsplit; k += 16) s += slab[(long long)k * n + i];
    } else {
      const long long j = i - n;
      for (int k = kg; k < nsplit; k += 16) s += bias_slab[(long long)k * nb + j];
    }
  }
  red[kg][il] = s;
  __syncthreads();
  if (kg == 0 && i < total) {
    float t = 0.f;
#pragma unroll
    for (int g = 0; g < 16; ++g) t += red[g][il];
    if (i < n) dw[i] = (beta != 0.f ? beta * dw[i] : 0.f) + t;
    else db[i - n] = (beta_b != 0.f ? beta_b * db[i - n] : 0.f) + t;
  }
}

int wgrad_blocks_per_cu(int bc, bool aligned) {
  static int cache[2][2] = {{0, 0}, {0, 0}};
  int& c = cache[bc == 128][aligned];
  if (c == 0) {
    int n = 0;
    hipError_t e;
    if (bc == 128) {
      if (aligned) e = hipOccupancyMaxActiveBlocksPerMultiprocessor(&n, conv_wgrad_kernel<128, true, true>, WTHR, 0);
      else e = hipOccupancyMaxActiveBlocksPerMultiprocessor(&n, conv_wgrad_kernel<128, false, false>, WTHR, 0);
    } else {
      if (aligned) e = hipOccupancyMaxActiveBlocksPerMultiprocessor(&n, conv_wgrad_kernel<64, true, true>, WTHR, 0);
      else e = hipOccupancyMaxActiveBlocksPerMultiprocessor(&n, conv_wgrad_kernel<64, false, false>, WTHR, 0);
    }
    if (e != hipSuccess) (void)hipGetLastError();
    c = (e == hipSuccess && n > 0) ? std::min(n, 8) : 2;
  }
  return c;
}

__global__ void upw_scatter_kernel(const float* __restrict__ dwc, float* __restrict__ dw, int Cout, int Cin) {
  const long long total = (long long)Cout * 25 * Cin;
  const long long per_phase = (long long)Cout * 9 * Cin;
  for (long long i = (long long)blockIdx.x * blockDim.x + threadIdx.x; i < total;
       i += (long long)gridDim.x * blockDim.x) {
    long long r = i;
    const int ci = (int)(r % Cin); r /= Cin;
    const int kw = (int)(r % 5); r /= 5;
    const int kh = (int)(r % 5); r /= 5;
    const int co = (int)r;
    float s = 0.f;
#pragma unroll
    for (int a = 0; a < 2; ++a) {
      const int dh = a == 0 ? (kh >> 1) : ((kh + 1) >> 1);
#pragma unroll
      for (int b = 0; b < 2; ++b) {
        const int dw_ = b == 0 ? (kw >> 1) : ((kw + 1) >> 1);
        s += dwc[(a * 2 + b) * per_phase + (((long long)co * 3 + dh) * 3 + dw_) * Cin + ci];
      }
    }
    dw[i] += s;
  }
}

__global__ void pad3to4_kernel(const float* __restrict__ x, f32x4* __restrict__ x4, long long npix) {
  for (long long i = (long long)blockIdx.x * blockDim.x + threadIdx.x; i < npix; i += (long long)gridDim.x * blockDim.x) {
    const f32x4 v = {x[3 * i], x[3 * i + 1], x[3 * i + 2], 0.f};
    x4[i] = v;
  }
}
__global__ void compact4to3_kernel(const float* __restrict__ dw4, float* __restrict__ dw, long long n3, float beta) {
  for (long long i = (long long)blockIdx.x * blockDim.x + threadIdx.x; i < n3; i += (long long)gridDim.x * blockDim.x) {
    const long long t = i / 3;
    const int c = (int)(i - 3 * t);
    dw[i] = (beta != 0.f ? beta * dw[i] : 0.f) + dw4[4 * t + c];
  }
}

struct WgradPlan {
  int bc, k_tiles, c_tiles, nsplit, pix_per_split;
  size_t slab_bytes, bias_bytes;
};

void plan_launch(int M, int Ktot, int Cout, bool aligned, WgradPlan* pl, bool big256 = false) {
  pl->bc = big256 ? 256 : (Cout <= 64 ? 64 : 128);
  pl->k_tiles = cdiv(Ktot, pl->bc == 128 ? 128 : 256);
  pl->c_tiles = cdiv(Cout, pl->bc);
  const int tiles = pl->k_tiles * pl->c_tiles;
  const int slots = big256 ? 256 : 256 * wgrad_blocks_per_cu(pl->bc, aligned);
  int want = std::max(1, slots / tiles);
  int max_by_pix = std::max(1, M / 128);
  int ns = std::max(1, std::min(std::min(want, max_by_pix), 512));
  int pps = cdiv(M, ns);
  pps = (pps + WP - 1) / WP * WP;
  ns = cdiv(M, pps);
  pl->nsplit = ns;
  pl->pix_per_split = pps;
  pl->slab_bytes = align_up((size_t)ns * Cout * Ktot * sizeof(float), 256);
  pl->bias_bytes = align_up((size_t)ns * Cout * sizeof(float), 256);
}

enum WgradForm {
  WG_REFUSED_BF16,
  WG_REFUSED_BF16_X,
  WG_BF16S_128,
  WG_BF16S_256,
  WG_REG_BF16,
  WG_REG_BF16_DY,
  WG_DMA,
  WG_CT1, WG_CT2,
  WG_FAST, WG_ALIGNED, WG_GENERIC
};
struct WgradChoice {
  WgradForm form;
  bool fast;
  long long x_bytes, dy_bytes;
};
WgradChoice wgrad_form(const WgradParams& p, const WgradPlan& pl, bool aligned) {
  WgradChoice c{};
  c.x_bytes = (long long)p.B * p.H * p.W * p.Cin * (p.x_bf16 ? 2 : 4);
  c.dy_bytes = (long long)p.B * p.dy_sb * (p.dy_bf16 ? 2 : 4);
  const bool any_bf16 = p.x_bf16 || p.dy_bf16;
  const bool fast_any = aligned && (p.Cout % 4 == 0) && c.x_bytes < (1ll << 31) && c.dy_bytes < (1ll << 31) &&
                        (long long)p.B * p.H * p.W < (1ll << 23) && (any_bf16 || !MUNIT_ENV_FLAG("MUNIT_DEBUG_NO_FAST_WGRAD"));
  const bool fast = c.fast = fast_any && !p.frame;
  if (any_bf16) {
    const bool dma_ok = p.x_bf16 && p.dy_bf16 && p.Cin % 128 == 0 && p.Cout % 8 == 0 && p.Ho + p.Wo <= DMA_MAX_HW;
    if (!fast && !(fast_any && dma_ok)) c.form = WG_REFUSED_BF16;
    else if (dma_ok && !MUNIT_ENV_FLAG("MUNIT_DEBUG_NO_WGRAD_DMA")) c.form = pl.bc == 256 ? WG_BF16S_256 : WG_BF16S_128;
    else if (p.x_bf16 && p.dy_bf16) c.form = WG_REG_BF16;
    else if (p.dy_bf16) c.form = WG_REG_BF16_DY;
    else c.form = WG_REFUSED_BF16_X;
  } else if (fast && p.ct == 0 && pl.bc == 128 && p.Cin % 128 == 0 && p.Ho + p.Wo <= DMA_MAX_HW &&
             !MUNIT_ENV_FLAG("MUNIT_DEBUG_NO_WGRAD_DMA")) {
    c.form = WG_DMA;
  } else if (fast && p.ct == 1) {
    c.form = WG_CT1;
  } else if (fast && p.ct == 2) {
    c.form = WG_CT2;
  } else {
    c.form = fast ? WG_FAST : aligned ? WG_ALIGNED : WG_GENERIC;
  }
  return c;
}

#define WGRAD_LAUNCH(...)                                                                                         \
  do {                                                                                                            \
    if (pl.bc == 64) hipLaunchKernelGGL((conv_wgrad_kernel<64, __VA_ARGS__>), grid, dim3(WTHR), 0, st, p);        \
    else hipLaunchKernelGGL((conv_wgrad_kernel<128, __VA_ARGS__>), grid, dim3(WTHR), 0, st, p);                   \
  } while (0)

int run_wgrad(WgradParams p, const WgradPlan& pl, bool aligned, float* dw, float* db, float beta, float beta_b,
              void* ws, hipStream_t st) {
  p.slab = reinterpret_cast<float*>(ws);
  p.bias_slab = db ? reinterpret_cast<float*>(reinterpret_cast<char*>(ws) + pl.slab_bytes) : nullptr;
  p.pix_per_split = pl.pix_per_split;
  dim3 grid((unsigned)pl.k_tiles, (unsigned)pl.c_tiles, (unsigned)pl.nsplit);
  const WgradChoice ch = wgrad_form(p, pl, aligned);
  p.x_bytes = ch.fast ? (unsigned)ch.x_bytes : 0u;
  p.dy_bytes = ch.fast ? (unsigned)ch.dy_bytes : 0u;
  switch (ch.form) {
    case WG_REFUSED_BF16:
      munit_set_error("conv2d_wgrad: bf16 tensors need Cin %% 4 == 0, Cout %% 4 == 0, tensors below 2 GiB and B*H*W < 2^23");
      return MUNIT_ERR_ARG;
    case WG_REFUSED_BF16_X:
      munit_set_error("conv2d_wgrad: bf16 x with fp32 dy exists for the 3-channel image head only");
      return MUNIT_ERR_ARG;
    case WG_BF16S_128:
    case WG_BF16S_256: {
      int pps = (cdiv(p.M, pl.nsplit) + BS_WP - 1) / BS_WP * BS_WP;
      p.pix_per_split = pps;
      const int ns = cdiv(p.M, pps);
      if (ch.form == WG_BF16S_256) {
        dim3 g2((unsigned)(p.Ktot / 256), (unsigned)(p.Cout / 256), (unsigned)ns);
        hipLaunchKernelGGL(conv_wgrad_bf16s_kernel<2>, g2, dim3(WTHR), 0, st, p);
      } else {
        dim3 g2((unsigned)cdiv(p.Ktot, 128), (unsigned)cdiv(p.Cout, 128), (unsigned)ns);
        hipLaunchKernelGGL(conv_wgrad_bf16s_kernel<1>, g2, dim3(WTHR), 0, st, p);
      }
      MUNIT_CHECK_LAUNCH("conv_wgrad_bf16s");
      const long long n = (long long)p.Cout * p.Ktot;
      const int blocks = (int)std::min<long long>((n + p.Cout + 255) / 256, 4096);
      hipLaunchKernelGGL(slab_reduce_kernel, dim3(blocks), dim3(256), 0, st, p.slab, dw, n, p.bias_slab, db, p.Cout,
                         ns, beta, beta_b);
      MUNIT_CHECK_LAUNCH("slab_reduce");
      return MUNIT_OK;
    }
    case WG_REG_BF16: WGRAD_LAUNCH(true, true, 1, true, true); break;
    case WG_REG_BF16_DY: WGRAD_LAUNCH(true, true, 0, false, true); break;
    case WG_DMA: hipLaunchKernelGGL((conv_wgrad_kernel<128, true, true, 3>), grid, dim3(WTHR), 0, st, p); break;
    case WG_CT1: WGRAD_LAUNCH(true, true, 1); break;
    case WG_CT2: WGRAD_LAUNCH(true, true, 2); break;
    case WG_FAST: WGRAD_LAUNCH(true, true); break;
    case WG_ALIGNED: WGRAD_LAUNCH(true, false); break;
    case WG_GENERIC: WGRAD_LAUNCH(false, false); break;
  }
  MUNIT_CHECK_LAUNCH("conv_wgrad");
  const long long n = (long long)p.Cout * p.Ktot;
  if (pl.nsplit >= 32 && n + p.Cout <= 64 * 2048) {
    hipLaunchKernelGGL(slab_reduce_wide_kernel, dim3(cdiv(n + p.Cout, 64)), dim3(1024), 0, st, p.slab, dw, n,
                       p.bias_slab, db, p.Cout, pl.nsplit, beta, beta_b);
    MUNIT_CHECK_LAUNCH("slab_reduce_wide");
    return MUNIT_OK;
  }
  const int blocks = (int)std::min<long long>((n + p.Cout + 255) / 256, 4096);
  hipLaunchKernelGGL(slab_reduce_kernel, dim3(blocks), dim3(256), 0, st, p.slab, dw, n, p.bias_slab, db, p.Cout,
                     pl.nsplit, beta, beta_b);
  MUNIT_CHECK_LAUNCH("slab_reduce");
  return MUNIT_OK;
}

bool cin3_padded_ok(const munit_conv_desc* d) {
  return d->Cin == 3 && d->Cout % 4 == 0 && d->upsample == 0 && !MUNIT_ENV_FLAG("MUNIT_DEBUG_NO_CIN3_PAD");
}

bool bf16s_big_tile(const munit_conv_desc* d, int Ho, int Wo) {
  if (MUNIT_ENV_FLAG("MUNIT_DEBUG_NO_WGRAD_BIG_TILE") || MUNIT_ENV_FLAG("MUNIT_DEBUG_NO_WGRAD_DMA")) return false;
  if (d->in_dtype != MUNIT_DTYPE_BF16 || d->out_dtype != MUNIT_DTYPE_BF16) return false;
  if (d->Cin % 256 != 0 || d->Cout % 256 != 0 || Ho + Wo > DMA_MAX_HW) return false;
  const long long tiles = (long long)(d->KH * d->KW * d->Cin / 256) * (d->Cout / 256);
  const long long M = (long long)d->B * Ho * Wo;
  return tiles <= 256 && M * tiles >= 256ll * 1024;
}

bool subpixel_wgrad_ok(const munit_conv_desc* d) {
  const bool f32 = d->in_dtype == MUNIT_DTYPE_F32 && d->out_dtype == MUNIT_DTYPE_F32;
  const bool b16 = d->in_dtype == MUNIT_DTYPE_BF16 && d->out_dtype == MUNIT_DTYPE_BF16 && d->Cin % 128 == 0 &&
                   d->Cout % 8 == 0 && 2 * (d->H + d->W) <= DMA_MAX_HW && !MUNIT_ENV_FLAG("MUNIT_DEBUG_NO_WGRAD_DMA");
  return (f32 || b16) && d->upsample == 1 && d->KH == 5 && d->KW == 5 && d->pad == 2 && d->stride == 1 &&
         d->pad_mode == MUNIT_PAD_REFLECT && d->Cin % 4 == 0 && d->H >= 3 && d->W >= 3 &&
         !MUNIT_ENV_FLAG("MUNIT_DEBUG_NO_SUBPIXEL");
}

struct SubpixelPlan {
  WgradPlan phase, frame;
  size_t dwc_bytes, slab_bytes;
  bool wino;
  int ring;
};
void plan_subpixel(const munit_conv_desc* d, SubpixelPlan* sp) {
  const bool aligned = d->Cin % 4 == 0;
  plan_launch(d->B * (d->H - 2) * (d->W - 2), 9 * d->Cin, d->Cout, aligned, &sp->phase);
  const int Ho = 2 * d->H, Wo = 2 * d->W;
  sp->wino = d->compute == MUNIT_COMPUTE_F32 && d->in_dtype == MUNIT_DTYPE_F32 && d->out_dtype == MUNIT_DTYPE_F32 && d->H >= 4 &&
             d->W >= 4 && munit_wino_wgrad_ok(d->B, d->H, d->W, d->Cin, d->Cout) &&
             (long long)d->B * 4 * d->H * d->W * d->Cout < (1ll << 29);
  sp->ring = sp->wino ? 1 : 2;
  plan_launch(d->B * (2 * sp->ring * Wo + 2 * sp->ring * (Ho - 2 * sp->ring)), 25 * d->Cin, d->Cout, aligned, &sp->frame);
  sp->dwc_bytes = align_up((size_t)4 * d->Cout * 9 * d->Cin * sizeof(float), 256);
  sp->slab_bytes = std::max(sp->phase.slab_bytes + sp->phase.bias_bytes, sp->frame.slab_bytes + sp->frame.bias_bytes);
  if (sp->wino)
    sp->slab_bytes = std::max(sp->slab_bytes, munit_wino_wgrad_workspace((long long)d->B * (d->H / 2) * (d->W / 2), d->Cin, d->Cout, 4));
}

bool wino_wgrad_layer(const munit_conv_desc* d) {
  return d->compute == MUNIT_COMPUTE_F32 && d->in_dtype == MUNIT_DTYPE_F32 && d->out_dtype == MUNIT_DTYPE_F32 && d->KH == 3 &&
         d->KW == 3 && d->stride == 1 && d->pad == 1 && d->upsample == 0 && munit_wino_wgrad_ok(d->B, d->H, d->W, d->Cin, d->Cout);
}
long long s2_tiles(const munit_conv_desc* d) { return (long long)d->B * cdiv(d->H / 2, 3) * cdiv(d->W / 2, 3); }
bool wino_s2_wgrad_layer(const munit_conv_desc* d) {
  return d->compute == MUNIT_COMPUTE_F32 && d->in_dtype == MUNIT_DTYPE_F32 && d->out_dtype == MUNIT_DTYPE_F32 && d->KH == 4 &&
         d->KW == 4 && d->stride == 2 && d->pad == 1 && d->upsample == 0 && d->H >= 4 && d->W >= 4 &&
         munit_wino_wgrad_ok(d->B, d->H, d->W, d->Cin, d->Cout) && !MUNIT_ENV_FLAG("MUNIT_DEBUG_NO_WINOGRAD_S2") &&
         s2_tiles(d) >= (getenv("MUNIT_WINO_S2_MIN_BLOCKS") ? 1 : 512);
}

enum WgradRoute { WGR_WINO_S2, WGR_WINO, WGR_SMALL, WGR_SUBPIXEL, WGR_CIN3, WGR_GENERIC };
struct WgradRoutePlan {
  int rc;
  WgradRoute route;
  int Ho, Wo;
  bool aligned;
  SubpixelPlan sp;
  WgradPlan gen;
  size_t x4_bytes, dw4_bytes;
  size_t ws_bytes;
};
WgradRoutePlan plan_wgrad(const munit_conv_desc* d) {
  WgradRoutePlan pl{};
  pl.rc = munit_conv2d_out_hw(d, &pl.Ho, &pl.Wo);
  if (pl.rc) return pl;
  pl.route = wino_s2_wgrad_layer(d) ? WGR_WINO_S2 : wino_wgrad_layer(d) ? WGR_WINO : munit_small_wgrad_ok(d) ? WGR_SMALL
             : subpixel_wgrad_ok(d) ? WGR_SUBPIXEL : cin3_padded_ok(d) ? WGR_CIN3 : WGR_GENERIC;
  pl.aligned = pl.route == WGR_CIN3 || d->Cin % 4 == 0;
  switch (pl.route) {
    case WGR_WINO_S2: pl.ws_bytes = munit_wino_wgrad_workspace(s2_tiles(d), d->Cin, d->Cout, 4); break;
    case WGR_WINO: pl.ws_bytes = munit_wino_wgrad_workspace((long long)d->B * (d->H / 2) * (d->W / 2), d->Cin, d->Cout, 1); break;
    case WGR_SMALL: pl.ws_bytes = munit_small_wgrad_workspace(d, pl.Ho); break;
    case WGR_SUBPIXEL:
      plan_subpixel(d, &pl.sp);
      pl.ws_bytes = pl.sp.dwc_bytes + pl.sp.slab_bytes;
      break;
    case WGR_CIN3:
      plan_launch(d->B * pl.Ho * pl.Wo, d->KH * d->KW * 4, d->Cout, true, &pl.gen);
      pl.x4_bytes = align_up((size_t)d->B * d->H * d->W * 4 * sizeof(float), 256);
      pl.dw4_bytes = align_up((size_t)d->Cout * d->KH * d->KW * 4 * sizeof(float), 256);
      pl.ws_bytes = pl.x4_bytes + pl.dw4_bytes + pl.gen.slab_bytes + pl.gen.bias_bytes;
      break;
    case WGR_GENERIC:
      plan_launch(d->B * pl.Ho * pl.Wo, d->KH * d->KW * d->Cin, d->Cout, pl.aligned, &pl.gen, bf16s_big_tile(d, pl.Ho, pl.Wo));
      pl.ws_bytes = pl.gen.slab_bytes + pl.gen.bias_bytes;
      break;
  }
  return pl;
}

WgradParams wgrad_params(const munit_conv_desc* d, int Ho, int Wo) {
  WgradParams p{};
  p.x_bf16 = d->in_dtype == MUNIT_DTYPE_BF16; p.dy_bf16 = d->out_dtype == MUNIT_DTYPE_BF16;
  p.B = d->B; p.H = d->H; p.W = d->W; p.Cin = d->Cin;
  p.ups = d->upsample; p.Hu = d->H << p.ups; p.Wu = d->W << p.ups;
  p.Ho = Ho; p.Wo = Wo; p.Cout = d->Cout;
  p.KH = d->KH; p.KW = d->KW; p.stride = d->stride; p.pad = d->pad;
  p.reflect = d->pad_mode == MUNIT_PAD_REFLECT;
  p.ct = d->compute;
  p.Ktot = d->KH * d->KW * d->Cin; p.M = d->B * Ho * Wo;
  p.dy_sw = d->Cout; p.dy_sh = (long long)Wo * d->Cout; p.dy_sb = (long long)Ho * Wo * d->Cout; p.dy_off = 0;
  return p;
}
WinoWgradParams wino_wgrad_params(const munit_conv_desc* d, int Ho, int Wo, WgradRoute route, const void* x, const void* dy) {
  WinoWgradParams q{};
  q.x = reinterpret_cast<const float*>(x); q.dy = reinterpret_cast<const float*>(dy);
  q.x_bytes = (unsigned)((size_t)d->B * d->H * d->W * d->Cin * 4); q.dy_bytes = (unsigned)((size_t)d->B * Ho * Wo * d->Cout * 4);
  q.dy_sw = d->Cout; q.dy_sh = (long long)Wo * d->Cout; q.dy_sb = (long long)Ho * Wo * d->Cout;
  q.B = d->B; q.H = d->H; q.W = d->W; q.Cin = d->Cin; q.Cout = d->Cout;
  q.reflect = d->pad_mode == MUNIT_PAD_REFLECT;
  q.th = d->H / 2; q.tw = d->W / 2; q.phases = 4;
  if (route == WGR_WINO_S2) {
    q.th = cdiv(Ho, 3); q.tw = cdiv(Wo, 3);
    q.s2 = 1; q.Ho = Ho; q.Wo = Wo;
  } else if (route == WGR_WINO) {
    q.xo = -1; q.phases = 1;
  } else {
    q.dy_sw *= 2; q.dy_sh *= 2; q.dy_prow = (long long)Wo * d->Cout; q.dy_pcol = d->Cout;
    q.reflect = 2; q.xo = -1; q.ring_mask = 1;
  }
  return q;
}
WgradParams subpixel_frame_params(const WgradParams& p, const munit_conv_desc* d, const SubpixelPlan& sp, int Ho, int Wo) {
  WgradParams f = p;
  f.frame = sp.ring;
  f.M = d->B * (2 * sp.ring * Wo + 2 * sp.ring * (Ho - 2 * sp.ring));
  return f;
}
WgradParams subpixel_phase_params(const WgradParams& p, const munit_conv_desc* d, int Wo, int ph) {
  const int a = ph >> 1, b = ph & 1;
  WgradParams q = p;
  q.ups = 0; q.Hu = d->H; q.Wu = d->W;
  q.Ho = d->H - 2; q.Wo = d->W - 2;
  q.KH = 3; q.KW = 3; q.pad = 0; q.reflect = 0;
  q.Ktot = 9 * d->Cin; q.M = d->B * q.Ho * q.Wo;
  q.dy_sw = 2 * d->Cout; q.dy_sh = (long long)2 * Wo * d->Cout;
  q.dy_off = ((long long)(2 + a) * Wo + 2 + b) * d->Cout;
  return q;
}
WgradParams cin3_params(const WgradParams& p, const munit_conv_desc* d) {
  WgradParams q = p;
  q.Cin = 4; q.Ktot = d->KH * d->KW * 4; q.x_bf16 = 0;
  q.ct = 0;
  return q;
}
const char* wgrad_refusal(WgradForm f) {
  if (f == WG_REFUSED_BF16) return "refused: bf16 tensors need Cin % 4 == 0, Cout % 4 == 0, tensors below 2 GiB and B*H*W < 2^23";
  if (f == WG_REFUSED_BF16_X) return "refused: bf16 x with fp32 dy exists for the 3-channel image head only";
  return nullptr;
}
}

extern "C" size_t munit_conv2d_wgrad_workspace_bytes(const munit_conv_desc* d) {
  const WgradRoutePlan pl = plan_wgrad(d);
  return pl.rc ? 0 : pl.ws_bytes;
}

extern "C" double munit_conv2d_executed_flops(const munit_conv_desc* d, int pass) {
  if (pass == MUNIT_PASS_FWD || pass == MUNIT_PASS_DGRAD) return munit_igemm_executed_flops(d, pass);
  if (pass != MUNIT_PASS_WGRAD) return 0.0;
  const WgradRoutePlan pl = plan_wgrad(d);
  if (pl.rc) return 0.0;
  const int Ho = pl.Ho, Wo = pl.Wo;
  const double cc = 2.0 * d->Cin * d->Cout;
  switch (pl.route) {
    case WGR_WINO: return cc * d->B * (d->H / 2) * (d->W / 2) * 16;
    case WGR_WINO_S2: return 4 * cc * (double)s2_tiles(d) * 16;
    case WGR_SUBPIXEL:
      if (pl.sp.wino) return cc * d->B * ((double)d->H * d->W * 4 * 4 + (2.0 * Wo + 2.0 * (Ho - 2)) * 25);
      return cc * d->B * ((double)(d->H - 2) * (d->W - 2) * 4 * 9 + (4.0 * Wo + 4.0 * (Ho - 4)) * 25);
    case WGR_CIN3: return 2.0 * 4 * d->Cout * d->B * Ho * Wo * d->KH * d->KW;
    default: return cc * d->B * Ho * Wo * d->KH * d->KW;
  }
}

extern "C" const char* munit_conv2d_kernel_name(const munit_conv_desc* d, int pass) {
  if (pass == MUNIT_PASS_FWD || pass == MUNIT_PASS_DGRAD) return munit_igemm_kernel_name(d, pass);
  if (pass != MUNIT_PASS_WGRAD) return "invalid";
  const WgradRoutePlan pl = plan_wgrad(d);
  if (pl.rc) return "invalid";
  const int Ho = pl.Ho, Wo = pl.Wo;
  const bool x_bf16 = d->in_dtype == MUNIT_DTYPE_BF16, dy_bf16 = d->out_dtype == MUNIT_DTYPE_BF16;
  const WgradParams p = wgrad_params(d, Ho, Wo);
  switch (pl.route) {
    case WGR_WINO_S2:
    case WGR_WINO: {
      const WinoWgradVariant v = munit_wino_wgrad_variant(wino_wgrad_params(d, Ho, Wo, pl.route, nullptr, nullptr));
      if (!v.s2) return v.fast ? "conv_wino_wgrad_kernel<false, true, false> + wino_wgrad_reduce_kernel"
                               : "conv_wino_wgrad_kernel<false, false, false> + wino_wgrad_reduce_kernel";
      return v.fast ? "conv_wino_wgrad_kernel<true, true, false> + wino_wgrad_reduce_kernel"
                    : v.ring ? "conv_wino_wgrad_kernel<true, false, true> + wino_wgrad_reduce_kernel"
                             : "conv_wino_wgrad_kernel<true, false, false> + wino_wgrad_reduce_kernel";
    }
    case WGR_SMALL:
      if (dy_bf16) return "refused: the 3-channel image head has an fp32 dy";
      if (!munit_small_wgrad_pk()) return x_bf16 ? "conv_lanes_wgrad_kernel<bf16_t>" : "conv_lanes_wgrad_kernel";
      return x_bf16 ? "conv_lanes_wgrad_pk_kernel<bf16_t>" : "conv_lanes_wgrad_pk_kernel";
    case WGR_SUBPIXEL: {
      if (pl.sp.wino) return "conv_wino_wgrad_kernel<false, ., true> x4 sub-pixel phases + frame + reduce";
      const WgradForm fr = wgrad_form(subpixel_frame_params(p, d, pl.sp, Ho, Wo), pl.sp.frame, pl.aligned).form;
      const WgradForm ph = wgrad_form(subpixel_phase_params(p, d, Wo, 0), pl.sp.phase, pl.aligned).form;
      if (wgrad_refusal(fr)) return wgrad_refusal(fr);
      if (wgrad_refusal(ph)) return wgrad_refusal(ph);
      if (ph == WG_BF16S_128 && fr == WG_BF16S_128) return "conv_wgrad_bf16s_kernel<1> x4 sub-pixel phases + frame";
      if (x_bf16 || dy_bf16) return "invalid";
      if (ph == WG_CT1) return "conv_wgrad_kernel<.., 1> x4 sub-pixel phases + fp32 frame";
      if (ph == WG_CT2) return "conv_wgrad_kernel<.., 2> x4 sub-pixel phases + fp32 frame";
      return "conv_wgrad_kernel x4 sub-pixel phases + frame";
    }
    case WGR_CIN3:
      if (x_bf16) return "refused: 3-channel inputs are fp32";
      break;
    case WGR_GENERIC: break;
  }
  const WgradForm f = wgrad_form(pl.route == WGR_CIN3 ? cin3_params(p, d) : p, pl.gen, pl.aligned).form;
  if (wgrad_refusal(f)) return wgrad_refusal(f);
  if (pl.route == WGR_CIN3) return f == WG_REG_BF16_DY ? "conv_wgrad_kernel<.., 0, false, true> (3 input channels padded to 4, bf16 dy)"
                                                       : "conv_wgrad_kernel (3 input channels padded to 4)";
  switch (f) {
    case WG_BF16S_128: return "conv_wgrad_bf16s_kernel<1> + slab_reduce_kernel";
    case WG_BF16S_256: return "conv_wgrad_bf16s_kernel<2> + slab_reduce_kernel";
    case WG_REG_BF16: return "conv_wgrad_kernel<.., 1, true, true> + slab_reduce_kernel";
    case WG_REG_BF16_DY: return "conv_wgrad_kernel<.., 0, false, true> + slab_reduce_kernel";
    case WG_CT1: return "conv_wgrad_kernel<.., 1> + slab_reduce_kernel";
    case WG_CT2: return "conv_wgrad_kernel<.., 2> + slab_reduce_kernel";
    default: return "conv_wgrad_kernel + slab_reduce_kernel";
  }
}

extern "C" int munit_conv2d_wgrad(const munit_conv_desc* d, const void* x, const void* dy, float* dw,
                                  float* db, float beta, void* ws, size_t ws_bytes,
                                  munit_stream_t stream) {
  const WgradRoutePlan pl = plan_wgrad(d);
  if (pl.rc) return pl.rc;
  const int Ho = pl.Ho, Wo = pl.Wo;
  MUNIT_CHECK_ARG(x && dy && dw && ws, "conv2d_wgrad: null pointer");
  if (ws_bytes < pl.ws_bytes) {
    munit_set_error("conv2d_wgrad: workspace %zu < %zu", ws_bytes, pl.ws_bytes);
    return MUNIT_ERR_WORKSPACE;
  }
  hipStream_t st = (hipStream_t)stream;
  WgradParams p = wgrad_params(d, Ho, Wo);
  p.x = x; p.dy = dy;
  switch (pl.route) {
    case WGR_WINO_S2:
    case WGR_WINO: return munit_wino_wgrad_launch(wino_wgrad_params(d, Ho, Wo, pl.route, x, dy), dw, 0, db, beta, beta, ws, st);
    case WGR_SMALL:
      MUNIT_CHECK_ARG(d->out_dtype == MUNIT_DTYPE_F32, "conv2d_wgrad: the 3-channel image head has an fp32 dy");
      return munit_small_wgrad(d, Ho, Wo, x, reinterpret_cast<const float*>(dy), dw, db, beta, ws, st);
    case WGR_SUBPIXEL: {
      const SubpixelPlan& sp = pl.sp;
      float* dwc = reinterpret_cast<float*>(ws);
      void* slabs = reinterpret_cast<char*>(ws) + sp.dwc_bytes;
      const WgradParams f = subpixel_frame_params(p, d, sp, Ho, Wo);
      int rc = run_wgrad(f, sp.frame, pl.aligned, dw, db, beta, beta, slabs, st);
      if (rc) return rc;
      if (sp.wino) rc = munit_wino_wgrad_launch(wino_wgrad_params(d, Ho, Wo, pl.route, x, dy), dwc, (long long)d->Cout * 9 * d->Cin, db, 0.0f, 1.0f, slabs, st);
      for (int ph = 0; ph < 4 && !sp.wino && !rc; ++ph)
        rc = run_wgrad(subpixel_phase_params(p, d, Wo, ph), sp.phase, pl.aligned, dwc + (long long)ph * d->Cout * 9 * d->Cin, db, 0.0f, 1.0f, slabs, st);
      if (rc) return rc;
      const long long total = (long long)d->Cout * 25 * d->Cin;
      const int blocks = (int)std::min<long long>((total + 255) / 256, 4096);
      hipLaunchKernelGGL(upw_scatter_kernel, dim3(blocks), dim3(256), 0, st, dwc, dw, d->Cout, d->Cin);
      MUNIT_CHECK_LAUNCH("upw_scatter");
      return MUNIT_OK;
    }
    case WGR_CIN3: {
      float* x4 = reinterpret_cast<float*>(ws);
      float* dw4 = reinterpret_cast<float*>(reinterpret_cast<char*>(ws) + pl.x4_bytes);
      void* slabs = reinterpret_cast<char*>(ws) + pl.x4_bytes + pl.dw4_bytes;
      const long long npix = (long long)d->B * d->H * d->W;
      hipLaunchKernelGGL(pad3to4_kernel, dim3((unsigned)std::min<long long>((npix + 255) / 256, 8192)), dim3(256), 0, st,
                         reinterpret_cast<const float*>(x), reinterpret_cast<f32x4*>(x4), npix);
      MUNIT_CHECK_ARG(d->in_dtype == MUNIT_DTYPE_F32, "conv2d_wgrad: 3-channel inputs are fp32");
      MUNIT_CHECK_LAUNCH("pad3to4");
      WgradParams c = cin3_params(p, d);
      c.x = x4;
      const int rc = run_wgrad(c, pl.gen, pl.aligned, dw4, db, 0.0f, beta, slabs, st);
      if (rc) return rc;
      const long long n3 = (long long)d->Cout * d->KH * d->KW * 3;
      hipLaunchKernelGGL(compact4to3_kernel, dim3((unsigned)std::min<long long>((n3 + 255) / 256, 4096)), dim3(256), 0, st, dw4, dw,
                         n3, beta);
      MUNIT_CHECK_LAUNCH("compact4to3");
      return MUNIT_OK;
    }
    case WGR_GENERIC: break;
  }
  return run_wgrad(p, pl.gen, pl.aligned, dw, db, beta, beta, ws, st);
}

#ifdef WGB_STAMP
extern "C" int munit_debug_wgrad_bf16_stamps(long long* host_out) {
  return hipMemcpyFromSymbol(host_out, HIP_SYMBOL(g_wgb_stamps), sizeof(long long) * 8 * 8 * 4) == hipSuccess ? 0 : -1;
}
#endif
```

Baseline: 80.08 images/s.

## Merge subpixel border ring taps into five pixel classes with pre-summed weights

The one-pixel border ring of the upsample plus reflect-pad 5x5 conv is sorted into five position classes (top/bottom by parity, left/right by parity, corners). Within each class, reflected input taps that land on the same source pixel are summed into at most six grouped taps, either in the weights (forward) or in the gradient (wgrad). Wgrad gets a new RING variant of the conv kernel, a per-class slab reduce, and an extended scatter that folds the grouped gradients back into the 25-tap layout. This removes the redundant 25-tap border GEMM at the cost of an extra reduce kernel and more workspace. The forward path stays behind an opt-in environment flag, while the wgrad path is enabled by default.

```diff
diff --git a/munit_amd/csrc/common.h b/munit_amd/csrc/common.h
--- a/munit_amd/csrc/common.h
+++ b/munit_amd/csrc/common.h
@@ -71,6 +71,36 @@
   return r < 0 ? -1 : (r >> ups);
 }
 
+constexpr int RING_CLASSES = 5, RING_TAPS = 6;
+__host__ __device__ inline long long ring_image_elems(int Cin, int Cout) { return (long long)RING_CLASSES * RING_TAPS * Cin * Cout; }
+__host__ __device__ inline int ring_row_kind(int cls) { return cls == 2 ? 0 : cls == 3 ? 1 : 2; }
+__host__ __device__ inline int ring_col_kind(int cls) { return cls == 0 ? 0 : cls == 1 ? 1 : 2; }
+__host__ __device__ inline int ring_groups(int kind) { return kind == 2 ? 2 : 3; }
+__host__ __device__ inline int ring_tap_mask(int kind, int g) {
+  return kind == 0 ? (g == 0 ? 0x03 : g == 1 ? 0x0C : 0x10) : kind == 1 ? (g == 0 ? 0x01 : g == 1 ? 0x06 : 0x18) : (g == 0 ? 0x0E : 0x11);
+}
+__host__ __device__ inline int ring_group_of(int kind, int k) { return kind == 0 ? k >> 1 : kind == 1 ? (k + 1) >> 1 : (k >= 1 && k <= 3 ? 0 : 1); }
+__host__ __device__ inline int ring_src(int o, int n, int kind, int g) {
+  if (kind == 2) return o == 0 ? g : n - 1 - g;
+  const int s = (o >> 1) - 1 + g;
+  return s < 0 ? 0 : s >= n ? n - 1 : s;
+}
+__host__ __device__ inline int ring_rows(int cls, int H, int W) { return cls < 2 ? 2 * (W - 1) : cls < 4 ? 2 * (H - 1) : 4; }
+__host__ __device__ inline void ring_decode(int cls, int m, int H, int W, int& b, int& oh, int& ow) {
+  const int n = ring_rows(cls, H, W);
+  b = m / n;
+  const int r = m - b * n;
+  if (cls == 4) {
+    oh = (r >> 1) ? 2 * H - 1 : 0;
+    ow = (r & 1) ? 2 * W - 1 : 0;
+    return;
+  }
+  const int half = n >> 1, side = r >= half, j = r - side * half;
+  const int par = cls & 1, o = par ? 2 * j + 1 : 2 * j + 2;
+  if (cls < 2) { oh = side ? 2 * H - 1 : 0; ow = o; }
+  else { ow = side ? 2 * W - 1 : 0; oh = o; }
+}
+
 double munit_igemm_executed_flops(const munit_conv_desc* d, int pass);
 const char* munit_igemm_kernel_name(const munit_conv_desc* d, int pass);
 
diff --git a/munit_amd/csrc/conv_igemm.hip b/munit_amd/csrc/conv_igemm.hip
--- a/munit_amd/csrc/conv_igemm.hip
+++ b/munit_amd/csrc/conv_igemm.hip
@@ -35,6 +35,7 @@
   int out_bf16;
   int bf16s;
   int cin4;
+  int ring;
 };
 
 __device__ inline f32x4 bf16x8_add4(f32x4 l, f32x4 a, f32x4 b, f32x4 c) {
@@ -160,7 +161,12 @@
   const float* __restrict__ xg = p.x;
   const float* __restrict__ wg = p.w;
   long long y_base = 0;
-  if (p.ps > 1) {
+  const int cls = ROLE == 3 ? (int)blockIdx.y : 0;
+  const int Mrows = ROLE == 3 ? p.B * ring_rows(cls, p.H, p.W) : p.M;
+  if constexpr (ROLE == 3) {
+    if (m0 >= Mrows) return;
+    wg += (long long)cls * p.w_phase;
+  } else if (p.ps > 1) {
     const int pa = blockIdx.y / p.ps, pb = blockIdx.y % p.ps;
     wg += (long long)blockIdx.y * p.w_phase;
     y_base = (long long)pa * p.y_phase_row + (long long)pb * p.y_phase_col;
@@ -177,13 +183,14 @@
 #pragma unroll
   for (int i = 0; i < AROWS; ++i) {
     int m = m0 + r0 + RSTEP * i;
-    a_ok[i] = m < p.M;
+    a_ok[i] = m < Mrows;
     int mm = a_ok[i] ? m : 0;
     int b, oh, ow;
-    decode_pixel(mm, p.Ho, p.Wo, p.frame, b, oh, ow);
+    if constexpr (ROLE == 3) ring_decode(cls, mm, p.H, p.W, b, oh, ow);
+    else decode_pixel(mm, p.Ho, p.Wo, p.frame, b, oh, ow);
     a_base[i] = b * p.H * p.W;
-    a_ih0[i] = oh * p.stride - p.pad;
-    a_iw0[i] = ow * p.stride - p.pad;
+    a_ih0[i] = ROLE == 3 ? oh : oh * p.stride - p.pad;
+    a_iw0[i] = ROLE == 3 ? ow : ow * p.stride - p.pad;
     if constexpr (PATCH) {
       constexpr int NONE = -(1 << 20);
       const int P = p.f_pad, K1 = p.KH - 1;
@@ -261,6 +268,12 @@
         }
         aoff[i] = o0;
         aoff1[i] = o1;
+      } else if constexpr (ROLE == 3) {
+        const int rk = ring_row_kind(cls), ck = ring_col_kind(cls), ncg = ring_groups(ck);
+        const int rg = kw / ncg, cg = kw - rg * ncg;
+        const bool ok = a_ok[i] && rg < ring_groups(rk);
+        const int ih = ring_src(a_ih0[i], p.H, rk, rg), iw = ring_src(a_iw0[i], p.W, ck, cg);
+        aoff[i] = ok ? (a_base[i] + ih * p.W + iw) * p.Cin : -1;
       } else {
         const int ih = src_coord(a_ih0[i] + kh, p.Hu, p.ups, p.reflect);
         const int iw = src_coord(a_iw0[i] + kw, p.Wu, p.ups, p.reflect);
@@ -633,7 +646,7 @@
 #pragma unroll 2
   for (int row = cr0; row < BM; row += CRPT) {
     const int m = m0 + row;
-    if (m >= p.M || n >= p.Cout) continue;
+    if (m >= Mrows || n >= p.Cout) continue;
     f32x4 v = *reinterpret_cast<const f32x4*>(&Cs[row * CLD + cq * 4]);
     if (split) {
       float* dst = sl + (long long)m * p.Cout + n;
@@ -647,7 +660,8 @@
       continue;
     }
     int b, oh, ow;
-    decode_pixel(m, p.Ho, p.Wo, p.frame, b, oh, ow);
+    if constexpr (ROLE == 3) ring_decode(cls, m, p.H, p.W, b, oh, ow);
+    else decode_pixel(m, p.Ho, p.Wo, p.frame, b, oh, ow);
     const long long off = y_base + (long long)b * p.y_sb + (long long)oh * p.y_sh + (long long)ow * p.y_sw + n;
 #pragma unroll
     for (int e = 0; e < 4; ++e) v[e] = apply_act(v[e] + bv[e], p.act, p.slope);
@@ -681,10 +695,15 @@
     const int ph = (int)(i / per);
     const long long r = i - (long long)ph * per;
     const int m = (int)(r / p.Cout), n = (int)(r - (long long)m * p.Cout);
+    int b, oh, ow;
+    if (p.ring) {
+      if (m >= p.B * ring_rows(ph, p.H, p.W)) continue;
+      ring_decode(ph, m, p.H, p.W, b, oh, ow);
+    } else {
+      decode_pixel(m, p.Ho, p.Wo, p.frame, b, oh, ow);
+    }
     float s = 0.f;
     for (int k = 0; k < p.ksplit; ++k) s += p.slab[((long long)ph * p.ksplit + k) * per + r];
-    int b, oh, ow;
-    decode_pixel(m, p.Ho, p.Wo, p.frame, b, oh, ow);
     long long off = (long long)b * p.y_sb + (long long)oh * p.y_sh + (long long)ow * p.y_sw + n;
     if (p.ps > 1) off += (long long)(ph / p.ps) * p.y_phase_row + (long long)(ph % p.ps) * p.y_phase_col;
     const float bv = p.bias != nullptr ? p.bias[n] : 0.f;
@@ -736,6 +755,36 @@
     for (int kw = w0; kw < w0 + wn; ++kw) s += it.w[(((long long)co * 5 + kh) * 5 + kw) * it.Cin + ci];
   if (it.bf16) reinterpret_cast<bf16_t*>(it.wp)[i] = (bf16_t)s;
   else it.wp[i] = s;
+}
+
+__global__ void ring_weights_kernel(const float* __restrict__ w, float* __restrict__ wr, int Cout, int Cin) {
+  const int c16 = Cin >> 4;
+  const long long total = (long long)RING_CLASSES * Cout * RING_TAPS * c16;
+  for (long long j = (long long)blockIdx.x * blockDim.x + threadIdx.x; j < total; j += (long long)gridDim.x * blockDim.x) {
+    long long r = j;
+    const int ci = (int)(r % c16) * 16; r /= c16;
+    const int t = (int)(r % RING_TAPS); r /= RING_TAPS;
+    const int co = (int)(r % Cout); r /= Cout;
+    const int cls = (int)r;
+    const int rk = ring_row_kind(cls), ck = ring_col_kind(cls), ncg = ring_groups(ck);
+    const int rg = t / ncg, cg = t - rg * ncg;
+    f32x4 s[4] = {{0.f, 0.f, 0.f, 0.f}, {0.f, 0.f, 0.f, 0.f}, {0.f, 0.f, 0.f, 0.f}, {0.f, 0.f, 0.f, 0.f}};
+    if (rg < ring_groups(rk)) {
+      const int mh = ring_tap_mask(rk, rg), mw = ring_tap_mask(ck, cg);
+#pragma unroll
+      for (int kh = 0; kh < 5; ++kh)
+#pragma unroll
+        for (int kw = 0; kw < 5; ++kw)
+          if (((mh >> kh) & 1) && ((mw >> kw) & 1)) {
+            const f32x4* src = reinterpret_cast<const f32x4*>(w + (((long long)co * 5 + kh) * 5 + kw) * Cin + ci);
+#pragma unroll
+            for (int q = 0; q < 4; ++q) s[q] += src[q];
+          }
+    }
+    f32x4* dst = reinterpret_cast<f32x4*>(wr + (((long long)cls * Cout + co) * RING_TAPS + t) * Cin + ci);
+#pragma unroll
+    for (int q = 0; q < 4; ++q) dst[q] = s[q];
+  }
 }
 
 __host__ __device__ inline long long prep_elems(const PrepItem& it) {
@@ -987,6 +1036,30 @@
   return MUNIT_OK;
 }
 
+int launch_ring(const IgemmParams& p, hipStream_t st, void* slab, size_t slab_bytes) {
+  const int bn = igemm_bn(p);
+  IgemmParams q = p;
+  q.n_tiles = cdiv(p.Cout, bn);
+  q.ksplit = 1;
+  const int ks = slab != nullptr ? pick_ksplit(p.M, p.Cout, p.Ktot, RING_CLASSES) : 1;
+  if (ks > 1 && slab_bytes >= splitk_bytes(p.M, p.Cout, p.Ktot, RING_CLASSES)) {
+    const int nk = cdiv(p.Ktot, BK);
+    q.kt_per_split = cdiv(nk, ks);
+    q.ksplit = cdiv(nk, q.kt_per_split);
+    q.slab = reinterpret_cast<float*>(slab);
+  }
+  dim3 grid((unsigned)(cdiv(p.M, BM) * q.n_tiles), RING_CLASSES, (unsigned)q.ksplit);
+  dim3 block(NTHR);
+  IGEMM_LAUNCH(true, 3, 3);
+  MUNIT_CHECK_LAUNCH("conv_igemm ring");
+  if (q.ksplit > 1) {
+    const long long total = (long long)p.M * p.Cout * RING_CLASSES;
+    hipLaunchKernelGGL(splitk_epilogue_kernel, dim3((unsigned)std::min<long long>((total + 255) / 256, 4096)), dim3(256), 0, st, q, RING_CLASSES);
+    MUNIT_CHECK_LAUNCH("splitk_epilogue");
+  }
+  return MUNIT_OK;
+}
+
 int check_desc(const munit_conv_desc* d) {
   MUNIT_CHECK_ARG(d != nullptr, "conv: null descriptor");
   MUNIT_CHECK_ARG(d->B > 0 && d->H > 0 && d->W > 0 && d->Cin > 0 && d->Cout > 0, "conv: bad dims");
@@ -1106,6 +1179,18 @@
   p->M = d->B * (2 * ring * Wo + 2 * ring * (Ho - 2 * ring));
 }
 
+bool merged_ring_ok() {
+  return NWAVES == 8 && MUNIT_ENV_FLAG("MUNIT_MERGED_RING_FWD") && !MUNIT_ENV_FLAG("MUNIT_DEBUG_NO_MERGED_RING") && !MUNIT_ENV_FLAG("MUNIT_DEBUG_NO_DMA");
+}
+int ring_max_rows(const munit_conv_desc* d) { return d->B * std::max(ring_rows(0, d->H, d->W), std::max(ring_rows(2, d->H, d->W), 4)); }
+void set_merged_ring(IgemmParams* p, const munit_conv_desc* d) {
+  p->ring = 1; p->frame = 0; p->ps = 1;
+  p->KH = 1; p->KW = RING_TAPS; p->stride = 1; p->pad = 0;
+  p->Ktot = RING_TAPS * d->Cin; p->w_row = p->Ktot;
+  p->w_phase = (long long)d->Cout * p->Ktot;
+  p->M = ring_max_rows(d);
+}
+
 bool wino_geometry_ok(const munit_conv_desc* d) {
   return d->compute == MUNIT_COMPUTE_F32 && d->in_dtype == MUNIT_DTYPE_F32 && d->out_dtype == MUNIT_DTYPE_F32 &&
          d->KH == 3 && d->KW == 3 && d->stride == 1 && d->pad == 1 && d->upsample == 0 && d->act != MUNIT_ACT_TANH;
@@ -1145,6 +1230,8 @@
   munit_prep_item prep;
   Cin4Plan cin4;
   int ring;
+  int merged;
+  size_t ringw_bytes;
   size_t img_bytes, ws_bytes;
 };
 FwdPlan plan_fwd(const munit_conv_desc* d) {
@@ -1159,6 +1246,7 @@
     const bool wino = subpixel_wino_ok(d);
     pl.route = wino ? FWD_SUBPIXEL_WINO : FWD_SUBPIXEL; kind = wino ? MUNIT_PREP_SUBPIXEL_WINOGRAD : MUNIT_PREP_SUBPIXEL;
     pl.ring = wino ? 1 : 2;
+    pl.merged = wino && merged_ring_ok();
   } else if (wino_fwd_ok(d)) {
     pl.route = FWD_WINO; kind = MUNIT_PREP_WINOGRAD;
   } else if (wino_s2_fwd_ok(d)) {
@@ -1171,8 +1259,10 @@
   if (pl.route == FWD_SMALL) pl.ws_bytes = munit_small_fwd_workspace(d);
   if (pl.route == FWD_CIN4) pl.cin4 = plan_cin4((long long)d->B * d->H * d->W, d->Cout, d->KH * d->KW), pl.ws_bytes = pl.cin4.x4_bytes + pl.cin4.w4_bytes;
   if (bf16 || munit_small_fwd_supported(d)) return pl;
+  if (pl.merged) pl.ws_bytes += pl.ringw_bytes = align_up((size_t)ring_image_elems(d->Cin, d->Cout) * sizeof(float), 256);
   if (pl.ring)
-    pl.ws_bytes += std::max(splitk_bytes(d->B * (4 * Wo + 4 * (Ho - 4)), d->Cout, Ktot, 1), splitk_bytes(d->B * (2 * Wo + 2 * (Ho - 2)), d->Cout, Ktot, 1));
+    pl.ws_bytes += std::max(std::max(splitk_bytes(d->B * (4 * Wo + 4 * (Ho - 4)), d->Cout, Ktot, 1), splitk_bytes(d->B * (2 * Wo + 2 * (Ho - 2)), d->Cout, Ktot, 1)),
+                            splitk_bytes(ring_max_rows(d), d->Cout, RING_TAPS * d->Cin, RING_CLASSES));
   if (pl.route == FWD_IGEMM) pl.ws_bytes += splitk_bytes(d->B * Ho * Wo, d->Cout, Ktot, 1);
   return pl;
 }
@@ -1274,6 +1364,16 @@
   if (pl.ring) {
     if (pl.route == FWD_SUBPIXEL) rc = launch_igemm<0>(subpixel_phase_params(p, d, Wo), 4, st);
     if (rc) return rc;
+    if (pl.merged) {
+      float* wr = reinterpret_cast<float*>(reinterpret_cast<char*>(ws) + pl.img_bytes);
+      const long long trips = ring_image_elems(d->Cin, d->Cout) / 16;
+      hipLaunchKernelGGL(ring_weights_kernel, dim3((unsigned)std::min<long long>((trips + 255) / 256, 4096)), dim3(256), 0, st, w, wr, d->Cout, d->Cin);
+      MUNIT_CHECK_LAUNCH("ring_weights");
+      set_merged_ring(&p, d);
+      p.w = wr;
+      const size_t head = pl.img_bytes + pl.ringw_bytes;
+      return launch_ring(p, st, reinterpret_cast<char*>(ws) + head, ws_bytes - head);
+    }
     set_subpixel_frame(&p, d, Ho, Wo, pl.ring);
     p.w = pl.prep.bf16 ? reinterpret_cast<const float*>(reinterpret_cast<const bf16_t*>(wimg) + (size_t)4 * 9 * d->Cout * d->Cin) : w;
   }
@@ -1780,7 +1880,8 @@
   if (pass == MUNIT_PASS_FWD) {
     const FwdPlan fp = plan_fwd(d);
     switch (fp.route) {
-      case FWD_SUBPIXEL_WINO: return cc * d->B * ((double)(d->H / 2) * (d->W / 2) * 4 * 16 + (2.0 * Wo + 2.0 * (Ho - 2)) * 25);
+      case FWD_SUBPIXEL_WINO:
+        return cc * d->B * ((double)(d->H / 2) * (d->W / 2) * 4 * 16 + (fp.merged ? (2.0 * Wo + 2.0 * (Ho - 2) - 4) * 6 + 4 * 4 : (2.0 * Wo + 2.0 * (Ho - 2)) * 25));
       case FWD_SUBPIXEL: return cc * d->B * ((double)d->H * d->W * 4 * 9 + (4.0 * Wo + 4.0 * (Ho - 4)) * 25);
       case FWD_WINO: return cc * d->B * (d->H / 2) * (d->W / 2) * 16;
       case FWD_WINO_S2: return 4 * cc * d->B * cdiv(Ho, 3) * cdiv(Wo, 3) * 16;
diff --git a/munit_amd/csrc/conv_wgrad.hip b/munit_amd/csrc/conv_wgrad.hip
--- a/munit_amd/csrc/conv_wgrad.hip
+++ b/munit_amd/csrc/conv_wgrad.hip
@@ -82,9 +82,10 @@
 
 __device__ inline int img_off(int row, int ch) { return 256 * row + 16 * (ch ^ (((row & 3) << 2) | ((row >> 2) & 3))); }
 
-template <int BC, bool ALIGNED, bool FAST, int CT = 0, bool XB = false, bool DYB = false>
+template <int BC, bool ALIGNED, bool FAST, int CT = 0, bool XB = false, bool DYB = false, bool RING = false>
 __global__ __launch_bounds__(WTHR, 4) void conv_wgrad_kernel(WgradParams p) {
   constexpr bool DMA = CT == 3;
+  static_assert(!RING || (ALIGNED && !FAST && CT == 0), "merged ring: aligned generic loader only");
   static_assert(!(XB || DYB) || (FAST && !DMA), "bf16 tensors: FAST register loader only");
   constexpr bool BF16 = CT == 1 || CT == 2;
   static_assert(!DMA || (FAST && ALIGNED), "direct-to-LDS loads: FAST variants only");
@@ -113,11 +114,14 @@
   const int lane = tid & 63;
   const int wave = tid >> 6;
   const int wm = wave >> 2, wn = wave & 3;
-  const int kc0 = blockIdx.x * WKT;
+  const int ktc = RING ? (p.Ktot + WKT - 1) / WKT : 1;
+  const int cls = RING ? (int)blockIdx.x / ktc : 0;
+  const int kc0 = (RING ? (int)blockIdx.x - cls * ktc : (int)blockIdx.x) * WKT;
   const int co0 = blockIdx.y * BC;
   const int split = blockIdx.z;
   const int m_begin = split * p.pix_per_split;
-  const int m_end = min(p.M, m_begin + p.pix_per_split);
+  const int m_end = min(RING ? p.B * ring_rows(cls, p.H, p.W) : p.M, m_begin + p.pix_per_split);
+  const int rk = ring_row_kind(cls), ck = ring_col_kind(cls);
 
   const int xq = tid % XQ;
   const int xr0 = tid / XQ;
@@ -235,11 +239,18 @@
       const int m = mbase + xr0 + XRPT * i;
       const bool mok = m < m_end;
       int b, oh, ow;
-      decode_pixel(mok ? m : 0, p.Ho, p.Wo, p.frame, b, oh, ow);
+      if constexpr (RING) ring_decode(cls, mok ? m : 0, p.H, p.W, b, oh, ow);
+      else decode_pixel(mok ? m : 0, p.Ho, p.Wo, p.frame, b, oh, ow);
       const long long base = (long long)b * p.H * p.W;
       int ih0 = oh * p.stride - p.pad, iw0 = ow * p.stride - p.pad;
       f32x4 v = {0.f, 0.f, 0.f, 0.f};
-      if constexpr (ALIGNED) {
+      if constexpr (RING) {
+        const int ncg = ring_groups(ck), rg = ekw[0] / ncg, cg = ekw[0] - rg * ncg;
+        if (mok && eok[0] && rg < ring_groups(rk)) {
+          const int ih = ring_src(oh, p.H, rk, rg), iw = ring_src(ow, p.W, ck, cg);
+          v = *reinterpret_cast<const f32x4*>(reinterpret_cast<const float*>(p.x) + (base + (long long)ih * p.W + iw) * p.Cin + eci[0]);
+        }
+      } else if constexpr (ALIGNED) {
         int ih = src_coord(ih0 + ekh[0], p.Hu, p.ups, p.reflect);
         int iw = src_coord(iw0 + ekw[0], p.Wu, p.ups, p.reflect);
         if (mok && eok[0] && ih >= 0 && iw >= 0)
@@ -261,7 +272,8 @@
       const int m = mbase + dr0 + DRPT * i;
       const bool mok = m < m_end;
       int b, oh, ow;
-      decode_pixel(mok ? m : 0, p.Ho, p.Wo, p.frame, b, oh, ow);
+      if constexpr (RING) ring_decode(cls, mok ? m : 0, p.H, p.W, b, oh, ow);
+      else decode_pixel(mok ? m : 0, p.Ho, p.Wo, p.frame, b, oh, ow);
       const float* ptr = reinterpret_cast<const float*>(p.dy) + (long long)b * p.dy_sb + (long long)oh * p.dy_sh +
                          (long long)ow * p.dy_sw + p.dy_off + co0 + dq * 4;
       const int co = co0 + dq * 4;
@@ -378,7 +390,7 @@
 #pragma unroll
       for (int r = 0; r < 4; ++r) acc[a][t][r] = 0.f;
   float bsum = 0.f;
-  const bool do_bias = p.bias_slab != nullptr && blockIdx.x == 0;
+  const bool do_bias = p.bias_slab != nullptr && (RING ? kc0 == 0 : blockIdx.x == 0);
 
   const int fj = lane & 15;
   const int fg = lane >> 4;
@@ -545,7 +557,8 @@
     }
   }
 
-  float* out = p.slab + (long long)split * p.Cout * p.Ktot;
+  const long long slice = RING ? (long long)split * RING_CLASSES + cls : split;
+  float* out = p.slab + slice * p.Cout * p.Ktot;
   if constexpr (BF16) {
 #pragma unroll
     for (int t = 0; t < MT; ++t)
@@ -584,7 +597,7 @@
       }
     }
   }
-  if (do_bias && tid < BC && co0 + tid < p.Cout) p.bias_slab[(long long)split * p.Cout + co0 + tid] = bsum;
+  if (do_bias && tid < BC && co0 + tid < p.Cout) p.bias_slab[slice * p.Cout + co0 + tid] = bsum;
 }
 
 constexpr int BS_WP = 64;
@@ -786,6 +799,22 @@
   }
 }
 
+__global__ void ring_reduce_kernel(const float* __restrict__ slab, float* __restrict__ dwr, long long n,
+                                   const float* __restrict__ bias_slab, float* __restrict__ db, int nb, int nsplit, float beta_b) {
+  const long long total = n + (db != nullptr ? nb : 0);
+  for (long long i = (long long)blockIdx.x * blockDim.x + threadIdx.x; i < total; i += (long long)gridDim.x * blockDim.x) {
+    float s = 0.f;
+    if (i < n) {
+      for (int k = 0; k < nsplit; ++k) s += slab[(long long)k * n + i];
+      dwr[i] = s;
+    } else {
+      const long long j = i - n;
+      for (int k = 0; k < nsplit * RING_CLASSES; ++k) s += bias_slab[(long long)k * nb + j];
+      db[j] = (beta_b != 0.f ? beta_b * db[j] : 0.f) + s;
+    }
+  }
+}
+
 __global__ __launch_bounds__(1024) void slab_reduce_wide_kernel(const float* __restrict__ slab, float* __restrict__ dw,
                                                                 long long n, const float* __restrict__ bias_slab,
                                                                 float* __restrict__ db, int nb, int nsplit, float beta,
@@ -833,7 +862,8 @@
   return c;
 }
 
-__global__ void upw_scatter_kernel(const float* __restrict__ dwc, float* __restrict__ dw, int Cout, int Cin) {
+__global__ void upw_scatter_kernel(const float* __restrict__ dwc, const float* __restrict__ dwr, float* __restrict__ dw, int Cout,
+                                   int Cin, float beta) {
   const long long total = (long long)Cout * 25 * Cin;
   const long long per_phase = (long long)Cout * 9 * Cin;
   for (long long i = (long long)blockIdx.x * blockDim.x + threadIdx.x; i < total;
@@ -853,7 +883,18 @@
         s += dwc[(a * 2 + b) * per_phase + (((long long)co * 3 + dh) * 3 + dw_) * Cin + ci];
       }
     }
-    dw[i] += s;
+    if (dwr == nullptr) {
+      dw[i] += s;
+      continue;
+    }
+    const long long per_class = (long long)Cout * RING_TAPS * Cin;
+#pragma unroll
+    for (int cls = 0; cls < RING_CLASSES; ++cls) {
+      const int rk = ring_row_kind(cls), ck = ring_col_kind(cls);
+      const int t = ring_group_of(rk, kh) * ring_groups(ck) + ring_group_of(ck, kw);
+      s += dwr[cls * per_class + ((long long)co * RING_TAPS + t) * Cin + ci];
+    }
+    dw[i] = (beta != 0.f ? beta * dw[i] : 0.f) + s;
   }
 }
 
@@ -1031,7 +1072,23 @@
   size_t dwc_bytes, slab_bytes;
   bool wino;
   int ring;
+  bool merged;
 };
+bool merged_ring_wgrad_ok(const munit_conv_desc* d) { return d->Cin % 4 == 0 && d->Cout % 4 == 0 && !MUNIT_ENV_FLAG("MUNIT_DEBUG_NO_MERGED_RING"); }
+int ring_max_rows(const munit_conv_desc* d) { return d->B * std::max(ring_rows(0, d->H, d->W), std::max(ring_rows(2, d->H, d->W), 4)); }
+void plan_ring(const munit_conv_desc* d, WgradPlan* pl) {
+  const int M = ring_max_rows(d), Ktot = RING_TAPS * d->Cin;
+  pl->bc = d->Cout <= 64 ? 64 : 128;
+  pl->k_tiles = RING_CLASSES * cdiv(Ktot, pl->bc == 128 ? 128 : 256);
+  pl->c_tiles = cdiv(d->Cout, pl->bc);
+  const int want = std::max(1, 256 * wgrad_blocks_per_cu(pl->bc, true) / (pl->k_tiles * pl->c_tiles));
+  int ns = std::max(1, std::min(std::min(want, std::max(1, M / 128)), 512));
+  int pps = (cdiv(M, ns) + WP - 1) / WP * WP;
+  pl->nsplit = cdiv(M, pps);
+  pl->pix_per_split = pps;
+  pl->slab_bytes = align_up((size_t)pl->nsplit * RING_CLASSES * d->Cout * Ktot * sizeof(float), 256);
+  pl->bias_bytes = align_up((size_t)pl->nsplit * RING_CLASSES * d->Cout * sizeof(float), 256);
+}
 void plan_subpixel(const munit_conv_desc* d, SubpixelPlan* sp) {
   const bool aligned = d->Cin % 4 == 0;
   plan_launch(d->B * (d->H - 2) * (d->W - 2), 9 * d->Cin, d->Cout, aligned, &sp->phase);
@@ -1040,8 +1097,10 @@
              d->W >= 4 && munit_wino_wgrad_ok(d->B, d->H, d->W, d->Cin, d->Cout) &&
              (long long)d->B * 4 * d->H * d->W * d->Cout < (1ll << 29);
   sp->ring = sp->wino ? 1 : 2;
-  plan_launch(d->B * (2 * sp->ring * Wo + 2 * sp->ring * (Ho - 2 * sp->ring)), 25 * d->Cin, d->Cout, aligned, &sp->frame);
-  sp->dwc_bytes = align_up((size_t)4 * d->Cout * 9 * d->Cin * sizeof(float), 256);
+  sp->merged = sp->wino && merged_ring_wgrad_ok(d);
+  if (sp->merged) plan_ring(d, &sp->frame);
+  else plan_launch(d->B * (2 * sp->ring * Wo + 2 * sp->ring * (Ho - 2 * sp->ring)), 25 * d->Cin, d->Cout, aligned, &sp->frame);
+  sp->dwc_bytes = align_up(((size_t)4 * d->Cout * 9 * d->Cin + (sp->merged ? (size_t)ring_image_elems(d->Cin, d->Cout) : 0)) * sizeof(float), 256);
   sp->slab_bytes = std::max(sp->phase.slab_bytes + sp->phase.bias_bytes, sp->frame.slab_bytes + sp->frame.bias_bytes);
   if (sp->wino)
     sp->slab_bytes = std::max(sp->slab_bytes, munit_wino_wgrad_workspace((long long)d->B * (d->H / 2) * (d->W / 2), d->Cin, d->Cout, 4));
@@ -1177,6 +1236,7 @@
     case WGR_WINO: return cc * d->B * (d->H / 2) * (d->W / 2) * 16;
     case WGR_WINO_S2: return 4 * cc * (double)s2_tiles(d) * 16;
     case WGR_SUBPIXEL:
+      if (pl.sp.merged) return cc * d->B * ((double)d->H * d->W * 4 * 4 + (2.0 * Wo + 2.0 * (Ho - 2) - 4) * 6 + 4 * 4);
       if (pl.sp.wino) return cc * d->B * ((double)d->H * d->W * 4 * 4 + (2.0 * Wo + 2.0 * (Ho - 2)) * 25);
       return cc * d->B * ((double)(d->H - 2) * (d->W - 2) * 4 * 9 + (4.0 * Wo + 4.0 * (Ho - 4)) * 25);
     case WGR_CIN3: return 2.0 * 4 * d->Cout * d->B * Ho * Wo * d->KH * d->KW;
@@ -1262,8 +1322,26 @@
       const SubpixelPlan& sp = pl.sp;
       float* dwc = reinterpret_cast<float*>(ws);
       void* slabs = reinterpret_cast<char*>(ws) + sp.dwc_bytes;
-      const WgradParams f = subpixel_frame_params(p, d, sp, Ho, Wo);
-      int rc = run_wgrad(f, sp.frame, pl.aligned, dw, db, beta, beta, slabs, st);
+      int rc = MUNIT_OK;
+      float* dwr = nullptr;
+      if (sp.merged) {
+        dwr = dwc + (long long)4 * d->Cout * 9 * d->Cin;
+        WgradParams f = p;
+        f.KH = 1; f.KW = RING_TAPS; f.Ktot = RING_TAPS * d->Cin; f.M = ring_max_rows(d);
+        f.slab = reinterpret_cast<float*>(slabs);
+        f.bias_slab = db ? reinterpret_cast<float*>(reinterpret_cast<char*>(slabs) + sp.frame.slab_bytes) : nullptr;
+        f.pix_per_split = sp.frame.pix_per_split;
+        dim3 grid((unsigned)sp.frame.k_tiles, (unsigned)sp.frame.c_tiles, (unsigned)sp.frame.nsplit);
+        if (sp.frame.bc == 64) hipLaunchKernelGGL((conv_wgrad_kernel<64, true, false, 0, false, false, true>), grid, dim3(WTHR), 0, st, f);
+        else hipLaunchKernelGGL((conv_wgrad_kernel<128, true, false, 0, false, false, true>), grid, dim3(WTHR), 0, st, f);
+        MUNIT_CHECK_LAUNCH("conv_wgrad ring");
+        const long long n = ring_image_elems(d->Cin, d->Cout);
+        hipLaunchKernelGGL(ring_reduce_kernel, dim3((unsigned)std::min<long long>((n + d->Cout + 255) / 256, 4096)), dim3(256), 0, st,
+                           f.slab, dwr, n, f.bias_slab, db, d->Cout, sp.frame.nsplit, beta);
+        MUNIT_CHECK_LAUNCH("ring_reduce");
+      } else {
+        rc = run_wgrad(subpixel_frame_params(p, d, sp, Ho, Wo), sp.frame, pl.aligned, dw, db, beta, beta, slabs, st);
+      }
       if (rc) return rc;
       if (sp.wino) rc = munit_wino_wgrad_launch(wino_wgrad_params(d, Ho, Wo, pl.route, x, dy), dwc, (long long)d->Cout * 9 * d->Cin, db, 0.0f, 1.0f, slabs, st);
       for (int ph = 0; ph < 4 && !sp.wino && !rc; ++ph)
@@ -1271,7 +1349,7 @@
       if (rc) return rc;
       const long long total = (long long)d->Cout * 25 * d->Cin;
       const int blocks = (int)std::min<long long>((total + 255) / 256, 4096);
-      hipLaunchKernelGGL(upw_scatter_kernel, dim3(blocks), dim3(256), 0, st, dwc, dw, d->Cout, d->Cin);
+      hipLaunchKernelGGL(upw_scatter_kernel, dim3(blocks), dim3(256), 0, st, dwc, dwr, dw, d->Cout, d->Cin, beta);
       MUNIT_CHECK_LAUNCH("upw_scatter");
       return MUNIT_OK;
     }
```

Result: no change. 80.53 images/s, median of 6 (+0.6%).
